# qcc4cp/qcc

Measured on AMD Instinct MI355X. Metric: gate-applies/sec (2^30-amplitude units), QFT, higher is better.
Workload: dtype f64; 1 GPU; 30-qubit QFT complex128, 465 gates/step (qc.qft order), basis-state input, state resident in HBM, 2^30 amplitudes per GPU [BASELINE config 2]; qubits=30, fusion=1

## Files before the change

### include/qcc_hip.h

```cpp
#ifndef QCC_HIP_H_
#define QCC_HIP_H_

#include <stdint.h>

#ifdef __cplusplus
extern "C" {
#endif

typedef struct qh_state_s *qh_handle;

#define QH_OK 0
#define QH_ERR_BAD_QUBIT 1
#define QH_ERR_SAME_QUBIT 2
#define QH_ERR_BAD_DTYPE 3
#define QH_ERR_HIP 4
#define QH_ERR_ARG 5
#define QH_ERR_NOMEM 6
#define QH_ERR_NO_DEVICE 7
#define QH_ERR_NONLOCAL 8
#define QH_ERR_COMM 9

#define QH_FUSE_OFF 0
#define QH_FUSE_SWEEP 1

const char *qh_last_error(void);
int qh_version(void);
int qh_device_count(int *count);

int qh_create(int nbits, int bit_width, int device, qh_handle *out);
int qh_attach(int nbits, int bit_width, int device, void *device_ptr,
              void *hip_stream, qh_handle *out);
int qh_create_host_mapped(int nbits, int bit_width, int device, qh_handle *out);
int qh_host_ptr(qh_handle h, void **host_ptr);
int qh_create_dry(int nbits, int bit_width, qh_handle *out);
int qh_destroy(qh_handle h);

int qh_set_shard(qh_handle h, int nbits_global, uint64_t shard_index);
int qh_device_ptr(qh_handle h, void **ptr);
int qh_set_relayout(qh_handle h, int on, int *actual);
int qh_stream(qh_handle h, void **stream);
int qh_nbits(qh_handle h, int *nbits_local, int *nbits_global);

int qh_init_basis(qh_handle h, uint64_t index);
int qh_init_product(qh_handle h, int nfactors, const int *nq, const double *const *amps,
                    const uint64_t *basis);
int qh_upload(qh_handle h, const void *host, uint64_t offset, uint64_t count);
int qh_download(qh_handle h, void *host, uint64_t offset, uint64_t count);

int qh_apply1(qh_handle h, int tgt, const double gate[8]);
int qh_applyc(qh_handle h, int ctl, int tgt, const double gate[8]);
int qh_apply_bits(qh_handle h, uint64_t ctl_mask, int tgt_bit,
                  const double gate[8]);
int qh_apply_matrix(qh_handle h, int k, const int32_t *bits, uint64_t ctl_mask, const double *matrix);

int qh_apply_mux(qh_handle h, int k, const int32_t *sel_bits, int tgt_bit, const double *gates);
int qh_apply_diag(qh_handle h, int k, const int32_t *bits, const double *values);

#define QH_NO_CTL INT32_MIN
int qh_apply_stream(qh_handle h, uint64_t count, const int32_t *ops, const double *gates);

int qh_set_fusion(qh_handle h, int level);
int qh_flush(qh_handle h);
int qh_sync(qh_handle h);
int qh_pending_gates(qh_handle h, uint64_t *count);
int qh_discard_pending(qh_handle h);

int qh_remap_swap(qh_handle h, int phys_bit_a, int phys_bit_b);
int qh_get_bitmap(qh_handle h, int32_t *phys_of_logical );
int qh_phys_to_logical(qh_handle h, uint64_t phys_index, uint64_t *logical);
int qh_logical_to_phys(qh_handle h, uint64_t logical_index, uint64_t *phys);

#define QH_COMM_ID_BYTES 128
typedef int (*qh_round_fn)(void *user, int npeers, const int *peers, void *const *send_host,
                           void *const *recv_host, uint64_t bytes);
typedef struct {
  uint64_t exchanges;
  uint64_t rounds;
  uint64_t bytes_sent;
  uint64_t slabs;
  uint64_t sweeps_overlapped;
  double span_ms;
  uint64_t rounds_packed;
  uint64_t geometry_checks;
  uint32_t comm_ranks;
  uint32_t comm_rank;
} qh_xstats;
typedef struct {
  uint64_t signature;
  uint64_t slab_mask;
  uint64_t block_bits;
  uint64_t rounds_per_slab;
  uint64_t staging_bytes;
  uint32_t slabs;
  uint32_t chunk_bits;
  uint32_t packed;
  uint32_t peers;
  uint32_t sweeps_before;
  uint32_t last_sweep_split;
} qh_xgeom;
int qh_exchange_geometry(qh_handle h, qh_xgeom *out);
int qh_comm_init_dry(qh_handle h, int nranks, int rank);
int qh_comm_unique_id(void *id );
int qh_comm_init(qh_handle h, int nranks, int rank, const void *id);
int qh_comm_init_custom(qh_handle h, int nranks, int rank, qh_round_fn fn, void *user);
int qh_comm_destroy(qh_handle h);
int qh_exchange_alltoall(qh_handle h, int base_bit, uint64_t chunk_amps);
int qh_exchange_pair(qh_handle h, int shard_bit, int local_bit, uint64_t chunk_amps);
int qh_exchange_loopback(qh_handle h, int local_bit, uint64_t chunk_amps);
int qh_exchange_wait(qh_handle h);
int qh_exchange_stats(qh_handle h, qh_xstats *out);
int qh_comm_allreduce_sum(qh_handle h, double *inout, int count);

int qh_norm2(qh_handle h, double *out);
int qh_amplitude(qh_handle h, uint64_t logical_index, double out[2]);
int qh_argmax(qh_handle h, uint64_t *phys_index, double *prob);
int qh_prob_bit(qh_handle h, int logical_bit, double *p1);
int qh_prob_bit_value(qh_handle h, int logical_bit, int value, double *p);
int qh_scale(qh_handle h, double re, double im);
int qh_project_bit(qh_handle h, int logical_bit, int value);
int qh_marginal(qh_handle h, int k, const int32_t *bits, double *out);
int qh_sample(qh_handle h, uint64_t count, const double *u, uint64_t *logical_out);
int qh_project_bits(qh_handle h, uint64_t mask, uint64_t value);
int qh_expect_pauli(qh_handle h, uint64_t nterms, const uint64_t *xmask, const uint64_t *zmask, double *out);
typedef struct { uint64_t index; double re, im; } qh_entry;
#define QH_SELECT_MAX (1u << 20)
#define QH_TOPK_MAX 4096
int qh_select(qh_handle h, double threshold, uint64_t cap, qh_entry *out, uint64_t *count, double *weight);
int qh_topk(qh_handle h, uint64_t k, qh_entry *out, uint64_t *count);
int qh_amplitudes(qh_handle h, uint64_t count, const uint64_t *logical, double *out, uint64_t *nlocal);

int qh_clone(qh_handle src, qh_handle *out);
int qh_copy(qh_handle dst, qh_handle src);
int qh_inner(qh_handle a, qh_handle b, double out[2]);
#define QH_INNER_LINEAR 0
#define QH_INNER_TILES 1
#define QH_INNER_GATHER 2
typedef struct {
  uint32_t path;
  uint32_t nrest;
  uint64_t free_a, free_b;
  uint8_t tile_a[8], tile_b[8], shuffle[8];
  uint8_t rest_a[56], rest_b[56];
  uint8_t pos_b[64];
} qh_inner_tiles;
int qh_inner_plan(qh_handle a, qh_handle b, qh_inner_tiles *out);
int qh_axpby(qh_handle dst, const double alpha[2], qh_handle src, const double beta[2], double *norm2);

int qh_extend(qh_handle src, int k, const double *amps, uint64_t basis, qh_handle *out);
int qh_release(qh_handle src, int k, const int32_t *bits, uint64_t value, double weight[2], qh_handle *out);

typedef struct {
  uint64_t gates_submitted;
  uint64_t kernels_launched;
  uint64_t sweeps;
  uint64_t bytes_algorithmic;
  uint64_t bytes_swept;
  uint64_t gates_noop;
} qh_stats;
int qh_get_stats(qh_handle h, qh_stats *out);
int qh_reset_stats(qh_handle h);
int qh_timer_begin(qh_handle h);
int qh_timer_end(qh_handle h, float *milliseconds);
int qh_timer_lap(qh_handle h);
int qh_timer_laps(qh_handle h, float *milliseconds, int cap, int *count);
int qh_plan_json(qh_handle h, char *buf, uint64_t cap, uint64_t *needed);

int qh_plan_export(qh_handle h, void *buf, uint64_t cap, uint64_t *needed);

int qh_plan_handlers(qh_handle h, void *buf, uint64_t cap, uint64_t *needed);

int qh_host_apply1(void *psi, const double gate[8], int nbits, int tgt,
                   int bit_width);
int qh_host_applyc(void *psi, const double gate[8], int nbits, int ctl, int tgt,
                   int bit_width);
int qh_host_release(void);

#ifdef __cplusplus
}
#endif
#endif
```

### qcc_amd/csrc/engine.hip

```cpp
#include <hip/hip_runtime.h>

#include <algorithm>
#include <chrono>
#include <cmath>
#include <cstdarg>
#include <cstddef>
#include <cstdio>
#include <cstdlib>
#include <cstring>
#include <ctime>
#include <string>
#include <vector>

#include "../../include/qcc_hip.h"
#include "buffers.hip.h"
#include "kernels_gate.hip.h"
#include "kernels_dense.hip.h"
#include "kernels_mux.hip.h"
#include "kernels_measure.hip.h"
#include "kernels_select.hip.h"
#include "select_plan.h"
#include "kernels_expect.hip.h"
#include "kernels_inner.hip.h"
#include "kernels_axpby.hip.h"
// ... 221 lines not shown
  launch_diag_u<R, 2, true>(h, nwork, sel, ins, f0r, f0i, f1r, f1i, lowpred);
}

int launch_single(qh_state_s *h, const qh::GateRec &r) {
  const Placed ctl = place(h, r.ctl_mask);
  if ((h->shard & ctl.held) != ctl.held) {
    h->stats.gates_noop++;
    return QH_OK;
  }
  const uint64_t cm_all = ctl.local;
  const LowSplit low = split_low(h, cm_all);
  uint32_t lowpred = low.lowpred;
  const uint64_t cm = low.cm;
  const int nc_all = __builtin_popcountll(cm_all);
  const int nc = __builtin_popcountll(cm);
  if (nc + 1 > qh::kMaxIns) return fail(QH_ERR_ARG, "too many local control bits (%d)", nc);
  const double *g = r.g;
  const bool diag = qh::is_diag(g);
  auto diag_kernel = [&](uint64_t nwork, int sel, uint64_t ones, double f0r, double f0i, double f1r, double f1i) {
    if (h->dry) return;
    const qh::BitIns ins = make_ins(ones, -1);
    with_real(h, [&](auto x) { launch_diag<decltype(x)>(h, nwork, sel, ins, f0r, f0i, f1r, f1i, lowpred); });
  };
  if (r.tgt >= h->nloc) {
    if (!diag)
      return fail(QH_ERR_NONLOCAL,
                  "non-diagonal gate targets physical bit %d held by the shard index "
                  "(local bits: %d); exchange first",
                  r.tgt, h->nloc);
    const bool set = (h->shard >> (r.tgt - h->nloc)) & 1ull;
    const double fr = set ? g[6] : g[0], fi = set ? g[7] : g[1];
    if (fr == 1.0 && fi == 0.0) {
      h->stats.gates_noop++;
      return QH_OK;
    }
    const uint64_t nwork = 1ull << (h->nloc - nc);
    diag_kernel(nwork, -1, cm, 1, 0, fr, fi);
    count_kernel(h, 1ull << (h->nloc - nc_all), nwork);
    return QH_OK;
  }
  if (diag) {
    const bool one_sided = (g[0] == 1.0 && g[1] == 0.0);
    if (one_sided && g[6] == 1.0 && g[7] == 0.0) {
      h->stats.gates_noop++;
      return QH_OK;
    }
    if (one_sided) {
      const bool tgt_low = h->nloc > 2 && r.tgt < 2;
      if (tgt_low) lowpred |= 1u << r.tgt;
      const uint64_t nwork = 1ull << (h->nloc - nc - (tgt_low ? 0 : 1));
      diag_kernel(nwork, -1, tgt_low ? cm : (cm | (1ull << r.tgt)), 1, 0, g[6], g[7]);
      count_kernel(h, 1ull << (h->nloc - nc_all - 1), nwork);
    } else {
      const uint64_t nwork = 1ull << (h->nloc - nc);
      diag_kernel(nwork, r.tgt, cm, g[0], g[1], g[6], g[7]);
      count_kernel(h, 1ull << (h->nloc - nc_all), nwork);
    }
    return QH_OK;
  }
  const uint64_t nwork = 1ull << (h->nloc - nc - 1);
  if (!h->dry) {
    const qh::BitIns ins = make_ins(cm, r.tgt), ins1 = make_ins(cm, -1);
    with_real(h, [&](auto x) { launch_pair<decltype(x)>(h, nwork, r.tgt, ins, ins1, g, lowpred); });
  }
  count_kernel(h, 1ull << (h->nloc - nc_all), 2 * nwork);
  return QH_OK;
}

int check_launch(qh_state_s *h) {
  if (h->dry) return QH_OK;
  hipError_t e = hipGetLastError();
  if (e != hipSuccess) return fail(QH_ERR_HIP, "kernel launch: %s", hipGetErrorString(e));
  return QH_OK;
}

int use_device(qh_state_s *h) {
  if (h->dry) return QH_OK;
  HIP_TRY(hipSetDevice(h->device));
  return QH_OK;
}

int comm_timeout_ms() { return env_int("QH_COMM_TIMEOUT_MS", 300000); }
bool watched(const qh_state_s *h) {
  if (!h->comm || h->comm->dry) return false;
  return (h->comm->nranks > 1 && !h->comm->custom) || env_int("QH_COMM_WATCH_ALL", 0) != 0;
}
void abort_comm_and_drain(qh_state_s *h) {
  qh::Comm *c = h->comm;
  if (!c || c->dry) return;
  if (c->nccl) {
    (void)qh::rccl().CommAbort(c->nccl);
    c->nccl = nullptr;
  }
  const auto t0 = std::chrono::steady_clock::now();
  for (hipStream_t s : {c->xstream, c->cstream, c->pstream, h->stream}) {
    if (!s) continue;
    while (hipStreamQuery(s) == hipErrorNotReady) {
      if (std::chrono::duration<double>(std::chrono::steady_clock::now() - t0).count() > 10.0) return;
      struct timespec ts = {0, 200000};
      nanosleep(&ts, nullptr);
    }
  }
  (void)hipGetLastError();
}
template <typename Query> int poll_until_done(qh_state_s *h, Query query, const char *what) {
  const auto t0 = std::chrono::steady_clock::now();
  for (unsigned spins = 0;; ++spins) {
    const hipError_t e = query();
    if (e == hipSuccess) return QH_OK;
    if (e != hipErrorNotReady) {
      (void)hipGetLastError();
      return fail(QH_ERR_HIP, "%s: %s", what, hipGetErrorString(e));
    }
    if (spins > 2000) {
      const double ms = std::chrono::duration<double, std::milli>(std::chrono::steady_clock::now() - t0).count();
      if (ms > comm_timeout_ms()) {
        h->poisoned = true;
        abort_comm_and_drain(h);
        return fail(QH_ERR_COMM, "%s: rank %d of %d still waiting after %.0f s (QH_COMM_TIMEOUT_MS): a peer is missing or the "
                    "ranks disagree about an exchange; the communicator was aborted, the state of this handle is undefined", what,
                    h->comm->rank, h->comm->nranks, ms * 1e-3);
      }
      struct timespec ts = {0, 50000};
      nanosleep(&ts, nullptr);
    }
  }
}
int wait_stream(qh_state_s *h, hipStream_t s, const char *what) {
  if (!watched(h)) {
    HIP_TRY(hipStreamSynchronize(s));
    return QH_OK;
  }
  return poll_until_done(h, [&] { return hipStreamQuery(s); }, what);
}
int wait_event(qh_state_s *h, hipEvent_t e, const char *what) {
  if (!watched(h)) {
    HIP_TRY(hipEventSynchronize(e));
    return QH_OK;
  }
  return poll_until_done(h, [&] { return hipEventQuery(e); }, what);
}

bool relayout_eligible(const qh_state_s *h) {
  return env_int("QH_RELAYOUT", 1) != 0 && h->owns_mem && !h->host_psi && qh::sweep_supported(h->nloc, h->bw);
}
bool relayout_wanted(const qh_state_s *h) {
  if (h->dry) return env_int("QH_RELAYOUT", 1) != 0;
  if (h->relayout >= 0) return h->relayout == 1;
  return relayout_eligible(h) && !(h->comm && h->comm->nranks > 1);
}
qh::PlanRequest plan_request(const qh_state_s *h, bool relayout) {
  return qh::PlanRequest{h->nloc, h->bw, h->shard, relayout, h->nglob > h->nloc, qh::PlanSwitches::from_env()};
}
hipError_t alloc_state_buffer(void **p, size_t bytes) {
  static const int contig = env_int("QH_ALLOC_CONTIG", -1), debug = env_int("QH_ALLOC_DEBUG", 0);
  const auto t0 = std::chrono::steady_clock::now();
  hipError_t e = hipErrorOutOfMemory;
  bool got_contig = false;
  const bool want_contig = contig < 0 ? (bytes >= (4ull << 30) && bytes <= (32ull << 30)) : (contig > 0 && bytes >= (64ull << 20));
  if (want_contig) {
    e = hipExtMallocWithFlags(p, bytes, hipDeviceMallocContiguous);
    got_contig = e == hipSuccess;
    if (!got_contig) {
      (void)hipGetLastError();
      *p = nullptr;
    }
  }
  if (!got_contig) e = hipMalloc(p, bytes);
  if (debug)
    fprintf(stderr, "[qh alloc %zu MiB %s at %p in %.1f ms]\n", bytes >> 20, got_contig ? "contiguous" : "plain", *p,
            std::chrono::duration<double, std::milli>(std::chrono::steady_clock::now() - t0).count());
  return e;
}
bool second_buffer_fits(const qh_state_s *h, size_t bytes) {
  size_t fr = 0, total = 0;
  const size_t reserve = (bytes >> 5) + (3ull << 29) + ((h->comm && h->comm->nranks > 1) ? (4ull << 30) : 0);
  return hipMemGetInfo(&fr, &total) == hipSuccess && fr > bytes + reserve;
}
bool alloc_second_buffer(qh_state_s *h) {
  if (h->d_alt) return true;
  const size_t bytes = (size_t)h->amp_bytes() << h->nloc;
  if (second_buffer_fits(h, bytes) && alloc_state_buffer(&h->d_alt, bytes) == hipSuccess)
    return true;
  (void)hipGetLastError();
  h->d_alt = nullptr;
  return false;
}
bool relayout_ready(qh_state_s *h) {
  if (h->dry) return relayout_wanted(h);
  if (h->relayout < 0) {
    h->relayout = 0;
    if (relayout_eligible(h) && !(h->comm && h->comm->nranks > 1) && alloc_second_buffer(h)) h->relayout = 1;
  }
  return h->relayout == 1;
}

bool layout_is_canonical(const qh_state_s *h) {
  int last = -1;
  for (int b = 0; b < h->nglob; ++b) {
    if (h->perm[b] >= h->nloc) continue;
    if (h->perm[b] < last) return false;
    last = h->perm[b];
  }
  return true;
}

int canonicalize(qh_state_s *h) {
  if (h->dry || layout_is_canonical(h)) return QH_OK;
  const bool borrowed = !h->d_alt;
  if (borrowed && !alloc_second_buffer(h))
    return fail(QH_ERR_NOMEM, "no room for the second buffer of %llu bytes that bringing a permuted layout back to canonical order needs",
                (unsigned long long)(h->amp_bytes() << h->nloc));
  std::vector<int> loc;
  for (int b = 0; b < h->nglob; ++b) if (h->perm[b] < h->nloc) loc.push_back(b);
  std::vector<int> posn;
  for (int b : loc) posn.push_back(h->perm[b]);
  std::sort(posn.begin(), posn.end());
  qh::BitPerm bp{};
  bp.n = h->nloc;
  for (size_t k = 0; k < loc.size(); ++k) bp.src_of_dst[posn[k]] = (uint8_t)h->perm[loc[k]];
  const uint64_t n = 1ull << h->nloc;
  with_real(h, [&](auto x) {
    using R = decltype(x);
    using A = typename qh::AmpT<R>::type;
    hipLaunchKernelGGL(qh::k_permute_bits<R>, dim3(grid_for(n, 1ull << 22)), dim3(256), 0, h->stream, (const A *)h->d_psi, (A *)h->d_alt, n, bp);
  });
  int rc = check_launch(h);
  if (rc == QH_OK && borrowed) {
    hipError_t e = hipMemcpyAsync(h->d_psi, h->d_alt, (size_t)h->amp_bytes() << h->nloc, hipMemcpyDefault, h->stream);
    if (e == hipSuccess) e = hipStreamSynchronize(h->stream);
    if (e != hipSuccess) rc = fail(QH_ERR_HIP, hipGetErrorString(e));
  }
  if (borrowed) {
    if (rc) (void)hipStreamSynchronize(h->stream);
    (void)hipFree(h->d_alt);
    h->d_alt = nullptr;
  } else if (rc == QH_OK) {
    std::swap(h->d_psi, h->d_alt);
  }
  if (rc) return rc;
  for (size_t k = 0; k < loc.size(); ++k) h->perm[loc[k]] = posn[k];
  return QH_OK;
}

int flush_impl(qh_state_s *h, qh::SlabIO *split = nullptr, qh::TileMaxOut *tmax = nullptr) {
  int rc = use_device(h);
  if (rc) return rc;
  if (h->poisoned)
    return fail(QH_ERR_HIP, "the state of this handle is undefined: a sweep of an earlier flush failed after others had run; "
                            "re-initialise it (qh_init_basis / qh_init_product / qh_upload of the whole shard)");
  std::vector<qh::Arrival> *arr = (h->comm && !h->comm->arrivals.empty()) ? &h->comm->arrivals : nullptr;
  if (h->queue.empty()) {
    qh::wait_all_arrivals(arr, h->stream);
    return QH_OK;
  }
  if (h->fusion == QH_FUSE_SWEEP && qh::sweep_supported(h->nloc, h->bw)) {
    const uint64_t launched0 = h->stats.kernels_launched;
    qh::SlabIO local;
    qh::SlabIO *io = split ? split : &local;
    io->arrivals = arr;
    io->comm = h->comm;
    const bool relay = relayout_ready(h);
    void *result = h->d_psi;
    uint8_t final_pos[64];
    rc = qh::run_fused(h->queue, plan_request(h, relay), h->d_psi, h->stream, h->dry, &h->sweep, &h->stats, &g_err,
                       h->comm ? io : nullptr, h->d_alt, &result, final_pos, tmax);
    if (rc == QH_OK && relay) {
      if (result != h->d_psi) std::swap(h->d_psi, h->d_alt);
      for (int b = 0; b < h->nglob; ++b)
        if (h->perm[b] < h->nloc) h->perm[b] = final_pos[h->perm[b]];
    }
    qh::wait_all_arrivals(arr, h->stream);
    if (h->comm) h->comm->stats.sweeps_overlapped += io->sweeps_overlapped;
    if (rc != QH_OK && h->stats.kernels_launched == launched0) return rc;
    if (rc == QH_OK) rc = check_launch(h);
    if (rc != QH_OK) {
      g_err += " [sweeps of this flush may have run partially: its gates were dropped and the state is undefined until re-initialised]";
      h->poisoned = true;
    }
    h->queue.clear();
    return rc;
  }
  qh::wait_all_arrivals(arr, h->stream);
  size_t done = 0;
  for (const auto &r : h->queue) {
    rc = launch_single(h, r);
    if (rc == QH_OK) rc = check_launch(h);
    if (rc) break;
    ++done;
  }
  h->queue.erase(h->queue.begin(), h->queue.begin() + done);
  return rc;
}

int enter(qh_state_s *h) {
  if (h->dry) return fail(QH_ERR_ARG, "not on a dry (planner-only) handle");
  return flush_impl(h);
}
int read_back(qh_state_s *h, void *host, const void *dev, size_t bytes, const char *what = "reader") {
  HIP_TRY(hipMemcpyAsync(host, dev, bytes, hipMemcpyDeviceToHost, h->stream));
  return wait_stream(h, h->stream, what);
}

int set_relayout(qh_state_s *h, bool on, int *actual = nullptr) {
  if (h->dry) {
    if (actual) *actual = relayout_wanted(h) ? 1 : 0;
// ... 1824 lines not shown
  return QH_OK;
}

}

namespace {

constexpr uint64_t kExpectBlocks = 4096;

template <typename R, int TT>
void launch_expect(qh_state_s *h, bool pair, unsigned nblk, const qh::ExpectArgs &a, double *slab) {
  using A = typename qh::AmpT<R>::type;
  if (pair)
    hipLaunchKernelGGL((qh::k_expect_batch<R, TT, true>), dim3(nblk), dim3(256), 0, h->stream, (const A *)h->d_psi, a, slab);
  else
    hipLaunchKernelGGL((qh::k_expect_batch<R, TT, false>), dim3(nblk), dim3(256), 0, h->stream, (const A *)h->d_psi, a, slab);
}

}

extern "C" {

int qh_expect_pauli(qh_handle h, uint64_t nterms, const uint64_t *xmask, const uint64_t *zmask, double *out) {
  if (!h || (nterms && (!xmask || !zmask || !out))) return fail(QH_ERR_ARG, "expect_pauli: null handle, masks or out");
  if (h->nglob < 64)
    for (uint64_t t = 0; t < nterms; ++t)
      if ((xmask[t] | zmask[t]) >> h->nglob)
        return fail(QH_ERR_BAD_QUBIT, "expect_pauli: term %llu (x 0x%llx, z 0x%llx) has bits >= %d", (unsigned long long)t,
                    (unsigned long long)xmask[t], (unsigned long long)zmask[t], h->nglob);
  int rc = enter(h);
  if (rc) return rc;
  if (nterms == 0) return QH_OK;
  struct Term { uint64_t px, pz, idx; uint32_t neg, ny; };
  std::vector<Term> terms(nterms);
  for (uint64_t t = 0; t < nterms; ++t) {
    const Placed x = place(h, to_phys(h, xmask[t])), z = place(h, to_phys(h, zmask[t]));
    if (x.held) {
      const int b = __builtin_ctzll(to_logical(h, x.held << h->nloc));
      return fail(QH_ERR_NONLOCAL, "expect_pauli: term %llu has X or Y on logical bit %d, held by the shard index (physical bit %d, "
                  "local bits: %d); exchange first", (unsigned long long)t, b, h->perm[b], h->nloc);
    }
    terms[t] = Term{x.local, z.local, t, (uint32_t)__builtin_popcountll(h->shard & z.held) & 1u,
                    (uint32_t)__builtin_popcountll(xmask[t] & zmask[t]) & 3u};
  }
  std::stable_sort(terms.begin(), terms.end(), [](const Term &l, const Term &r) { return l.px < r.px; });
  qh::ScratchLayout lay;
  const size_t slab_off = lay.add((size_t)kExpectBlocks * qh::kExpectT * sizeof(double)), out_off = lay.add((size_t)nterms * sizeof(double));
  HIP_TRY(h->meas.reserve(lay.total));
  double *slab = (double *)(h->meas.as<char>() + slab_off), *dout = (double *)(h->meas.as<char>() + out_off);
  uint64_t batches = 0;
  for (uint64_t first = 0; first < nterms;) {
    uint64_t cnt = 1;
    while (first + cnt < nterms && cnt < (uint64_t)qh::kExpectT && terms[first + cnt].px == terms[first].px) ++cnt;
    const uint64_t px = terms[first].px;
    const bool pair = (px >> 6) != 0;
    qh::ExpectArgs a{};
    a.x = px;
    a.tb = pair ? 63 - __builtin_clzll(px) : 0;
    const int per_bits = pair ? 3 : 4, nom = 8 + per_bits, wbits = pair ? h->nloc - 1 : h->nloc;
    a.cw = std::min(nom, wbits);
    const uint64_t nchunks = 1ull << (wbits - a.cw), nblk = std::min(nchunks, kExpectBlocks);
    a.cpb = (uint32_t)(nchunks / nblk);
    for (uint64_t k = 0; k < cnt; ++k) {
      const Term &tm = terms[first + k];
      uint64_t z = tm.pz;
      if (pair) z = (z & ((1ull << a.tb) - 1ull)) | ((z >> (a.tb + 1)) << a.tb);
      a.zt[k] = (uint8_t)(z & 255ull);
      const uint32_t zu = (uint32_t)(z >> 8) & ((1u << per_bits) - 1u);
      for (uint32_t u = 0; u < (1u << per_bits); ++u) a.zu[k] |= (uint16_t)((__builtin_popcount(u & zu) & 1) << u);
      a.zc[k] = z >> nom;
      const uint32_t one = (((tm.ny >> 1) ^ tm.neg) & 1u) ? 0xBFF00000u : 0x3FF00000u;
      if (tm.ny & 1u) a.cim[k] = one; else a.cre[k] = one;
    }
    const int tt = cnt <= 4 ? 4 : qh::kExpectT;
    with_real(h, [&](auto x) {
      using R = decltype(x);
      if (tt == 4) launch_expect<R, 4>(h, pair, (unsigned)nblk, a, slab);
      else launch_expect<R, qh::kExpectT>(h, pair, (unsigned)nblk, a, slab);
    });
    hipLaunchKernelGGL(qh::k_expect_fold, dim3((unsigned)cnt), dim3(256), 0, h->stream, (const double *)slab, (uint32_t)nblk, tt,
                       pair ? 2.0 : 1.0, dout + first);
    if ((rc = check_launch(h))) return rc;
    first += cnt;
    ++batches;
  }
  std::vector<double> vals(nterms);
  if ((rc = read_back(h, vals.data(), dout, (size_t)nterms * sizeof(double)))) return rc;
  for (uint64_t k = 0; k < nterms; ++k) out[terms[k].idx] = vals[k];
  h->stats.kernels_launched += batches;
  h->stats.bytes_swept += batches * ((1ull << h->nloc) * h->amp_bytes());
  return QH_OK;
}

int qh_get_stats(qh_handle h, qh_stats *out) {
  if (!h || !out) return fail(QH_ERR_ARG, "null");
  *out = h->stats;
  return QH_OK;
}
int qh_reset_stats(qh_handle h) {
  if (!h) return fail(QH_ERR_ARG, "null");
  h->stats = qh_stats{};
  return QH_OK;
}

int qh_timer_begin(qh_handle h) {
  if (!h) return fail(QH_ERR_ARG, "null handle");
  int rc = enter(h);
  if (rc) return rc;
  rc = make_events(h);
  if (rc) return rc;
  HIP_TRY(hipEventRecord(h->ev0, h->stream));
  return QH_OK;
}
int qh_timer_end(qh_handle h, float *ms) {
  if (!h || !ms) return fail(QH_ERR_ARG, "null handle or out");
  if (!h->ev0) return fail(QH_ERR_ARG, "qh_timer_end without qh_timer_begin");
  int rc = enter(h);
  if (rc) return rc;
  HIP_TRY(hipEventRecord(h->ev1, h->stream));
  if ((rc = wait_event(h, h->ev1, "qh_timer_end"))) return rc;
  HIP_TRY(hipEventElapsedTime(ms, h->ev0, h->ev1));
  return QH_OK;
}

int qh_timer_lap(qh_handle h) {
  if (!h) return fail(QH_ERR_ARG, "null handle");
  const int rc = enter(h);
  if (rc) return rc;
  if (h->laps_used == h->laps.size()) {
    hipEvent_t e = nullptr;
    HIP_TRY(hipEventCreate(&e));
    h->laps.push_back(e);
  }
  HIP_TRY(hipEventRecord(h->laps[h->laps_used++], h->stream));
  return QH_OK;
}
int qh_timer_laps(qh_handle h, float *ms, int cap, int *count) {
  if (!h || !count || h->dry) return fail(QH_ERR_ARG, "null/dry");
  HIP_TRY(hipSetDevice(h->device));
  const int n = h->laps_used > 0 ? (int)h->laps_used - 1 : 0;
  if (h->laps_used) {
    const int rc = wait_event(h, h->laps[h->laps_used - 1], "qh_timer_laps");
    if (rc) return rc;
  }
  for (int k = 0; k < n && ms && k < cap; ++k) HIP_TRY(hipEventElapsedTime(&ms[k], h->laps[k], h->laps[k + 1]));
  *count = n;
  h->laps_used = 0;
  return QH_OK;
}

int qh_plan_json(qh_handle h, char *buf, uint64_t cap, uint64_t *needed) {
  if (!h) return fail(QH_ERR_ARG, "null");
  std::string s;
  if (int rc = qh::guard_planning(&g_err, [&] { s = qh::plan_to_json(h->queue, plan_request(h, relayout_wanted(h))); })) return rc;
  if (needed) *needed = s.size() + 1;
  if (buf && cap) {
    const uint64_t n = std::min<uint64_t>(cap - 1, s.size());
    memcpy(buf, s.data(), n);
    buf[n] = 0;
  }
  return QH_OK;
}

int qh_plan_export(qh_handle h, void *buf, uint64_t cap, uint64_t *needed) {
  if (!h) return fail(QH_ERR_ARG, "null");
  if (!qh::sweep_supported(h->nloc, h->bw)) return fail(QH_ERR_ARG, "state too small for sweeps");
  qh::PlanResult pr;
  if (int rc = qh::guard_planning(&g_err, [&] { pr = qh::plan_best(h->queue, plan_request(h, relayout_wanted(h))); })) return rc;
  std::vector<uint64_t> out;
  auto put_bytes = [&](const void *p, size_t n) {
    const size_t w = (n + 7) / 8, at = out.size();
    out.resize(at + w, 0);
    if (n) memcpy(&out[at], p, n);
  };
  out.push_back(0x51485033ull);
  out.push_back(pr.sweeps.size());
  out.push_back(pr.noop_gates);
  put_bytes(pr.final_pos, 64);
  for (auto &sp : pr.sweeps) {
    int64_t hdr[28] = {0};
    int k = 0;
    hdr[k++] = sp.rb;
    for (int i = 0; i < 6; ++i) hdr[k++] = sp.regpos[i];
    for (int i = 0; i < 6; ++i) hdr[k++] = sp.regpos_store[i];
    for (int i = 0; i < 3; ++i) hdr[k++] = sp.lanehi[i];
    hdr[k++] = sp.nwave;
    for (int i = 0; i < 2; ++i) hdr[k++] = sp.wavepos[i];
    hdr[k++] = (int64_t)sp.fixed_ones;
    hdr[k++] = (int64_t)sp.ntiles;
    hdr[k++] = (int64_t)sp.ops.size();
    hdr[k++] = (int64_t)sp.groups.size();
    hdr[k++] = (int64_t)sp.oterms.size();
    hdr[k++] = (int64_t)sp.tables.size();
    hdr[k++] = sp.n_ltab;
    hdr[k++] = sp.lane_low;
    hdr[k++] = sp.relayout ? 1 : 0;
    put_bytes(hdr, sizeof hdr);
    put_bytes(sp.dest_pos, 64);
    {
      int64_t st[20] = {0};
      for (int i = 0; i < 6; ++i) { st[i] = sp.seat[i]; st[6 + i] = sp.seat_store[i]; st[12 + i] = sp.seat_dest[i]; }
      st[18] = sp.wavepos_store[0];
      st[19] = sp.wavepos_store[1];
      put_bytes(st, sizeof st);
      int64_t kd[8 + 1 + 2 * qh::kMaxUnitSegs] = {0};
      for (int i = 0; i < 6; ++i) kd[i] = sp.reg_dest[i];
      kd[6] = sp.wave_dest[0];
      kd[7] = sp.wave_dest[1];
      uint64_t masks[qh::kMaxUnitSegs] = {0};
      int shifts[qh::kMaxUnitSegs] = {0};
      kd[8] = sp.relayout ? qh::unit_segments(sp, h->nloc, masks, shifts) : 0;
      for (int i = 0; i < qh::kMaxUnitSegs; ++i) { kd[9 + i] = (int64_t)masks[i]; kd[9 + qh::kMaxUnitSegs + i] = shifts[i]; }
      put_bytes(kd, sizeof kd);
    }
    put_bytes(sp.ops.data(), sp.ops.size() * sizeof(qh::SweepOp));
    put_bytes(sp.groups.data(), sp.groups.size() * sizeof(qh::DGroup));
    put_bytes(sp.oterms.data(), sp.oterms.size() * sizeof(qh::OTerm));
    put_bytes(sp.tables.data(), sp.tables.size() * sizeof(double));
  }
  const uint64_t bytes = out.size() * 8;
  if (needed) *needed = bytes;
  if (buf && cap) {
    if (cap < bytes) return fail(QH_ERR_ARG, "buffer too small (call with NULL to get the size)");
    memcpy(buf, out.data(), bytes);
  }
  return QH_OK;
}

int qh_plan_handlers(qh_handle h, void *buf, uint64_t cap, uint64_t *needed) {
  if (!h) return fail(QH_ERR_ARG, "null");
  if (!qh::sweep_supported(h->nloc, h->bw)) return fail(QH_ERR_ARG, "state too small for sweeps");
  qh::PlanResult pr;
  if (int rc = qh::guard_planning(&g_err, [&] { pr = qh::plan_best(h->queue, plan_request(h, relayout_wanted(h))); })) return rc;
  std::vector<uint32_t> out{0x51484831u, (uint32_t)pr.sweeps.size()};
  std::vector<qh::SweepOp> ops;
  std::vector<qh::DGroup> groups;
  for (auto &sp : pr.sweeps) {
    ops.assign(sp.ops.size() + 1, qh::SweepOp{});
    groups.assign(sp.groups.size(), qh::DGroup{});
    const uint32_t n_ltab_lds = (uint32_t)(h->bw == 128 ? qh::ltab_lds_count<true>(sp) : qh::ltab_lds_count<false>(sp));
    qh::build_device_copy(sp, h->bw, n_ltab_lds, ops.data(), groups.data());
    for (uint32_t v : {(uint32_t)h->bw, (uint32_t)sp.rb, (uint32_t)sp.nwave, (uint32_t)(sp.relayout ? 1 : 0), (uint32_t)sp.ops.size(),
                       (uint32_t)sp.groups.size()})
      out.push_back(v);
    for (size_t k = 0; k < sp.ops.size(); ++k) { out.push_back(ops[k].kind); out.push_back(ops[k].flags); }
    for (const qh::DGroup &g : groups) out.push_back(g.flags);
  }
  if (out.size() & 1) out.push_back(0);
  const uint64_t bytes = out.size() * 4;
  if (needed) *needed = bytes;
  if (buf && cap) {
    if (cap < bytes) return fail(QH_ERR_ARG, "buffer too small (call with NULL to get the size)");
    memcpy(buf, out.data(), bytes);
  }
  return QH_OK;
}

}

namespace {

#define NCCL_TRY(expr)                                                                     \
  do {                                                                                     \
    ncclResult_t r_ = (expr);                                                              \
    if (r_ != ncclSuccess)                                                                 \
      return fail(QH_ERR_COMM, "%s: %s (%s:%d)", #expr, qh::rccl().GetErrorString(r_), __FILE__, __LINE__); \
  } while (0)

int check_ranks(int nranks, int rank) {
  if (nranks < 1 || (nranks & (nranks - 1)) || rank < 0 || rank >= nranks)
    return fail(QH_ERR_ARG, "nranks %d must be a power of two, rank %d inside it", nranks, rank);
  if (nranks > qh::kMaxXferMoves + 1) return fail(QH_ERR_ARG, "at most %d ranks", qh::kMaxXferMoves + 1);
  return QH_OK;
}

int comm_common_init(qh_state_s *h, int nranks, int rank) {
  if (!h) return fail(QH_ERR_ARG, "null handle");
  if (h->comm) return fail(QH_ERR_ARG, "handle already has a communicator");
  if (int rc = check_ranks(nranks, rank)) return rc;
  if (h->bw != 128 && h->bw != 64) return fail(QH_ERR_BAD_DTYPE, "bit width");
  int rc0 = enter(h);
  if (rc0) return rc0;
  if (nranks > 1 && h->relayout != 0) {
    rc0 = set_relayout(h, false);
    if (rc0) return rc0;
  }
  auto *c = new qh::Comm;
  c->nranks = nranks;
  c->rank = rank;
  hipError_t e = hipStreamCreateWithFlags(&c->xstream, hipStreamNonBlocking);
  if (e == hipSuccess) e = hipStreamCreateWithFlags(&c->cstream, hipStreamNonBlocking);
  if (e == hipSuccess) e = hipStreamCreateWithFlags(&c->pstream, hipStreamNonBlocking);
  if (e == hipSuccess) e = hipEventCreate(&c->t0);
  if (e == hipSuccess) e = hipEventCreate(&c->t1);
  if (e != hipSuccess) {
    delete c;
    return fail(QH_ERR_HIP, "exchange streams/events: %s", hipGetErrorString(e));
  }
  h->comm = c;
  return QH_OK;
}

void close_timing(qh::Comm *c) {
  if (!c->timing_open) return;
  float ms = 0;
  if (hipEventSynchronize(c->t1) == hipSuccess && hipEventElapsedTime(&ms, c->t0, c->t1) == hipSuccess)
    c->stats.span_ms += ms;
  c->timing_open = false;
}

template <typename A>
void launch_xfer(bool unpack, void *psi, void *stage, uint64_t n, uint64_t start, const qh::XferGeom &g, hipStream_t st) {
  const uint64_t total = n * (uint64_t)g.np;
  const unsigned grid = grid_for(total, 1ull << 20);
  if (unpack) hipLaunchKernelGGL(qh::k_xunpack<A>, dim3(grid), dim3(256), 0, st, (A *)psi, (const A *)stage, n, start, g);
  else hipLaunchKernelGGL(qh::k_xpack<A>, dim3(grid), dim3(256), 0, st, (const A *)psi, (A *)stage, n, start, g);
}

int verify_geometry(qh_state_s *h, uint64_t sig) {
  qh::Comm *c = h->comm;
  if (c->nranks <= 1) return QH_OK;
  if (c->custom) {
    const int np = c->nranks - 1;
    std::vector<uint64_t> mine(np, sig), theirs(np, 0);
    std::vector<int> peers;
    std::vector<void *> sp, rp;
    for (int j = 0, k = 0; j < c->nranks; ++j) {
      if (j == c->rank) continue;
      peers.push_back(j);
      sp.push_back(&mine[k]);
      rp.push_back(&theirs[k]);
      ++k;
    }
    if (c->custom(c->custom_user, np, peers.data(), sp.data(), rp.data(), sizeof(uint64_t)) != 0)
      return fail(QH_ERR_COMM, "host-staged transport: the round callback failed (geometry check)");
    for (int k = 0; k < np; ++k)
      if (theirs[k] != sig)
        return fail(QH_ERR_COMM, "exchange geometry differs between rank %d (%016llx) and rank %d (%016llx): the ranks "
                    "planned different sweeps or layouts", c->rank, (unsigned long long)sig, peers[k], (unsigned long long)theirs[k]);
    c->stats.geometry_checks++;
    return QH_OK;
  }
  if (!c->nccl) return fail(QH_ERR_COMM, "no RCCL communicator on this handle (never set up, or aborted by the watchdog)");
  static const int mode = env_int("QH_EXCHANGE_VERIFY", -1);
  if (mode == 0) return QH_OK;
  if (mode < 0 && std::find(c->verified.begin(), c->verified.end(), sig) != c->verified.end()) return QH_OK;
  HIP_TRY(c->d_sig.reserve(4 * sizeof(double)));
  HIP_TRY(c->h_sig.reserve(8 * sizeof(double)));
  double *v = c->h_sig.as<double>(), *w = v + 4, *d_sig = c->d_sig.as<double>();
  v[0] = (double)(sig >> 32); v[1] = (double)(sig & 0xffffffffu); v[2] = -v[0]; v[3] = -v[1];
  HIP_TRY(hipMemcpyAsync(d_sig, v, 4 * sizeof(double), hipMemcpyHostToDevice, c->xstream));
  NCCL_TRY(qh::rccl().AllReduce(d_sig, d_sig, 4, ncclDouble, ncclMax, c->nccl, c->xstream));
  HIP_TRY(hipMemcpyAsync(w, d_sig, 4 * sizeof(double), hipMemcpyDeviceToHost, c->xstream));
  const int rc = wait_stream(h, c->xstream, "exchange geometry check (all-reduce of the signature)");
  if (rc) return rc;
  if (w[0] != -w[2] || w[1] != -w[3])
    return fail(QH_ERR_COMM, "exchange geometry differs between ranks (signature of rank %d: %016llx; largest / smallest halves seen: "
                "%08x%08x / %08x%08x): the ranks planned different sweeps or layouts, or run with different planner switches "
                "(QH_* environment) or builds", c->rank, (unsigned long long)sig, (unsigned)w[0], (unsigned)w[1], (unsigned)-w[2], (unsigned)-w[3]);
  if (c->verified.size() >= 256) c->verified.erase(c->verified.begin());
  c->verified.push_back(sig);
  c->stats.geometry_checks++;
  return QH_OK;
}

uint64_t env_build_hash(const qh::ExchangeSwitches &xsw) {
  std::string s = qh::PlanSwitches::from_env().key();
  s += xsw.key() + std::to_string(env_int("QH_RELAYOUT", 1) != 0) + ";";
  s += "v" + std::to_string(qh_version()) + ":" + std::to_string(sizeof(qh::SweepArgs)) + ":" + std::to_string(sizeof(qh::SweepOp)) +
       ":" + std::to_string(sizeof(qh::SweepPlan)) + ":" + std::to_string(sizeof(qh_xgeom));
  uint64_t hsh = 0xcbf29ce484222325ull;
  for (unsigned char ch : s) { hsh ^= ch; hsh *= 0x100000001b3ull; }
  return hsh;
}

void launch_packed_round(qh_state_s *h, const qh::ExchangePlan &pl, const std::vector<qh::BlockMove> &moves, bool unpack, void *stage,
                         int k, uint64_t ci, hipStream_t st) {
  qh::XferGeom g{};
  g.ins.n = pl.nins;
  for (int i = 0; i < pl.nins; ++i) g.ins.pos[i] = pl.ins_pos[i];
  g.np = pl.np;
  for (int m = 0; m < pl.np; ++m) g.off[m] = pl.packed_offset(k, unpack ? moves[m].land : moves[m].blk);
  with_real(h, [&](auto x) {
    launch_xfer<typename qh::AmpT<decltype(x)>::type>(unpack, h->d_psi, stage, pl.chunk_amps(), pl.round_start(ci), g, st);
  });
}
// ... 409 lines not shown
```

### qcc_amd/csrc/kernels_sweep.hip.h

```cpp
#pragma once
#include <hip/hip_runtime.h>

#include <string>
#include <vector>

#include "kernels_gate.hip.h"
#include <deque>
#include <memory>

#include "planner.h"
#include "exchange.hip.h"

namespace qh {

struct SweepParams {
  const SweepOp *ops;
  const DGroup *groups;
  const OTerm *oterms;
  uint32_t nops;
  uint32_t tables_rel;
  uint32_t n_ltab_lds;
  uint32_t pad0;
  uint64_t store_delta_mask;
  uint64_t prof_buf;
  uint64_t tilemax;
  uint64_t slot_off[64];
  uint64_t slot_off_store[64];
};
static_assert(kMaxInsertBits + kMaxSlabBits <= kMaxIns, "planner/kernels disagree on inserted bits");
static_assert(kExchangeSlabBits == kMaxSlabBits, "exchange_plan.h / planner disagree on slab bits");
static_assert(sizeof(SweepOp) == 96 && sizeof(DGroup) == 64 && sizeof(OTerm) == 24, "asm island layouts");
static_assert(offsetof(SweepParams, slot_off) == 0x40 && offsetof(SweepParams, nops) == 0x18 && offsetof(SweepParams, tilemax) == 0x38 &&
                  offsetof(SweepParams, slot_off_store) == 0x240 && offsetof(SweepParams, store_delta_mask) == 0x28,
              "asm island layouts");

struct LaneGeom {
  int lane_low;
  int rot;
  int blk_bits;
  int nwave;
  int wpos[kMaxWaveBits];
  int wdst[kMaxWaveBits];
  int ltab_in_island;
};

constexpr uint64_t kProfRows = 8192, kProfRecs = 128;
struct UnitPerm {
  int n;
  int shift[kMaxUnitSegs];
  uint64_t mask[kMaxUnitSegs];
  int nslab;
  int slab_pos[kMaxSlabBits];
  uint64_t slab_val;
};

struct alignas(8) SweepArgs {
  uint64_t psi;
  uint64_t dst;
  uint64_t prm;
  uint64_t idx_high;
  uint64_t nunits;
  uint64_t ins_ones;
  uint64_t slab_val;
  uint64_t ltab_src;
  uint32_t n_ltab;
  uint32_t exch_bytes;
  uint32_t stride_units;
  uint32_t seat_dest;
  uint8_t ins_n, lane_low, rot, blk_bits;
  uint8_t nwave, wpos[2], island_copies;
  uint8_t wdst[2], up_n, up_nslab;
  uint8_t slab_pos[kMaxSlabBits], wpb;
  uint8_t seat[8];
  uint8_t ins_pos[16];
  int8_t up_shift[kMaxUnitSegs];
  uint64_t up_mask[kMaxUnitSegs];
};
static_assert(kMaxUnitSegs == 8 && kMaxSlabBits == 3 && kMaxIns <= 16 && kMaxWaveBits == 2 && kLaneBits <= 8, "SweepArgs layout");
static_assert(offsetof(SweepArgs, n_ltab) == 64 && offsetof(SweepArgs, ins_n) == 80 && offsetof(SweepArgs, ins_pos) == 104 &&
                  offsetof(SweepArgs, up_shift) == 120 && offsetof(SweepArgs, up_mask) == 128 && sizeof(SweepArgs) == 192,
              "SweepArgs layout (k_sweep reads it by dword index)");

typedef uint32_t qh_u32x16 __attribute__((ext_vector_type(16)));

inline int flush_pace(const PlanResult &pr, bool wide, int nloc) {
  if (const char *e = getenv("QH_SWEEP_PACE")) return atoi(e);
  if (!wide || pr.sweeps.empty()) return 0;
  double joules = 0, ms = 0;
  for (const SweepPlan &sp : pr.sweeps) {
    if (sp.nwave > 1) return 0;
    const double units = (double)sp.swept_bytes / (2.0 * 16.0 * (double)(1ull << 30));
    ms += (nloc <= 31 ? 5.45 : 5.85) * units;
    joules += 4.9 * units + sweep_op_energy_nj(sp) * (double)sp.ntiles * 1e-9 * 1.15;
  }
  const double watts = joules / ms * 1e3;
  return (watts >= 1320.0 && watts <= 1450.0) ? 12 : 0;
}

template <int RB, bool WIDE>
__global__ __launch_bounds__(256) void k_sweep(SweepArgs args_in_kernarg_segment) {
  constexpr uint32_t kAmp = WIDE ? 16u : 8u;
#ifdef QH_PROF
  const uint64_t prof_t_entry = __builtin_amdgcn_s_memtime();
#endif
  const uint32_t lane_u = threadIdx.x & 63;
  const uint32_t wave_s = __builtin_amdgcn_readfirstlane(threadIdx.x >> 6);
  extern __shared__ __attribute__((aligned(16))) unsigned char xbuf[];
  const uint32_t lds_base = (uint32_t)(uintptr_t)(__attribute__((address_space(3))) unsigned char *)xbuf;
  for (uint32_t turn = 0;; ++turn) {
    qh_u32x16 q0, q1, q2;
    asm volatile("s_load_dwordx16 %0, %3, 0x0\n\ts_load_dwordx16 %1, %3, 0x40\n\ts_load_dwordx16 %2, %3, 0x80\n\t"
                 "s_waitcnt lgkmcnt(0)"
                 : "=&s"(q0), "=&s"(q1), "=&s"(q2)
                 : "s"((uint64_t)(uintptr_t)__builtin_amdgcn_kernarg_segment_ptr()));
    auto dw = [&](int i) -> uint32_t { return i < 16 ? q0[i] : i < 32 ? q1[i - 16] : q2[i - 32]; };
    auto qw = [&](int i) -> uint64_t { return (uint64_t)dw(i) | ((uint64_t)dw(i + 1) << 32); };
    auto by = [&](int i, int b) -> uint32_t { return (dw(i) >> (8 * b)) & 255u; };
    const uint32_t lane_low = by(20, 1), nwave = by(21, 0), wpb = by(23, 3);
    const uint32_t n_lt = dw(16), exch_bytes = dw(17);
    const uint32_t lds_ltab = lds_base + exch_bytes;
    const uint32_t wg_threads = wpb << 6;
    const bool island_copies = by(21, 3) != 0;
    if (turn == 0 && n_lt && !island_copies) {
      typedef double v2d_t __attribute__((ext_vector_type(2)));
      const __attribute__((address_space(1))) v2d_t *src = (const __attribute__((address_space(1))) v2d_t *)qw(14);
      v2d_t *dst = (v2d_t *)(xbuf + exch_bytes);
      for (uint32_t i = threadIdx.x; i < n_lt * 64u; i += wg_threads) dst[i] = src[i];
      __syncthreads();
    }
    const uint32_t nlt_now = island_copies && turn == 0 ? n_lt : 0u;
    uint64_t bi = blockIdx.x;
    const uint32_t rot = by(20, 2), blk_bits = by(20, 3);
    if (rot) bi = ((bi >> rot) | (bi << (blk_bits - rot))) & ((1ull << blk_bits) - 1);
    const uint32_t upb = wpb >> nwave;
    const uint64_t wu = bi * upb + (wave_s >> nwave) + (uint64_t)turn * dw(18);
    if (wu >= qw(8)) break;
    uint32_t lane_t = lane_u;
    asm volatile("" : "+v"(lane_t));
    uint32_t loff = 0;
#pragma unroll
    for (int i = 0; i < kLaneBits; ++i) loff |= ((lane_t >> i) & 1u) << by(24 + i / 4, i % 4);
    const uint32_t voff = loff * kAmp;
    uint64_t wave_off = 0, woff = 0;
#pragma unroll
    for (int j = 0; j < kMaxWaveBits; ++j)
      if ((uint32_t)j < nwave) {
        wave_off |= (uint64_t)((wave_s >> j) & 1u) << by(21, 1 + j);
        woff |= (uint64_t)((wave_s >> j) & 1u) << by(22, j);
      }
    uint64_t base = wu << lane_low;
    const uint32_t ins_n = by(20, 0);
#pragma unroll
    for (int k = 0; k < kMaxIns; ++k)
      if ((uint32_t)k < ins_n) {
        const uint64_t low = (1ull << by(26 + k / 4, k % 4)) - 1ull;
// ... 43 lines not shown
#ifdef QH_PROF
    const uint64_t prof_id = (wu << nwave) | (wave_s & ((1u << nwave) - 1u));
    const uint64_t prof_buf = ((const __attribute__((address_space(4))) SweepParams *)prm)->prof_buf;
    const uint64_t prof_row = (prof_buf && (prof_id & 63) == 0 && (prof_id >> 6) < kProfRows)
                                  ? prof_buf + (prof_id >> 6) * (kProfRecs * 8) : 0;
    if (prof_row && lane_u == 0) ((uint64_t *)prof_row)[125] = prof_t_entry;
#endif
    if constexpr (WIDE) {
      if constexpr (RB == 2) {
#include "sweep_island_rb2.inc"
      } else if constexpr (RB == 3) {
#include "sweep_island_rb3.inc"
      } else if constexpr (RB == 4) {
#include "sweep_island_rb4.inc"
      } else {
#ifdef QH_PROF
#include "sweep_island_prof_rb5.inc"
#else
#include "sweep_island_rb5.inc"
#endif
      }
    } else {
      if constexpr (RB == 2) {
#include "sweep_island_f32_rb2.inc"
      } else if constexpr (RB == 3) {
#include "sweep_island_f32_rb3.inc"
      } else if constexpr (RB == 4) {
#include "sweep_island_f32_rb4.inc"
      } else if constexpr (RB == 5) {
#include "sweep_island_f32_rb5.inc"
      } else {
#include "sweep_island_f32_rb6.inc"
      }
    }
  }
}

inline uint32_t group_handler_bits(const DGroup &g, int rb, bool sign_oterms = false) {
  uint32_t id = 0;
  const int pc = popc(g.reg_mask);
  if (pc == 1) id = 1 + (uint32_t)__builtin_ctz(g.reg_mask);
  else if (pc == 2) {
    const int b0 = __builtin_ctz(g.reg_mask), b1 = 31 - __builtin_clz(g.reg_mask);
    int idx = 0;
    for (int x = 0; x < b0; ++x) idx += rb - 1 - x;
    id = 1 + (uint32_t)rb + (uint32_t)(idx + b1 - b0 - 1);
  } else if (pc > 2) id = 1 + (uint32_t)rb + (uint32_t)(rb * (rb - 1) / 2);
  const uint32_t n_masks = 1 + (uint32_t)rb + (uint32_t)(rb * (rb - 1) / 2) + 1;
  const bool general = (g.flags & DG_LTAB) || g.ntab || g.n_oterms;
  if (sign_oterms) return 16u | ((id + n_masks + (uint32_t)rb) << 8);
  if (g.flags & DG_BITFAC)
    id = (general ? n_masks : 4 * n_masks + (uint32_t)rb) + (uint32_t)__builtin_ctz(g.reg_mask);
  else if (!general && g.re == -1.0 && g.im == 0.0) id += n_masks + (uint32_t)rb;
  else if (!general && g.lane_mask == 0) id += 2 * n_masks + (uint32_t)rb;
  else if (!general) id += 3 * n_masks + (uint32_t)rb;
  return (general ? 4u : 0u) | (id << 8);
}
#include "sweep_handlers.inc"
inline uint32_t reg_mask_number(uint32_t reg_mask, int rb) {
  const int pc = popc(reg_mask);
  if (pc == 1) return (uint32_t)__builtin_ctz(reg_mask);
  if (pc == 2) {
    const int b0 = __builtin_ctz(reg_mask), b1 = 31 - __builtin_clz(reg_mask);
    int idx = 0;
    for (int x = 0; x < b0; ++x) idx += rb - 1 - x;
    const uint32_t no = (uint32_t)(rb + idx + b1 - b0 - 1);
    return no < 15u ? no : 15u;
  }
  return 15u;
}
constexpr uint32_t kOpSentinel = (kHidDone << 16) | 0xffffu;
inline uint32_t op_handler_id(const SweepOp &o) {
  switch (o.kind) {
    case OP_DIAG: return kHidDiag;
    case OP_WSWAP: return kHidWswap;
    case OP_LSWAP: return kHidLswap + 2 * o.cm_reg + (o.tb - 4);
    default: break;
  }
  if (!(o.flags & OPF_BFLY)) return kHidDense;
  if (o.kind == OP_DENSE_LANE) return (o.flags & OPF_LANE_DPP) ? kHidBflyLaneDpp : kHidBflyLane;
  const uint32_t variant = (o.flags >> OPF_BFLY_SHIFT) & 7;
  if (o.flags & (OPF_ROT_P | OPF_ROT_M)) return kHidBflyRot + 8 * (5 * ((o.flags & OPF_ROT_M) ? 1u : 0u) + variant) + o.tb;
  return kHidBflyReg + 8 * variant + o.tb;
}

inline void build_device_copy(const SweepPlan &sp, int bw, uint32_t n_ltab_lds, SweepOp *ops_out, DGroup *groups_out) {
  if (!sp.ops.empty()) memcpy(ops_out, sp.ops.data(), sp.ops.size() * sizeof(SweepOp));
  for (size_t k = 0; k < sp.ops.size(); ++k) {
    SweepOp *o = ops_out + k;
    o->kind |= op_handler_id(*o) << 16;
    if (o->flags & (OPF_ROT_P | OPF_ROT_M)) {
      const double c = o->g[0], c2 = 2.0 * o->g[0];
      memcpy(&o->cm_thread, &c, 8);
      memcpy(&o->cm_reg, &c2, 8);
    }
  }
  ops_out[sp.ops.size()].kind = kOpSentinel;
  for (size_t k = 0; k < sp.ops.size(); ++k) {
    SweepOp *o = ops_out + k;
    if ((o->kind & 0xffffu) != OP_DIAG) continue;
    bool any = false, all_neg = true;
    for (uint32_t gi = 0; gi < o->n_groups; ++gi) {
      const DGroup &g = sp.groups[o->group_off + gi];
      if (g.reg_mask) continue;
      any = true;
      all_neg &= !(g.flags & (DG_LTAB | DG_BITFAC)) && !g.ntab && !g.n_oterms && g.re == -1.0 && g.im == 0.0;
    }
    if (any && all_neg) o->flags |= 1u << 9;
  }
  if (bw == 128)
    for (size_t k = 0; k < sp.ops.size(); ++k) {
      SweepOp *o = ops_out + k;
      if ((o->kind & 0xffffu) != OP_DIAG || o->n_groups != 1 || (o->flags & OPF_DEFER_C)) continue;
      const DGroup &g = sp.groups[o->group_off];
      if (!g.reg_mask || (g.flags & (DG_LTAB | DG_BITFAC)) || g.ntab || g.n_oterms || g.lane_mask > 63u) continue;
      const uint32_t cls = (g.re == -1.0 && g.im == 0.0) ? 0u : g.lane_mask == 0 ? 1u : 2u;
      const uint32_t mi = reg_mask_number(g.reg_mask, sp.rb);
      o->kind = OP_DIAG | ((kHidDiag1 + 16u * cls + mi) << 16);
      o->tb = g.lane_mask | (g.reg_mask << 8);
      memcpy(&o->cm_reg, &g.re, 8);
      memcpy(&o->cm_thread, &g.im, 8);
    }
  if (!sp.groups.empty()) memcpy(groups_out, sp.groups.data(), sp.groups.size() * sizeof(DGroup));
  for (size_t k = 0; k < sp.groups.size(); ++k) {
    DGroup *g = groups_out + k;
    if (n_ltab_lds && (g->flags & DG_LTAB) && g->ltab_off / 64 < n_ltab_lds) g->flags |= DG_LTAB_LDS;
    bool sign_ot = !(g->flags & (DG_LTAB | DG_BITFAC)) && g->ntab == 0 && g->n_oterms > 0 && g->re == 1.0 && g->im == 0.0;
    for (uint32_t t = 0; sign_ot && t < g->n_oterms; ++t) {
      const OTerm &o = sp.oterms[g->oterm_off + t];
      sign_ot = o.re == -1.0 && o.im == 0.0;
    }
    g->flags |= group_handler_bits(*g, sp.rb, sign_ot);
  }
}

struct PlanCacheEntry {
  std::vector<GateRec> queue;
  std::string key;
  std::shared_ptr<const PlanResult> plan;
};

inline bool same_queue(const std::vector<GateRec> &a, const std::vector<GateRec> &b) {
  if (a.size() != b.size()) return false;
  for (size_t i = 0; i < a.size(); ++i)
    if (a[i].ctl_mask != b[i].ctl_mask || a[i].tgt != b[i].tgt || a[i].neg_mask != b[i].neg_mask ||
        memcmp(a[i].g, b[i].g, sizeof a[i].g) != 0)
      return false;
  return true;
}

struct SweepBuffers {
  std::deque<PlanCacheEntry> plans;
  StagedUpload<1> ops;
};

inline bool sweep_supported(int nloc, int bw) { return (bw == 128 || bw == 64) && nloc >= kLaneBits + 2; }

template <bool WIDE> inline void sweep_block_shape(const SweepPlan &sp, int *wpb, size_t *exch_bytes) {
  const bool contiguous = sp.contiguous();
  *wpb = contiguous ? 2 : 4;
  *exch_bytes = 0;
  if (sp.nwave) {
    *wpb = 1 << sp.nwave;
    const int nr = 1 << sp.rb;
    *exch_bytes = (size_t)*wpb * std::min(8, nr / 2) * 64 * (WIDE ? 16 : 8);
  }
}

template <bool WIDE> inline int ltab_lds_count(const SweepPlan &sp) {
  constexpr int cap = 16;
  int wpb;
  size_t exch;
  sweep_block_shape<WIDE>(sp, &wpb, &exch);
  const long per_wg = 160l * 1024 * wpb / 12 - (long)exch - 512;
  const int fit = (int)std::max(0l, per_wg / 1024);
  return std::max(0, std::min(std::min(sp.n_ltab, cap), fit));
}

inline int sweep_rot(bool contiguous) { return contiguous ? 3 : 6; }

inline uint64_t sweep_tile_bits(const SweepPlan &sp) {
  uint64_t m = ((1ull << sp.lane_low) - 1) | sp.fixed_ones;
  for (int k = 0; k < sp.rb; ++k) m |= (1ull << sp.regpos[k]) | (1ull << sp.regpos_store[k]);
  for (int k = 0; k < sp.nlanehi(); ++k) m |= 1ull << sp.lanehi[k];
  for (int k = 0; k < sp.nwave; ++k) m |= 1ull << sp.wavepos[k];
  return m;
}

inline bool sweep_takes_slab(const SweepPlan &sp, uint64_t slab_mask) {
  return !(sweep_tile_bits(sp) & slab_mask) && popc(slab_mask) <= kMaxSlabBits &&
         popc(sp.fixed_ones) + sp.rb + sp.nlanehi() + sp.nwave + popc(slab_mask) <= kMaxIns &&
         (sp.ntiles >> popc(slab_mask)) >= 64;
}

inline BitIns make_tile_ins(const SweepPlan &sp, uint64_t slab_mask = 0, uint64_t slab_val = 0) {
  BitIns ins{};
  ins.n = 0;
  ins.ones = sp.fixed_ones | slab_val;
  uint64_t regmask = slab_mask;
  for (int k = 0; k < sp.rb; ++k) regmask |= 1ull << sp.regpos[k];
  for (int k = 0; k < sp.nlanehi(); ++k) regmask |= 1ull << sp.lanehi[k];
  for (int k = 0; k < sp.nwave; ++k) regmask |= 1ull << sp.wavepos[k];
  for (int b = 0; b < 64; ++b)
    if (((regmask | sp.fixed_ones) >> b) & 1ull) ins.pos[ins.n++] = b;
  return ins;
}

template <bool WIDE>
void launch_sweep_t(const SweepPlan &sp, void *psi, int nloc, uint64_t shard, hipStream_t stream,
                    const SweepParams *d_prm, const SweepParams &h_prm, int pace, uint64_t slab_mask, uint64_t slab_val, void *dst) {
  int wpb;
  size_t lds_bytes;
  sweep_block_shape<WIDE>(sp, &wpb, &lds_bytes);
  const uint32_t exch_bytes = (uint32_t)lds_bytes;
  lds_bytes += (size_t)ltab_lds_count<WIDE>(sp) * 1024;
  const uint64_t ntiles = sp.ntiles >> popc(slab_mask);
  uint64_t blocks = (ntiles + wpb - 1) / wpb;
  const int upw = sp.nwave >= 2 ? 4 : 1;
  if (upw > 1 && blocks % upw == 0 && blocks / upw >= 4096) blocks /= upw;
  if (blocks > 0x7fffffffull) blocks = 0x7fffffffull;
  const dim3 grid((unsigned)blocks), block(64 * wpb);
  const BitIns ins = make_tile_ins(sp, slab_mask, slab_val);
  LaneGeom lg;
  lg.lane_low = sp.lane_low;
  lg.nwave = sp.nwave;
  for (int k = 0; k < kMaxWaveBits; ++k) lg.wpos[k] = k < sp.nwave ? sp.wavepos[k] : 0;
  for (int k = 0; k < kMaxWaveBits; ++k) lg.wdst[k] = k < sp.nwave ? sp.wave_dest[k] : 0;
  lg.ltab_in_island = !WIDE;
  lg.rot = 0;
  lg.blk_bits = 0;
  while ((1ull << lg.blk_bits) < blocks) lg.blk_bits++;
  const int rot = sweep_rot(sp.contiguous());
  if (rot > 0 && (1ull << lg.blk_bits) == blocks && ntiles % (blocks * wpb) == 0 && lg.blk_bits > rot + 2) lg.rot = rot;
  const uint64_t idx_high = shard << nloc;
  UnitPerm up{};
  if (dst && sp.relayout) {
    up.n = unit_segments(sp, nloc, up.mask, up.shift);
    if (up.n == 1 && up.shift[0] == 0) up.n = 0;
    if (slab_mask) {
      const uint64_t tile = sweep_tile_bits(sp);
      for (uint64_t m = slab_mask; m; m &= m - 1) {
        const int b = __builtin_ctzll(m);
        const int upos = popc(~tile & ((1ull << b) - 1));
        up.slab_pos[up.nslab++] = upos;
        if ((slab_val >> b) & 1ull) up.slab_val |= 1ull << upos;
      }
    }
  }
  SweepArgs ka{};
  ka.psi = (uint64_t)psi;
  ka.dst = (uint64_t)dst;
  ka.prm = (uint64_t)d_prm;
  ka.idx_high = idx_high;
  ka.nunits = ntiles >> sp.nwave;
  ka.ins_ones = ins.ones;
  ka.slab_val = up.slab_val;
  ka.ltab_src = (uint64_t)((const char *)h_prm.groups + h_prm.tables_rel);
  ka.n_ltab = h_prm.n_ltab_lds;
  ka.exch_bytes = exch_bytes;
  const uint32_t upb = (uint32_t)wpb >> sp.nwave;
  ka.stride_units = (uint32_t)blocks * upb;
  ka.ins_n = (uint8_t)ins.n;
  ka.lane_low = (uint8_t)lg.lane_low;
  ka.rot = (uint8_t)lg.rot;
  ka.blk_bits = (uint8_t)lg.blk_bits;
  ka.nwave = (uint8_t)lg.nwave;
  for (int k = 0; k < kMaxWaveBits; ++k) { ka.wpos[k] = (uint8_t)lg.wpos[k]; ka.wdst[k] = (uint8_t)lg.wdst[k]; }
  ka.island_copies = lg.ltab_in_island && (uint64_t)blocks * upb == ka.nunits;
  ka.up_n = (uint8_t)up.n;
  ka.up_nslab = (uint8_t)up.nslab;
  for (int k = 0; k < kMaxSlabBits; ++k) ka.slab_pos[k] = (uint8_t)up.slab_pos[k];
  ka.wpb = (uint8_t)wpb;
  for (int i = 0; i < kLaneBits; ++i) {
    ka.seat[i] = (uint8_t)sp.seat[i];
    ka.seat_dest |= (uint32_t)((dst && sp.relayout) ? sp.seat_dest[i] : i) << (4 * i);
  }
  ka.seat[7] = (uint8_t)std::max(0, std::min(255, pace));
  for (int k = 0; k < ins.n; ++k) ka.ins_pos[k] = (uint8_t)ins.pos[k];
  for (int k = 0; k < up.n; ++k) { ka.up_shift[k] = (int8_t)up.shift[k]; ka.up_mask[k] = up.mask[k]; }
  switch (sp.rb) {
    case 2: hipLaunchKernelGGL((k_sweep<2, WIDE>), grid, block, lds_bytes, stream, ka); break;
    case 3: hipLaunchKernelGGL((k_sweep<3, WIDE>), grid, block, lds_bytes, stream, ka); break;
    case 4: hipLaunchKernelGGL((k_sweep<4, WIDE>), grid, block, lds_bytes, stream, ka); break;
    case 6:
      if constexpr (!WIDE) {
        hipLaunchKernelGGL((k_sweep<6, false>), grid, block, lds_bytes, stream, ka);
        break;
      }
      [[fallthrough]];
    default: hipLaunchKernelGGL((k_sweep<5, WIDE>), grid, block, lds_bytes, stream, ka); break;
  }
}

inline void launch_sweep(const SweepPlan &sp, void *psi, int nloc, uint64_t shard, int bw, hipStream_t stream,
                         const SweepParams *d_prm, const SweepParams &h_prm, int pace, uint64_t slab_mask, uint64_t slab_val,
                         void *dst) {
  if (bw == 128) launch_sweep_t<true>(sp, psi, nloc, shard, stream, d_prm, h_prm, pace, slab_mask, slab_val, dst);
  else launch_sweep_t<false>(sp, psi, nloc, shard, stream, d_prm, h_prm, pace, slab_mask, slab_val, dst);
}

struct TileMaxOut {
  void *buf = nullptr;
  uint64_t cap = 0;
  bool valid = false;
  uint64_t nunits = 0;
  BitIns ins{};
  uint64_t tile_mask = 0;
};

struct SlabIO {
  std::vector<Arrival> *arrivals = nullptr;
  bool split_last = false;
  uint64_t avoid = 0;
  int want_bits = 3;
  Comm *comm = nullptr;
  uint64_t slab_mask = 0;
  std::vector<uint64_t> slab_vals;
  std::vector<hipEvent_t> slab_done;
  bool split_done = false;
  uint64_t sweeps_overlapped = 0;
};

inline void wait_all_arrivals(std::vector<Arrival> *arr, hipStream_t stream) {
  if (!arr) return;
  for (const Arrival &a : *arr) if (a.ev) (void)hipStreamWaitEvent(stream, a.ev, 0);
  arr->clear();
}

inline int run_fused(const std::vector<GateRec> &queue, const PlanRequest &rq, void *psi, hipStream_t stream, bool dry,
                     SweepBuffers *bufs, qh_stats *stats, std::string *err, SlabIO *slab = nullptr, void *psi_alt = nullptr,
                     void **result = nullptr, uint8_t *final_pos = nullptr, TileMaxOut *tmax = nullptr) {
  const int nloc = rq.nloc, bw = rq.bw;
  const uint64_t shard = rq.shard;
  std::shared_ptr<const PlanResult> cached;
  const int rc = guard_planning(err, [&] {
    const std::string key = rq.key();
    const bool use_cache = !getenv("QH_PLAN_CACHE") || atoi(getenv("QH_PLAN_CACHE")) != 0;
    if (use_cache)
      for (auto &e : bufs->plans)
        if (e.key == key && same_queue(e.queue, queue)) { cached = e.plan; return; }
    cached = std::make_shared<const PlanResult>(plan_best(queue, rq));
    if (use_cache) {
      bufs->plans.push_front(PlanCacheEntry{queue, key, cached});
      if (bufs->plans.size() > 4) bufs->plans.pop_back();
    }
  });
  if (rc) return rc;
  const PlanResult &pr = *cached;
  const int pace = dry ? 0 : flush_pace(pr, bw == 128, nloc);
  stats->gates_noop += pr.noop_gates;
  size_t n_ops = 0, n_groups = 0, n_ot = 0, n_tab = 0;
  for (auto &sp : pr.sweeps) {
    if (popc(sp.fixed_ones) + sp.rb + sp.nlanehi() + sp.nwave > kMaxIns) {
      *err = "sweep needs more inserted bits than the tile enumeration supports";
      return QH_ERR_ARG;
    }
    n_ops += sp.ops.size() + 1;
    n_groups += sp.groups.size();
    n_ot += sp.oterms.size();
    n_tab += sp.tables.size();
  }
  const bool want_tmax = tmax && tmax->buf && !dry && !slab && !pr.sweeps.empty() && pr.sweeps.back().fixed_ones == 0 &&
                         (pr.sweeps.back().ntiles >> pr.sweeps.back().nwave) <= tmax->cap;
  if (tmax) tmax->valid = false;
  const size_t bytes_prm = pr.sweeps.size() * sizeof(SweepParams);
  const size_t bytes_ops = n_ops * sizeof(SweepOp), bytes_groups = n_groups * sizeof(DGroup),
               bytes_ot = (n_ot * sizeof(OTerm) + 15) / 16 * 16, bytes_tab = n_tab * sizeof(double);
  const size_t total = bytes_prm + bytes_ops + bytes_groups + bytes_ot + bytes_tab + 256;
  std::vector<char> host_dry;
  char *hbase = nullptr, *d_base = nullptr;
  if (dry) {
    host_dry.resize(total);
    hbase = host_dry.data();
  } else {
    if (hipEvent_t e = bufs->ops.busy()) (void)hipEventSynchronize(e);
    size_t cap = bufs->ops.host.cap;
    if (cap < total) {
      if (cap) (void)hipStreamSynchronize(stream);
      cap = std::max<size_t>(total * 2, 1 << 20);
    }
    unsigned slot = 0;
    const hipError_t e = bufs->ops.acquire(cap, &hbase, &d_base, &slot);
    if (e != hipSuccess) {
      *err = std::string("op buffers (pinned + device): ") + hipGetErrorString(e);
      return e == hipErrorOutOfMemory ? QH_ERR_NOMEM : QH_ERR_HIP;
    }
  }
  memset(hbase, 0, total);
  char *h_prm = hbase, *h_ops = h_prm + bytes_prm, *h_groups = h_ops + bytes_ops,
       *h_ot = h_groups + bytes_groups, *h_tab = h_ot + bytes_ot;
  {
    size_t io = 0, ig = 0, it = 0, is = 0, itab = 0;
    for (auto &sp : pr.sweeps) {
      SweepParams prm{};
      prm.ops = (const SweepOp *)(d_base + bytes_prm) + io;
      prm.groups = (const DGroup *)(d_base + bytes_prm + bytes_ops) + ig;
      prm.oterms = (const OTerm *)(d_base + bytes_prm + bytes_ops + bytes_groups) + it;
      prm.nops = (uint32_t)sp.ops.size();
      prm.n_ltab_lds = (uint32_t)(bw == 128 ? ltab_lds_count<true>(sp) : ltab_lds_count<false>(sp));
      prm.tables_rel = (uint32_t)((d_base + bytes_prm + bytes_ops + bytes_groups + bytes_ot + itab * sizeof(double)) -
                                  (const char *)prm.groups);
      for (int k = 0; k < 64; ++k) {
        uint64_t o = 0;
        for (int b = 0; b < sp.rb; ++b)
          if ((k >> b) & 1) o |= 1ull << sp.regpos[b];
        prm.slot_off[k] = o * (bw == 128 ? 16 : 8);
        o = 0;
        for (int b = 0; b < sp.rb; ++b)
          if ((k >> b) & 1) o |= 1ull << (sp.relayout ? sp.reg_dest[b] : sp.regpos_store[b]);
        prm.slot_off_store[k] = o * (bw == 128 ? 16 : 8);
      }
      prm.store_delta_mask = sp.relayout ? 0ull : ~0ull;
      if (want_tmax && is + 1 == pr.sweeps.size()) prm.tilemax = (uint64_t)tmax->buf;
      memcpy(h_prm + is * sizeof(SweepParams), &prm, sizeof prm);
      build_device_copy(sp, bw, prm.n_ltab_lds, (SweepOp *)(h_ops + io * sizeof(SweepOp)), (DGroup *)(h_groups + ig * sizeof(DGroup)));
      if (!sp.oterms.empty()) memcpy(h_ot + it * sizeof(OTerm), sp.oterms.data(), sp.oterms.size() * sizeof(OTerm));
      if (!sp.tables.empty()) memcpy(h_tab + itab * sizeof(double), sp.tables.data(), sp.tables.size() * sizeof(double));
      io += sp.ops.size() + 1; ig += sp.groups.size(); it += sp.oterms.size(); itab += sp.tables.size(); is++;
    }
  }
  if (!dry) {
    hipError_t e = hipMemcpyAsync(d_base, hbase, total, hipMemcpyHostToDevice, stream);
    if (e == hipSuccess) e = bufs->ops.commit(stream, 0);
    if (e != hipSuccess) {
      *err = std::string("hipMemcpyAsync(op buffer): ") + hipGetErrorString(e);
      return QH_ERR_HIP;
    }
  }
#ifdef QH_PROF
  static char *d_prof = nullptr;
  const size_t prof_bytes = kProfRows * kProfRecs * 8;
  if (!dry) {
    if (!d_prof) (void)hipMalloc(&d_prof, prof_bytes * 16);
    (void)hipMemsetAsync(d_prof, 0, prof_bytes * 16, stream);
    for (size_t k = 0; k < pr.sweeps.size() && k < 16; ++k) {
      const uint64_t v = (uint64_t)(d_prof + k * prof_bytes);
      (void)hipMemcpyAsync(d_base + k * sizeof(SweepParams) + offsetof(SweepParams, prof_buf), &v, 8,
                           hipMemcpyHostToDevice, stream);
      (void)hipStreamSynchronize(stream);
    }
  }
#endif
  if (result) *result = psi;
  if (final_pos) memcpy(final_pos, pr.final_pos, 64);
  static const bool timing = env_flag("QH_SWEEP_TIMING", false);
  std::vector<hipEvent_t> tev;
  void *cur = psi, *other = psi_alt;
  size_t is = 0;
  uint64_t avoid_cur = slab ? slab->avoid : 0;
  uint64_t earlier_tiles = 0;
  for (auto &sp : pr.sweeps) {
    auto moved = [&](uint64_t v) {
      if (!sp.relayout) return v;
      uint64_t o = v >> nloc << nloc;
      for (uint64_t t = v & ((1ull << nloc) - 1); t; t &= t - 1) o |= 1ull << sp.dest_pos[__builtin_ctzll(t)];
      return o;
    };
    if (sp.relayout && !dry && !other) {
      *err = "internal: a relayout sweep was planned without a second buffer";
      return QH_ERR_ARG;
    }
    const SweepParams *prm = (const SweepParams *)d_base + is;
    SweepParams hprm;
    memcpy(&hprm, h_prm + is * sizeof(SweepParams), sizeof hprm);
    const bool first = is == 0, last = is + 1 == pr.sweeps.size();
    bool launched = false;
    if (slab) {
      if (first && slab->arrivals && !slab->arrivals->empty()) {
        const uint64_t am = (*slab->arrivals)[0].slab_mask;
        const bool split_too = last && slab->split_last;
        if (am && !split_too && sweep_takes_slab(sp, am)) {
          for (const Arrival &a : *slab->arrivals) {
            if (dry) continue;
            (void)hipStreamWaitEvent(stream, a.ev, 0);
            launch_sweep(sp, cur, nloc, shard, bw, stream, prm, hprm, pace, a.slab_mask, a.slab_val, sp.relayout ? other : nullptr);
          }
          slab->arrivals->clear();
          slab->sweeps_overlapped++;
          launched = true;
        } else {
          wait_all_arrivals(slab->arrivals, stream);
        }
      }
      if (!launched && last && slab->split_last && (slab->comm || dry)) {
        const int want = std::min(slab->want_bits, kMaxSlabBits);
        const uint64_t taken_bits = avoid_cur | sweep_tile_bits(sp);
        uint64_t m = pick_slab_bits(nloc, taken_bits | ~earlier_tiles, want, kLaneBits);
        if (popc(m) < want) m |= pick_slab_bits(nloc, taken_bits | m, want - popc(m), kLaneBits);
        while (m && !sweep_takes_slab(sp, m)) m &= m - 1;
        if (m) {
          const int K = 1 << popc(m);
          for (int k = 0; k < K; ++k) {
            const uint64_t sv = deposit_bits((uint64_t)k, m);
            hipEvent_t e = nullptr;
            if (!dry) {
              launch_sweep(sp, cur, nloc, shard, bw, stream, prm, hprm, pace, m, sv, sp.relayout ? other : nullptr);
              e = slab->comm->event();
              if (e) (void)hipEventRecord(e, stream);
            }
            slab->slab_done.push_back(e);
            slab->slab_vals.push_back(moved(sv));
          }
          slab->slab_mask = moved(m);
          slab->sweeps_overlapped++;
          slab->split_done = true;
          launched = true;
        }
      }
    }
    if (timing && !dry) {
      hipEvent_t e;
      (void)hipEventCreate(&e);
      (void)hipEventRecord(e, stream);
      tev.push_back(e);
    }
    if (want_tmax && last) {
      tmax->nunits = sp.ntiles >> sp.nwave;
      if (hipMemsetAsync(tmax->buf, 0, tmax->nunits * 8, stream) != hipSuccess) { *err = "hipMemsetAsync(tile maxima)"; return QH_ERR_HIP; }
      uint64_t tm = 0;
      const int tb = kLaneBits + sp.rb + sp.nwave;
      if (sp.relayout) tm = (1ull << tb) - 1;
      else {
        for (int i = 0; i < kLaneBits; ++i) tm |= 1ull << sp.seat_store[i];
        for (int k = 0; k < sp.rb; ++k) tm |= 1ull << sp.regpos_store[k];
        for (int k = 0; k < sp.nwave; ++k) tm |= 1ull << sp.wavepos_store[k];
      }
      tmax->tile_mask = tm;
      tmax->ins = BitIns{};
      for (int b = 0; b < 64; ++b) if ((tm >> b) & 1ull) tmax->ins.pos[tmax->ins.n++] = b;
      tmax->valid = popc(tm) == tb && tmax->ins.n <= kMaxIns;
    }
    if (!dry && !launched) launch_sweep(sp, cur, nloc, shard, bw, stream, prm, hprm, pace, 0, 0, sp.relayout ? other : nullptr);
    if (!dry && sp.relayout) {
      std::swap(cur, other);
      if (result) *result = cur;
    }
    avoid_cur = moved(avoid_cur);
    earlier_tiles = moved(earlier_tiles | (sweep_tile_bits(sp) & ~((1ull << kLaneBits) - 1)));
    is++;
    stats->kernels_launched++;
    stats->sweeps++;
    stats->bytes_algorithmic += sp.alg_bytes;
    stats->bytes_swept += sp.swept_bytes;
  }
#ifdef QH_PROF
  if (!dry && getenv("QH_PROF_OUT")) {
    (void)hipStreamSynchronize(stream);
    std::vector<uint64_t> rec(kProfRows * kProfRecs);
    FILE *f = fopen(getenv("QH_PROF_OUT"), "a");
    for (size_t k = 0; f && k < pr.sweeps.size() && k < 16; ++k) {
      const SweepPlan &sp = pr.sweeps[k];
      (void)hipMemcpy(rec.data(), d_prof + k * prof_bytes, prof_bytes, hipMemcpyDeviceToHost);
      const size_t nrec = std::min<size_t>(sp.ops.size() + 5, kProfRecs);
      std::vector<std::vector<double>> dt(nrec);
      size_t rows = 0;
      for (size_t r = 0; r < kProfRows; ++r) {
        const uint64_t *t = &rec[r * kProfRecs];
        if (!t[0] || !t[nrec - 1]) continue;
        rows++;
        for (size_t j = 0; j + 1 < nrec; ++j) dt[j].push_back((double)(t[j + 1] - t[j]));
      }
      double life = 0, real = 0, tmin = 1e300, tmax = 0, rmin = 1e300, rmax = 0;
      for (size_t r = 0; r < kProfRows; ++r) {
        const uint64_t *t = &rec[r * kProfRecs];
        if (!t[0] || !t[nrec - 1] || !t[126] || !t[127]) continue;
        life += (double)(t[nrec - 1] - t[0]);
        real += (double)(t[127] - t[126]);
        tmin = std::min(tmin, (double)t[0]); tmax = std::max(tmax, (double)t[nrec - 1]);
        rmin = std::min(rmin, (double)t[126]); rmax = std::max(rmax, (double)t[127]);
      }
      fprintf(f, "sweep %zu rb %d nwave %d relayout %d ops %zu rows %zu\n", k, sp.rb, sp.nwave, (int)sp.relayout, sp.ops.size(), rows);
      if (real > 0)
        fprintf(f, "  s_memtime ticks per 10 ns of s_memrealtime: %.3f (waves), %.3f (whole sweep); sweep = %.3f ms by the 100 MHz counter; "
                   "mean wave lifetime %.0f ticks\n", life / real, (tmax - tmin) / (rmax - rmin), (rmax - rmin) * 1e-5, life / rows);
      auto stat = [&](size_t j, const char *what) {
        std::vector<double> &v = dt[j];
        if (v.empty()) return;
        std::sort(v.begin(), v.end());
        double sum = 0;
        for (double x : v) sum += x;
        fprintf(f, "  %-44s mean %9.0f  p10 %8.0f  median %8.0f  p90 %8.0f\n", what, sum / v.size(), v[v.size() / 10], v[v.size() / 2],
                v[v.size() * 9 / 10]);
      };
      stat(0, "tile load (issue + wait)");
      char what[128];
      for (size_t j = 0; j < sp.ops.size() && j + 2 < nrec - 1; ++j) {
        const SweepOp &o = sp.ops[j];
        static const char *kn[] = {"REG", "LANE", "DIAG", "LSWAP", "WSWAP"};
        snprintf(what, sizeof what, "op %2zu %-5s tb %u flags %#x groups %u", j, kn[o.kind], o.tb, o.flags, o.kind == OP_DIAG ? o.n_groups : 0);
        stat(j + 2, what);
      }
      stat(1, "first op header wait / dispatch");
      {
        std::vector<double> v;
        for (size_t r = 0; r < kProfRows; ++r) {
          const uint64_t *t = &rec[r * kProfRecs];
          if (t[0] && t[125] && t[0] > t[125]) v.push_back((double)(t[0] - t[125]));
        }
        if (!v.empty()) {
          std::sort(v.begin(), v.end());
          double sum = 0;
          for (double x : v) sum += x;
          fprintf(f, "  %-44s mean %9.0f  p10 %8.0f  median %8.0f  p90 %8.0f\n", "kernel entry -> island (C++ prologue)", sum / v.size(),
                  v[v.size() / 10], v[v.size() / 2], v[v.size() * 9 / 10]);
        }
      }
      if (sp.ops.size() + 5 <= kProfRecs) {
        stat(nrec - 3, "store issue");
        stat(nrec - 2, "store completion");
      }
    }
    if (f) fclose(f);
  }
#endif
  if (timing && !dry && !tev.empty()) {
    hipEvent_t e;
    (void)hipEventCreate(&e);
    (void)hipEventRecord(e, stream);
    tev.push_back(e);
    (void)hipEventSynchronize(e);
    fprintf(stderr, "[qh sweeps psi=%p alt=%p]", psi, psi_alt);
    for (size_t i = 0; i + 1 < tev.size(); ++i) {
      float ms = 0;
      (void)hipEventElapsedTime(&ms, tev[i], tev[i + 1]);
      fprintf(stderr, " %.3f", ms);
    }
    fprintf(stderr, " ms\n");
    for (hipEvent_t x : tev) (void)hipEventDestroy(x);
  }
  return QH_OK;
}

}
```

### qcc_amd/csrc/planner.h

```cpp
#pragma once
#include <sched.h>
#include <stdint.h>

#include <algorithm>
#include <atomic>
#include <cassert>
#include <cmath>
#include <cstdio>
#include <cstdlib>
#include <cstring>
#include <exception>
#include <new>
#include <string>
#include <thread>
#include <vector>

#include "../../include/qcc_hip.h"

namespace qh {

struct GateRec {
  uint64_t ctl_mask;
  int tgt;
  double g[8];
  uint64_t neg_mask = 0;
  uint8_t ghost = 0, variant = 0;
  uint8_t force_dense = 0;
};

inline bool is_diag(const double g[8]) {
  return g[2] == 0.0 && g[3] == 0.0 && g[4] == 0.0 && g[5] == 0.0;
}
inline bool is_one(double re, double im) { return re == 1.0 && im == 0.0; }
inline bool plan_diag(const double g[8], int tgt) {
  return is_diag(g) && (tgt < 0 || !(g[0] == 0.0 && g[1] == 0.0));
}
inline bool plan_diag(const GateRec &r) { return !r.force_dense && plan_diag(r.g, r.tgt); }

constexpr int kLaneBits = 6;
constexpr int kLaneLow = 3;
constexpr int kLaneHi = 3;
constexpr int kMaxLaneHiBit = 27;
constexpr int kMaxRegBits = 6;
inline int max_reg_bits(int bw) { return bw == 128 ? 5 : 6; }
constexpr int kMaxWaveBits = 2;
constexpr int kMaxSweepOps = 1024;
constexpr int kMaxInsertBits = 12;
constexpr int kMaxSlabBits = 3;

enum : uint32_t { OP_DENSE_REG = 0, OP_DENSE_LANE = 1, OP_DIAG = 2,
                  OP_LSWAP = 3,
                  OP_WSWAP = 4 };
enum : uint32_t { OPF_DEFER_C = 1, OPF_USE_C = 2, OPF_REAL = 4,
                  OPF_BFLY = 8, OPF_BFLY_SHIFT = 4,
                  OPF_LANE_DPP = 128, OPF_SWAP_RI = 256,
                  OPF_GHOST = 1024,
                  OPF_ROT_P = 2048, OPF_ROT_M = 4096 };

inline bool env_flag(const char *name, bool dflt) {
  const char *e = getenv(name);
  return e ? atoi(e) != 0 : dflt;
}

inline int env_int(const char *name, int dflt) {
  const char *e = getenv(name);
  return e ? atoi(e) : dflt;
}

struct PlanSwitches {
  bool wave_pinned = false;
  int wave_bits = 1;
  bool split_lanes = true;
  int max_rb = kMaxRegBits;
  bool bfly = true, propagate_x = true, defer_diag = true, rot_fuse = true;
  int lane_valu = 1, seats = 1;
  bool search = true, search_wb2 = true;
  bool steps_pinned = false; uint64_t steps = 0;
  int streams = 0;
  int only_wb = -1, pick = -1;
  int tiles_wb = 0;
  std::vector<std::vector<int>> tiles;
  bool threads = true, log = false, dag = false, verbose = false;

  static PlanSwitches from_env() {
    PlanSwitches w;
    if (const char *e = getenv("QH_WAVE_BITS")) { w.wave_pinned = true; w.wave_bits = std::max(0, std::min(kMaxWaveBits, atoi(e))); }
    w.split_lanes = env_flag("QH_SPLIT_LANES", true);
    w.max_rb = std::max(2, std::min(kMaxRegBits, env_int("QH_SWEEP_RB", kMaxRegBits)));
    w.bfly = env_flag("QH_BFLY", true), w.propagate_x = env_flag("QH_PROPAGATE_X", true);
    w.defer_diag = env_flag("QH_DEFER_DIAG", true), w.rot_fuse = env_flag("QH_ROT_FUSE", true);
    w.lane_valu = env_int("QH_LANE_VALU", 1), w.seats = env_int("QH_SEATS", 1);
    w.search = env_flag("QH_PLAN_SEARCH", true), w.search_wb2 = env_flag("QH_PLAN_SEARCH_WB2", true);
    if (const char *e = getenv("QH_PLAN_SEARCH_STEPS")) { w.steps_pinned = true; w.steps = strtoull(e, nullptr, 10); }
    if (const char *e = getenv("QH_PLAN_SEARCH_STREAMS")) w.streams = std::max(1, std::min(8, atoi(e)));
    w.only_wb = env_int("QH_PLAN_ONLY_WB", -1), w.pick = env_int("QH_PLAN_SEARCH_PICK", -1);
    if (const char *e = getenv("QH_PLAN_TILES")) {
      w.tiles.emplace_back();
      w.tiles_wb = atoi(e);
      const char *p = strchr(e, ':');
      for (p = p ? p + 1 : e; *p; ++p) {
        if (*p == ';') w.tiles.emplace_back();
        else if (*p != ',') { char *end = nullptr; w.tiles.back().push_back((int)strtol(p, &end, 10)); if (end == p) break; p = end - 1; }
      }
    }
    w.threads = env_flag("QH_PLAN_SEARCH_THREADS", true), w.log = env_flag("QH_PLAN_SEARCH_LOG", false);
    w.dag = env_flag("QH_PLAN_DAG", false), w.verbose = env_flag("QH_PLAN_VERBOSE", false);
    return w;
  }
  std::string key() const {
    char b[192];
    snprintf(b, sizeof b, "%d,%d;%d;%d;%d%d%d%d;%d;%d;%d%d;%d,%llu;%d;%d;%d;%d:", wave_pinned, wave_bits, split_lanes, max_rb, bfly,
             propagate_x, defer_diag, rot_fuse, lane_valu, seats, search, search_wb2, steps_pinned, (unsigned long long)steps, streams,
             only_wb, pick, tiles_wb);
    std::string s = b;
    for (const auto &t : tiles) {
      s += ';';
      for (int v : t) s += std::to_string(v) + ',';
    }
    return s;
  }
};

struct PlanRequest {
  int nloc, bw;
  uint64_t shard;
  bool relayout;
  bool keep_ghosts;
  PlanSwitches sw;
  std::string key() const {
    return std::to_string(nloc) + "," + std::to_string(bw) + "," + std::to_string(shard) + "," + std::to_string(relayout) +
           std::to_string(keep_ghosts) + ":" + sw.key();
  }
};

inline int butterfly_variant(const double *g) {
  const double cr = g[0], ci = g[1];
  if (cr == 0.0 && ci == 0.0) return -1;
  auto eq = [&](int k, double r, double i) { return g[2 * k] == r && g[2 * k + 1] == i; };
  if (eq(1, cr, ci) && eq(2, cr, ci) && eq(3, -cr, -ci)) return 0;
  if (eq(1, -cr, -ci) && eq(2, cr, ci) && eq(3, cr, ci)) return 1;
  if (eq(1, cr, ci) && eq(2, -cr, -ci) && eq(3, cr, ci)) return 2;
  if (eq(1, ci, -cr) && eq(2, ci, -cr) && eq(3, cr, ci)) return 3;
  if (eq(1, -ci, cr) && eq(2, -ci, cr) && eq(3, cr, ci)) return 4;
  return -1;
}

struct OTerm {
  uint64_t mask;
  double re, im;
};
constexpr uint32_t DG_LTAB = 1u;
constexpr uint32_t DG_LTAB_LDS = 2u;
constexpr uint32_t DG_BITFAC = 8u;
constexpr int kBitFacs = 4;
inline int bitfac_others(int rb, int j, int out[kBitFacs]) {
  int n = 0;
  for (int b = 0; b < rb && n < kBitFacs; ++b) if (b != j) out[n++] = b;
  return n;
}
struct DGroup {
  uint32_t lane_mask, reg_mask;
  uint32_t oterm_off, n_oterms;
  double re, im;
  uint32_t flags, ltab_off;
  uint32_t ntab, tab_shift;
  uint32_t tab_off[4];
};
struct SweepOp {
  uint32_t kind;
  uint32_t tb;
  uint32_t cm_reg;
  uint32_t n_groups;
  uint64_t cm_thread;
  uint32_t group_off;
  uint32_t flags;
  double g[8];
};

struct SweepPlan {
  int rb = 0;
  int regpos[kMaxRegBits] = {0};
  int regpos_store[kMaxRegBits] = {0};
  int lane_low = kLaneLow;
  int lanehi[kLaneHi] = {3, 4, 5};
  int nlanehi() const { return kLaneBits - lane_low; }
  int seat[kLaneBits] = {0, 1, 2, 3, 4, 5};
  int seat_store[kLaneBits] = {0, 1, 2, 3, 4, 5};
  int seat_dest[kLaneBits] = {0, 1, 2, 3, 4, 5};
  bool contiguous() const {
    for (int k = 0; k < nlanehi(); ++k) if (lanehi[k] != lane_low + k) return false;
    return true;
  }
  int nwave = 0;
  int wavepos[kMaxWaveBits] = {0};
  uint64_t fixed_ones = 0;
  uint64_t ntiles = 0;
  bool relayout = false;
  uint8_t dest_pos[64] = {0};
  int wavepos_store[kMaxWaveBits] = {0};
  int reg_dest[kMaxRegBits] = {6, 7, 8, 9, 10, 11};
  int wave_dest[kMaxWaveBits] = {11, 12};
  std::vector<SweepOp> ops;
  std::vector<DGroup> groups;
  std::vector<OTerm> oterms;
  std::vector<double> tables;
  std::vector<double> ltabs;
  int n_ltab = 0;
  uint64_t gates = 0;
  uint64_t alg_bytes = 0;
  uint64_t swept_bytes = 0;
};

struct PlanResult {
  std::vector<SweepPlan> sweeps;
  uint64_t noop_gates = 0;
  bool moved = false;
  uint8_t final_pos[64];
  PlanResult() { for (int p = 0; p < 64; ++p) final_pos[p] = (uint8_t)p; }
};

inline int popc(uint64_t x) { return __builtin_popcountll(x); }

inline uint64_t gate_alg_bytes(const GateRec &r, int nloc, uint64_t amp_bytes) {
  const uint64_t lm = (nloc >= 64) ? ~0ull : ((1ull << nloc) - 1);
  const int nc = popc(r.ctl_mask & lm);
  const bool diag = is_diag(r.g);
  uint64_t touched = 1ull << (nloc - nc);
  if (diag && r.tgt < nloc && is_one(r.g[0], r.g[1])) touched >>= 1;
  return touched * amp_bytes * 2;
}

constexpr int kMaxUnitSegs = 8;
inline int unit_segments(const SweepPlan &sp, int nloc, uint64_t *masks, int *shifts) {
  uint64_t tile = 0;
  for (int i = 0; i < kLaneBits; ++i) tile |= 1ull << sp.seat_store[i];
  for (int k = 0; k < sp.rb; ++k) tile |= 1ull << sp.regpos_store[k];
  for (int k = 0; k < sp.nwave; ++k) tile |= 1ull << sp.wavepos_store[k];
  const int tilebits = popc(tile);
  int nseg = 0, i = 0, last_shift = 1 << 20;
  for (int p = 0; p < nloc; ++p) {
    if ((tile >> p) & 1ull) continue;
    const int shift = ((int)sp.dest_pos[p] - tilebits) - i;
    if (shift != last_shift) {
      ++nseg;
      last_shift = shift;
      if (masks && nseg <= kMaxUnitSegs) { masks[nseg - 1] = 0; shifts[nseg - 1] = shift; }
    }
    if (masks && nseg <= kMaxUnitSegs) masks[nseg - 1] |= 1ull << i;
    ++i;
  }
  return nseg;
}

class Planner {
 public:
  struct PassRec { uint64_t dense_bits, diag_bits; uint32_t score; int tgt; };
  struct PassState { size_t idx = 0; uint64_t blocked_all = 0, blocked_diag = 0; size_t count = 0, score = 0; bool valid = false; };
  explicit Planner(const PlanRequest &rq, int wave_bits = -1)
      : nloc_(rq.nloc), shard_(rq.shard), amp_bytes_(rq.bw == 128 ? 16 : 8), split_lanes_(rq.sw.split_lanes),
        relayout_(rq.relayout), keep_ghosts_(rq.keep_ghosts), butterflies_(rq.sw.bfly),
        max_wave_(wave_bits >= 0 ? std::min(wave_bits, kMaxWaveBits) : rq.sw.wave_bits), propagate_x_(rq.sw.propagate_x),
        lane_valu_(rq.sw.lane_valu), defer_diag_(rq.sw.defer_diag), rot_fuse_(rq.sw.rot_fuse), seats_(rq.sw.seats) {
    rb_cap_ = std::min({rq.sw.max_rb, max_reg_bits(rq.bw), nloc_ - kLaneBits});
    lane_low_ = rq.bw == 128 ? 3 : 4;
    lane_hi_ = kLaneBits - lane_low_;
  }

  void prepare(const std::vector<GateRec> &queue, std::vector<GateRec> *pending_out, std::vector<uint64_t> *alg_out, uint64_t *noops) {
    struct { uint64_t noop_gates = 0; } out;
    std::vector<GateRec> pending;
    pending.reserve(queue.size());
    alg_override_.clear();
    const uint64_t lm = (1ull << nloc_) - 1;
    for (const auto &q : queue) {
      const uint64_t hi = q.ctl_mask >> nloc_;
      GateRec r = q;
      r.ctl_mask &= lm;
      r.variant = (hi != 0 || q.tgt >= nloc_) ? 1 : 0;
      r.ghost = ((shard_ & hi) != hi) ? 1 : 0;
      if (r.ghost && !keep_ghosts_) { out.noop_gates++; continue; }
      if (r.tgt >= nloc_) {
        const bool set = (shard_ >> (r.tgt - nloc_)) & 1ull;
        const double fr = set ? r.g[6] : r.g[0], fi = set ? r.g[7] : r.g[1];
        if (is_one(fr, fi)) r.ghost = 1;
        if (r.ghost && !keep_ghosts_) { out.noop_gates++; continue; }
        if (r.ctl_mask) {
          const int c = __builtin_ctzll(r.ctl_mask);
          r.ctl_mask &= ~(1ull << c);
          r.tgt = c;
          r.force_dense = ((r.g[0] == 0.0 && r.g[1] == 0.0) || (r.g[6] == 0.0 && r.g[7] == 0.0)) ? 1 : 0;
          r.g[0] = 1; r.g[1] = 0; r.g[6] = fr; r.g[7] = fi;
        } else {
          r.tgt = -1;
          r.g[0] = fr; r.g[1] = fi; r.g[6] = fr; r.g[7] = fi;
        }
        if (r.ghost) { r.g[0] = r.g[6] = 1; r.g[1] = r.g[7] = 0; }
        r.g[2] = r.g[3] = r.g[4] = r.g[5] = 0;
        if (r.ghost) out.noop_gates++;
        pending.push_back(r);
        alg_override_.push_back(r.ghost ? 0 : gate_alg_bytes(q, nloc_, amp_bytes_));
        continue;
      }
      if (!r.variant && is_diag(r.g) && is_one(r.g[0], r.g[1]) && is_one(r.g[6], r.g[7])) { out.noop_gates++; continue; }
      if (r.ghost) out.noop_gates++;
      pending.push_back(r);
      alg_override_.push_back(r.ghost ? 0 : gate_alg_bytes(r, nloc_, amp_bytes_));
    }
    std::vector<uint64_t> alg = alg_override_;
    std::vector<uint32_t> weight(pending.size(), 1);
    for (size_t i = 0; i < pending.size(); ++i) if (pending[i].ghost) weight[i] = 0;
    fuse_sleator_weinfurter(&pending, &alg, &weight);
    if (propagate_x_) propagate_x(&pending, &alg, &weight, &out.noop_gates);
    weight_.swap(weight);
    pending_out->swap(pending);
    alg_out->swap(alg);
    *noops = out.noop_gates;
  }

  void skeleton(const std::vector<GateRec> &queue, size_t *nsweeps, bool *far_tile, std::vector<uint64_t> *tiles_out = nullptr) {
    std::vector<GateRec> pending;
    std::vector<uint64_t> alg;
    uint64_t noops = 0;
    prepare(queue, &pending, &alg, &noops);
    *nsweeps = 0;
    *far_tile = false;
    const uint64_t always = (1ull << lane_low_) - 1;
    while (!pending.empty()) {
      std::vector<int> sel, lanehi, regs, waves;
      select_tile_bits(pending, &sel);
      assign_bits(sel, &lanehi, &regs, &waves);
      if (!relayout_ || *nsweeps == 0) {
        int far = 0;
        for (int b : lanehi) far += b >= 25;
        for (int b : regs) far += b >= 25;
        if (far >= 8) *far_tile = true;
      }
      std::vector<uint8_t> flags(pending.size(), 0);
      pass(pending, always | mask_of(lanehi) | mask_of(regs) | mask_of(waves), pending.size(), &flags);
      if (tiles_out) tiles_out->push_back(mask_of(sel));
      std::vector<GateRec> rest;
      for (size_t i = 0; i < pending.size(); ++i) if (!flags[i]) rest.push_back(pending[i]);
      if (rest.size() == pending.size()) rest.erase(rest.begin());
      pending.swap(rest);
      ++*nsweeps;
    }
  }

  void canonical_records(const std::vector<GateRec> &pending, std::vector<PassRec> *rec0, int back[64], uint64_t *movable) {
    const uint64_t always = (1ull << lane_low_) - 1;
    int canon[64], ncanon = lane_low_;
    for (int b = 0; b < 64; ++b) canon[b] = b < lane_low_ ? b : -1;
    auto canon_mask = [&](uint64_t m) {
      uint64_t o = 0;
      for (uint64_t t = m; t; t &= t - 1) {
        const int b = __builtin_ctzll(t);
        if (canon[b] < 0) canon[b] = ncanon++;
        o |= 1ull << canon[b];
      }
      return o;
    };
    rec0->resize(pending.size());
    uint64_t dense_used = 0;
    for (size_t i = 0; i < pending.size(); ++i) {
      const GateRec &r = pending[i];
// ... 39 lines not shown
  }
  std::string dag_json(const std::vector<GateRec> &queue) {
    std::vector<GateRec> pending;
    std::vector<uint64_t> alg;
    uint64_t noops = 0;
    prepare(queue, &pending, &alg, &noops);
    std::vector<PassRec> rec0;
    int back[64];
    uint64_t movable = 0;
    canonical_records(pending, &rec0, back, &movable);
    std::vector<int> node_bit;
    std::vector<std::vector<int>> succ, pred;
    build_dag(rec0, &node_bit, &succ, &pred);
    std::string o = "{\"line_bits\":" + std::to_string(lane_low_) + ",\"cap_per_wave_bits\":[" + std::to_string(lane_hi_ + rb_cap_) + "," +
                    std::to_string(lane_hi_ + rb_cap_ + 1) + "," + std::to_string(lane_hi_ + rb_cap_ + 2) + "],\"target_bit\":[";
    for (size_t g = 0; g < node_bit.size(); ++g) o += (g ? "," : "") + std::to_string(back[node_bit[g]]);
    o += "],\"edges\":[";
    bool first = true;
    for (size_t u = 0; u < succ.size(); ++u)
      for (int v : succ[u]) { o += (first ? "[" : ",[") + std::to_string(u) + "," + std::to_string(v) + "]"; first = false; }
    return o + "]}";
  }
  bool search_levels(const std::vector<GateRec> &queue, size_t K, uint64_t change_budget, uint64_t stream,
                     std::vector<std::vector<int>> *tiles_out, uint64_t *changes_used = nullptr) {
    if (changes_used) *changes_used = 0;
    if (K < 2 || K > 8) return false;
    std::vector<GateRec> pending;
    std::vector<uint64_t> alg;
    uint64_t noops = 0;
    prepare(queue, &pending, &alg, &noops);
    std::vector<PassRec> rec0;
    int back[64];
    uint64_t movable = 0;
    canonical_records(pending, &rec0, back, &movable);
    const uint64_t always = (1ull << lane_low_) - 1;
    const int cap = lane_hi_ + rb_cap_ + max_wave_;
    if ((size_t)popc(movable) > K * (size_t)cap) return false;
    std::vector<int> node_bit;
    std::vector<std::vector<int>> succ, pred;
    build_dag(rec0, &node_bit, &succ, &pred);
    const int ng = (int)node_bit.size();
    if (!ng) return false;
    std::vector<int> depth(ng, 0);
    int maxd = 0;
    for (int u = 0; u < ng; ++u) for (int v : succ[u]) { depth[v] = std::max(depth[v], depth[u] + 1); maxd = std::max(maxd, depth[v]); }
    std::vector<int> chain[64];
    for (int g = 0; g < ng; ++g) chain[node_bit[g]].push_back(g);
    std::vector<int8_t> L(ng);
    int occ[64][8], ntile[8];
    uint64_t changes = 0;
    auto set_level = [&](int g, int to) {
      const int q = node_bit[g], from = L[g];
      ++changes;
      if (!((always >> q) & 1)) {
        if (--occ[q][from] == 0) --ntile[from];
        if (occ[q][to]++ == 0) ++ntile[to];
      }
      L[g] = (int8_t)to;
    };
    auto init = [&]() {
      memset(occ, 0, sizeof occ);
      memset(ntile, 0, sizeof ntile);
      for (int g = 0; g < ng; ++g) {
        L[g] = (int8_t)std::min<int>((int)K - 1, depth[g] * (int)K / (maxd + 1));
        const int q = node_bit[g];
        if (!((always >> q) & 1) && occ[q][L[g]]++ == 0) ++ntile[L[g]];
      }
    };
    auto cost = [&](int *over) {
      long sq = 0;
      int o = 0;
      for (size_t s = 0; s < K; ++s) { sq += (long)ntile[s] * ntile[s]; if (ntile[s] > cap) o += ntile[s] - cap; }
      *over = o;
      return (long)o * 100000 + sq;
    };
    std::vector<int> stk;
    std::vector<std::pair<int, int8_t>> undo;
    auto move = [&](int g, bool down) {
      const int to = L[g] + (down ? -1 : 1);
      if (to < 0 || to >= (int)K) return false;
      stk.assign(1, g);
      undo.emplace_back(g, L[g]);
      set_level(g, to);
      while (!stk.empty()) {
        const int u = stk.back();
        stk.pop_back();
        for (int v : down ? pred[u] : succ[u])
          if (down ? L[v] > to : L[v] < to) { undo.emplace_back(v, L[v]); set_level(v, to); stk.push_back(v); }
      }
      return true;
    };
    auto revert = [&]() { for (size_t i = undo.size(); i-- > 0;) set_level(undo[i].first, undo[i].second); undo.clear(); };
    uint64_t rng = 0x9e3779b97f4a7c15ull * (2 * stream + 1);
    auto rnd = [&](uint32_t n) { rng ^= rng << 13; rng ^= rng >> 7; rng ^= rng << 17; return (uint32_t)((rng >> 11) % n); };
    constexpr long kRestart = 1500;
    constexpr int kTenure = 7;
    std::vector<long> tabu((size_t)ng * 2);
    std::vector<int> cands;
    bool found = false;
    for (long walk = 0; !found; ++walk) {
      init();
      std::fill(tabu.begin(), tabu.end(), -1);
      int over = 0, best_over = 0;
      long best_key = cost(&best_over);
      over = best_over;
      for (long it = 0; it < kRestart && over > 0; ++it) {
        if (++changes > change_budget) goto out;
        if (walk == 0 && it == 400 && best_over > 4) goto out;
        cands.clear();
        for (size_t s = 0; s < K; ++s) {
          if (ntile[s] <= cap) continue;
          for (uint64_t t = movable; t; t &= t - 1) {
            const int q = __builtin_ctzll(t);
            if (!occ[q][s]) continue;
            int first = -1, last = -1;
            for (int g : chain[q]) if (L[g] == (int8_t)s) { if (first < 0) first = g; last = g; }
            cands.push_back(first * 2);
            cands.push_back(last * 2 + 1);
          }
        }
        long bk = 1L << 60;
        int bm = -1, ties = 0;
        for (int m : cands) {
          undo.clear();
          if (!move(m >> 1, m & 1)) continue;
          int o = 0;
          const long k = cost(&o);
          revert();
          if (tabu[m] > it && !(o < best_over)) continue;
          if (k < bk) { bk = k; bm = m; ties = 1; }
          else if (k == bk && rnd((uint32_t)++ties) == 0) bm = m;
        }
        if (bm < 0) continue;
        undo.clear();
        move(bm >> 1, bm & 1);
        const long k = cost(&over);
        for (const auto &u : undo) tabu[(size_t)u.first * 2 + ((bm & 1) ? 0 : 1)] = it + kTenure + (long)rnd(kTenure);
        if (k < best_key) { best_key = k; best_over = over; }
      }
      found = over == 0;
    }
  out:
    if (changes_used) *changes_used = changes;
    if (!found) return false;
    tiles_out->clear();
    for (size_t s = 0; s < K; ++s) {
      std::vector<int> b;
      for (uint64_t t = movable; t; t &= t - 1) if (occ[__builtin_ctzll(t)][s]) b.push_back(back[__builtin_ctzll(t)]);
      std::sort(b.begin(), b.end());
      tiles_out->push_back(b);
    }
    return true;
  }
  void set_tiles(const std::vector<std::vector<int>> &t) { tiles_ = t; }

  PlanResult plan(const std::vector<GateRec> &queue) {
    PlanResult out;
    std::vector<GateRec> pending;
    std::vector<uint64_t> alg;
    prepare(queue, &pending, &alg, &out.noop_gates);
    const uint64_t lm = (1ull << nloc_) - 1;
    std::vector<int> first_tile;
    keep_line_bits_ = !tiles_.empty();
    while (!pending.empty()) {
      std::vector<GateRec> rest;
      std::vector<uint64_t> rest_alg;
      std::vector<uint32_t> rest_w;
      std::vector<int> forced;
      const std::vector<int> *fs = nullptr;
      if (out.sweeps.size() < tiles_.size()) {
        for (int b : tiles_[out.sweeps.size()])
          if (b >= lane_low_ && b < nloc_) forced.push_back(out.final_pos[b]);
        fs = &forced;
      }
      out.sweeps.push_back(build_sweep(pending, alg, &rest, &rest_alg, &rest_w, fs));
      if (out.sweeps.size() == 1) {
        const SweepPlan &f = out.sweeps[0];
        for (int k = 0; k < f.nlanehi(); ++k) first_tile.push_back(f.lanehi[k]);
        for (int k = 0; k < f.rb; ++k) first_tile.push_back(f.regpos[k]);
        for (int k = 0; k < f.nwave; ++k) first_tile.push_back(f.wavepos[k]);
      }
      if (out.sweeps.back().relayout) {
        std::vector<int> ahead;
        if (!rest.empty() && out.sweeps.size() < tiles_.size()) {
          for (int b : tiles_[out.sweeps.size()])
            if (b >= lane_low_ && b < nloc_) ahead.push_back(out.final_pos[b]);
        } else if (!rest.empty()) {
          select_tile_bits(rest, &ahead);
        } else if (out.sweeps.size() > 1) {
          for (int p : first_tile) ahead.push_back(out.final_pos[p]);
        }
        std::sort(ahead.begin(), ahead.end());
        finish_relayout(&out.sweeps.back(), ahead);
        if (unit_segments(out.sweeps.back(), nloc_, nullptr, nullptr) > kMaxUnitSegs)
          finish_relayout(&out.sweeps.back(), std::vector<int>());
      }
      const SweepPlan &done = out.sweeps.back();
      if (done.relayout) {
        auto map_mask = [&](uint64_t m) {
          uint64_t o = m >> nloc_ << nloc_;
          for (uint64_t t = m & lm; t; t &= t - 1) o |= 1ull << done.dest_pos[__builtin_ctzll(t)];
          return o;
        };
        for (GateRec &r : rest) {
          r.ctl_mask = map_mask(r.ctl_mask);
          r.neg_mask = map_mask(r.neg_mask);
          if (r.tgt >= 0 && r.tgt < nloc_) r.tgt = done.dest_pos[r.tgt];
        }
        for (int p = 0; p < nloc_; ++p) out.final_pos[p] = done.dest_pos[out.final_pos[p]];
        out.moved = true;
      }
      pending.swap(rest);
      alg.swap(rest_alg);
      weight_.swap(rest_w);
    }
    return out;
  }

 private:
  int nloc_;
  uint64_t shard_;
  uint64_t amp_bytes_;
  int rb_cap_;
  int lane_low_ = kLaneLow, lane_hi_ = kLaneHi;
  bool split_lanes_;
  bool relayout_;
  bool keep_ghosts_;
  bool butterflies_;
  static constexpr size_t dense_weight_ = 1;
  int max_wave_;
  bool propagate_x_;
  static constexpr bool store_swapped_ = true, lanes_by_count_ = true, lanes_high_ = true, bitfac_ = true, fold_sink_ = true;
  static constexpr int min_table_terms_ = 2;
  bool fold_pending_ = false;
  bool keep_line_bits_ = false;
  double fold_re_ = 1, fold_im_ = 0;
  int lane_valu_;
  bool defer_diag_;
  static constexpr bool lookahead_ = true, reorder_ = true, lswap_early_ = true;
  bool rot_fuse_;
  int seats_;
  std::vector<uint64_t> alg_override_;
  std::vector<uint32_t> weight_;
  std::vector<std::vector<int>> tiles_;

  static bool near(double a, double b) { return std::fabs(a - b) <= 4e-15; }
  static bool same_gate(const double a[8], const double b[8]) {
    for (int i = 0; i < 8; ++i) if (!near(a[i], b[i])) return false;
    return true;
  }
  static bool is_x(const double g[8]) {
    const double x[8] = {0, 0, 1, 0, 1, 0, 0, 0};
    for (int i = 0; i < 8; ++i) if (g[i] != x[i]) return false;
    return true;
  }
  void propagate_x(std::vector<GateRec> *pending, std::vector<uint64_t> *alg, std::vector<uint32_t> *weight,
                   uint64_t *noops) const {
    std::vector<GateRec> out;
    std::vector<uint64_t> oalg;
    std::vector<uint32_t> ow;
    uint64_t flip = 0, carry_alg = 0;
    uint32_t carry_w = 0;
    auto emit_x = [&](int bit) {
      GateRec x{};
      x.ctl_mask = 0;
      x.tgt = bit;
      x.g[2] = 1.0; x.g[4] = 1.0;
      out.push_back(x);
      oalg.push_back(carry_alg);
      ow.push_back(carry_w);
      carry_alg = 0;
      carry_w = 0;
    };
    for (size_t i = 0; i < pending->size(); ++i) {
      GateRec r = (*pending)[i];
      if (r.tgt >= 0 && r.ctl_mask == 0 && r.neg_mask == 0 && is_x(r.g) && !r.variant) {
        flip ^= 1ull << r.tgt;
        carry_alg += (*alg)[i];
        carry_w += (*weight)[i];
        continue;
      }
      if (r.tgt >= 0 && ((flip >> r.tgt) & 1ull)) {
        for (int k = 0; k < 2; ++k) {
          std::swap(r.g[k], r.g[6 + k]);
          std::swap(r.g[2 + k], r.g[4 + k]);
        }
      }
      uint64_t c = (r.ctl_mask | r.neg_mask) & flip;
      const bool singular = r.variant || (r.g[0] == 0.0 && r.g[1] == 0.0) || (r.g[6] == 0.0 && r.g[7] == 0.0);
      if (plan_diag(r) && c && (singular || popc((r.neg_mask ^ c) & (r.ctl_mask | r.neg_mask)) > 3)) {
        for (uint64_t t = c; t; t &= t - 1) {
          const int b = __builtin_ctzll(t);
          emit_x(b);
          flip &= ~(1ull << b);
        }
        c = 0;
      }
      const uint64_t to_neg = r.ctl_mask & c, to_pos = r.neg_mask & c;
      r.ctl_mask = (r.ctl_mask & ~to_neg) | to_pos;
      r.neg_mask = (r.neg_mask & ~to_pos) | to_neg;
      out.push_back(r);
      oalg.push_back((*alg)[i] + carry_alg);
      ow.push_back((*weight)[i] + carry_w);
      carry_alg = 0;
      carry_w = 0;
    }
    for (uint64_t t = flip; t; t &= t - 1) emit_x(__builtin_ctzll(t));
    if (carry_w) {
      if (!ow.empty()) { ow.back() += carry_w; oalg.back() += carry_alg; }
      else *noops += carry_w;
    }
    pending->swap(out);
    alg->swap(oalg);
    weight->swap(ow);
  }

  static void mat2(const double a[8], const double b[8], double out[8]) {
    for (int r = 0; r < 2; ++r)
      for (int c = 0; c < 2; ++c) {
        double re = 0, im = 0;
        for (int k = 0; k < 2; ++k) {
          const double ar = a[2 * (2 * r + k)], ai = a[2 * (2 * r + k) + 1];
          const double br = b[2 * (2 * k + c)], bi = b[2 * (2 * k + c) + 1];
          re += ar * br - ai * bi;
          im += ar * bi + ai * br;
        }
        out[2 * (2 * r + c)] = re;
        out[2 * (2 * r + c) + 1] = im;
      }
  }

  void fuse_sleator_weinfurter(std::vector<GateRec> *pending, std::vector<uint64_t> *alg,
                               std::vector<uint32_t> *weight) const {
    std::vector<GateRec> out;
    std::vector<uint64_t> oalg;
    std::vector<uint32_t> ow;
    const std::vector<GateRec> &q = *pending;
    size_t i = 0;
    while (i < q.size()) {
      bool fused = false;
      if (i + 4 < q.size()) {
        const GateRec &g1 = q[i], &g2 = q[i + 1], &g3 = q[i + 2], &g4 = q[i + 3], &g5 = q[i + 4];
        const int t = g1.tgt, b = g2.tgt;
        const bool any_variant = g1.variant || g2.variant || g3.variant || g4.variant || g5.variant;
        if (!any_variant && t >= 0 && b >= 0 && b != t && g3.tgt == t && g5.tgt == t && g4.tgt == b && is_x(g2.g) &&
            is_x(g4.g) && g2.ctl_mask == g4.ctl_mask && g1.ctl_mask == g2.ctl_mask &&
            g3.ctl_mask == g5.ctl_mask && !((g1.ctl_mask >> b) & 1ull) && ((g3.ctl_mask >> b) & 1ull)) {
          const uint64_t common = g3.ctl_mask & ~(1ull << b);
          const uint64_t a_mask = g1.ctl_mask & ~common;
          if ((g1.ctl_mask & common) == common && popc(a_mask) == 1 && same_gate(g1.g, g5.g)) {
            double prod[8];
            mat2(g3.g, g1.g, prod);
            const double id[8] = {1, 0, 0, 0, 0, 0, 1, 0};
            if (same_gate(prod, id)) {
              GateRec r = g1;
              r.ctl_mask = g1.ctl_mask | (1ull << b);
              mat2(g1.g, g1.g, r.g);
              for (int k = 0; k < 8; ++k) {
                if (std::fabs(r.g[k]) < 4e-16) r.g[k] = 0.0;
                if (near(r.g[k], 1.0)) r.g[k] = 1.0;
                if (near(r.g[k], -1.0)) r.g[k] = -1.0;
              }
              out.push_back(r);
              oalg.push_back((*alg)[i] + (*alg)[i + 1] + (*alg)[i + 2] + (*alg)[i + 3] + (*alg)[i + 4]);
              ow.push_back(5);
              i += 5;
              fused = true;
// ... 875 lines not shown
        g.re = groups[uniform].re; g.im = groups[uniform].im;
        attach_outside(g, groups[uniform]);
        done[uniform] = true;
      }
      sp->groups.push_back(g);
    }
    for (size_t i = 0; i < groups.size(); ++i) {
      if (done[i]) continue;
      PGroup &pg = groups[i];
      DGroup g{};
      g.lane_mask = pg.lane; g.reg_mask = pg.reg; g.re = pg.re; g.im = pg.im;
      attach_outside(g, pg);
      sp->groups.push_back(g);
    }
    if (fold_pending_) {
      DGroup *host = nullptr;
      bool c_part = false;
      for (size_t k = op.group_off; k < sp->groups.size(); ++k) {
        DGroup &g = sp->groups[k];
        if (g.reg_mask) continue;
        c_part = true;
        if (!host && ((g.flags & DG_LTAB) || g.lane_mask == 0)) host = &g;
      }
      if (host) {
        cmul_acc(&host->re, &host->im, fold_re_, fold_im_);
        fold_pending_ = false;
      } else if (c_part) {
        DGroup g{};
        g.re = fold_re_; g.im = fold_im_;
        sp->groups.push_back(g);
        fold_pending_ = false;
      }
    }
    fuse_bit_factors(sp, op.group_off, geom.rb);
    op.n_groups = (uint32_t)(sp->groups.size() - op.group_off);
    sp->ops.push_back(op);
  }

  void fuse_bit_factors(SweepPlan *sp, uint32_t first, int rb) const {
    if (!bitfac_) return;
    auto scalar2 = [](const DGroup &g) {
      return g.lane_mask == 0 && g.flags == 0 && g.ntab == 0 && g.n_oterms == 0 && popc(g.reg_mask) == 2;
    };
    int best_j = -1, best_n = 0;
    for (int j = 0; j < rb; ++j) {
      int others[kBitFacs];
      const int no = bitfac_others(rb, j, others);
      int n = 0;
      for (size_t k = first; k < sp->groups.size(); ++k) {
        const DGroup &g = sp->groups[k];
        if (!scalar2(g) || !(g.reg_mask >> j & 1)) continue;
        const int i = __builtin_ctz(g.reg_mask & ~(1u << j));
        for (int t = 0; t < no; ++t) n += others[t] == i;
      }
      if (n > best_n) { best_n = n; best_j = j; }
    }
    if (best_j < 0) return;
    int base = -1;
    for (size_t k = first; k < sp->groups.size(); ++k)
      if (sp->groups[k].reg_mask == (1u << best_j) && sp->groups[k].ntab <= 3) { base = (int)k; break; }
    if (best_n < (base >= 0 ? 2 : 3)) return;
    int others[kBitFacs];
    const int no = bitfac_others(rb, best_j, others);
    double w[2 * kBitFacs] = {1, 0, 1, 0, 1, 0, 1, 0};
    std::vector<DGroup> kept;
    const int base_abs = base;
    for (size_t k = first; k < sp->groups.size(); ++k) {
      const DGroup &g = sp->groups[k];
      int slot = -1;
      if (scalar2(g) && (g.reg_mask >> best_j & 1)) {
        const int i = __builtin_ctz(g.reg_mask & ~(1u << best_j));
        for (int t = 0; t < no; ++t) if (others[t] == i) slot = t;
      }
      if (slot < 0) { kept.push_back(g); continue; }
      cmul_acc(&w[2 * slot], &w[2 * slot + 1], g.re, g.im);
      if ((int)k < base_abs) base--;
    }
    if (base < 0) {
      DGroup g{};
      g.reg_mask = 1u << best_j;
      g.re = 1; g.im = 0;
      kept.push_back(g);
      base = (int)kept.size() - 1;
    } else {
      base -= (int)first;
    }
    kept[base].flags |= DG_BITFAC;
    kept[base].tab_off[3] = (uint32_t)(sp->tables.size() / 2);
    for (double x : w) sp->tables.push_back(x);
    sp->groups.resize(first);
    for (const DGroup &g : kept) sp->groups.push_back(g);
  }
};

inline bool plan_has_far_tile(const PlanResult &pr) {
  for (const SweepPlan &sp : pr.sweeps) {
    int far = 0;
    for (int k = 0; k < sp.nlanehi(); ++k) far += sp.lanehi[k] >= 25;
    for (int k = 0; k < sp.rb; ++k) far += sp.regpos[k] >= 25;
    if (far >= 8) return true;
  }
  return false;
}

inline double sweep_op_energy_nj(const SweepPlan &sp) {
  const double nr = (double)(1u << sp.rb);
  double e = 0;
  for (const SweepOp &op : sp.ops) {
    const uint32_t f = op.flags;
    if (f & OPF_GHOST) continue;
    switch (op.kind) {
      case OP_DENSE_REG:
        if ((f & OPF_BFLY) && (f & (OPF_ROT_P | OPF_ROT_M))) e += 3 * nr * 1.58;
        else if (f & OPF_BFLY) e += 2 * nr * 1.5;
        else if (f & OPF_REAL) e += 5 * nr * 1.9;
        else e += (10 * nr + 10) * 1.95;
        break;
      case OP_DENSE_LANE:
        if ((f & OPF_LANE_DPP) && (f & OPF_BFLY)) e += (nr * (op.tb == 2 ? 10 : 6) + 14) * 1.0;
        else if (f & OPF_LANE_DPP) e += (nr * (op.tb == 2 ? 12 : 8) + 20) * 1.1;
        else if (f & OPF_BFLY) e += (2 * nr + 8) * 1.5 + 4 * nr * 1.0;
        else e += (((f & OPF_REAL) ? 4 : 10) * nr + 30) * 1.9 + 4 * nr * 1.0;
        break;
      case OP_LSWAP: e += (2 * nr + 8) * 1.2; break;
      case OP_WSWAP: e += 5 * 1.0 + 2 * nr * 1.0; break;
      case OP_DIAG: {
        bool c_touched = false, c_sign = false;
        for (uint32_t gi = 0; gi < op.n_groups; ++gi) {
          const DGroup &g = sp.groups[op.group_off + gi];
          const double slots = nr / (double)(1u << popc((uint64_t)g.reg_mask));
          const bool general = (g.flags & DG_LTAB) || g.ntab || g.n_oterms;
          const bool sign = g.re == -1.0 && g.im == 0.0 && !(g.flags & DG_LTAB) && !g.ntab;
          if (g.flags & DG_BITFAC) { e += (124 + ((g.lane_mask || general) ? 11 : 0)) * 1.95; continue; }
          if (sign) {
            if (!g.reg_mask) { e += 6 * 1.0; c_touched = c_sign = true; }
            else e += (4 + 2 * slots) * 1.0;
            continue;
          }
          double pro = 0;
          if (general) pro = 4 + 4 * g.ntab + 4 * g.n_oterms + ((g.flags & DG_LTAB) ? 4 : 7);
          else if (g.lane_mask) pro = 11;
          if (!g.reg_mask) { e += (pro + 4) * 1.9; c_touched = true; c_sign = false; }
          else e += 4 * slots * 1.95 + pro * 1.0;
        }
        if (c_touched && !(f & OPF_DEFER_C)) e += (c_sign ? (2 * nr + 1) : 4 * nr) * 1.95;
        break;
      }
      default: break;
    }
  }
  return e;
}

inline double plan_predicted_ms(const PlanResult &pr, int nloc, int bw) {
  double ms = 0;
  for (const SweepPlan &sp : pr.sweeps) {
    const double scale = (double)sp.swept_bytes / (2.0 * 16.0 * (double)(1ull << 30));
    const double e_ops_j = sweep_op_energy_nj(sp) * (double)sp.ntiles * 1e-9;
    const double floor_ms = (sp.nwave >= 2 ? 6.0 : 5.5) * scale;
    ms += std::max(floor_ms, 3.0 * scale + 0.99 * e_ops_j) + (sp.nwave >= 2 ? 0.3 * scale : 0.0);
  }
  (void)nloc; (void)bw;
  return ms;
}

inline unsigned usable_cpus() {
  unsigned n = std::thread::hardware_concurrency();
  cpu_set_t set;
  if (sched_getaffinity(0, sizeof set, &set) == 0) { const int c = CPU_COUNT(&set); if (c > 0 && (!n || (unsigned)c < n)) n = (unsigned)c; }
  for (const char *path : {"/sys/fs/cgroup/cpu.max", "/sys/fs/cgroup/cpu/cpu.cfs_quota_us"}) {
    FILE *f = fopen(path, "r");
    if (!f) continue;
    long long quota = -1, period = 100000;
    char word[32] = {0};
    if (fscanf(f, "%31s %lld", word, &period) >= 1 && strcmp(word, "max") != 0) quota = atoll(word);
    fclose(f);
    if (strstr(path, "cfs_quota")) {
      period = 100000;
      if (FILE *g = fopen("/sys/fs/cgroup/cpu/cpu.cfs_period_us", "r")) { if (fscanf(g, "%lld", &period) != 1) period = 100000; fclose(g); }
    }
    if (quota > 0 && period > 0) { const unsigned q = (unsigned)std::max<long long>(1, quota / period); if (!n || q < n) n = q; }
    break;
  }
  return n;
}

inline PlanResult plan_best(const std::vector<GateRec> &queue, const PlanRequest &rq) {
  const PlanSwitches &sw = rq.sw;
  const int nloc = rq.nloc, bw = rq.bw;
  const bool keep_ghosts = rq.keep_ghosts;
  if (sw.wave_pinned) return Planner(rq).plan(queue);
  if (!sw.tiles.empty()) {
    Planner forced(rq, sw.tiles_wb);
    forced.set_tiles(sw.tiles);
    return forced.plan(queue);
  }
  int best_wb = 1;
  size_t best_n = 0, n_of[kMaxWaveBits + 1] = {0, 0, 0};
  bool have = false, best_far = false, far_of[kMaxWaveBits + 1] = {false, false, false};
  const int only_wb = sw.only_wb;
  for (int wb : {1, 2, 0}) {
    if (only_wb >= 0 && wb != only_wb) continue;
    size_t n = 0;
    bool far = false;
    Planner(rq, wb).skeleton(queue, &n, &far);
    n_of[wb] = n;
    far_of[wb] = far;
    if (!have || (best_far && !far) || (best_far == far && n < best_n)) {
      best_wb = wb;
      best_n = n;
      best_far = far;
      have = true;
    }
    if (best_n <= 1 && !best_far) break;
  }
  Planner chosen(rq, best_wb);
  uint64_t dense_bits = 0;
  for (const GateRec &q : queue) if (q.tgt >= 0 && q.tgt < nloc && !plan_diag(q.g, q.tgt)) dense_bits |= 1ull << q.tgt;
  const int lane_low = bw == 128 ? 3 : 4;
  const int cap0 = (kLaneBits - lane_low) + std::min({sw.max_rb, max_reg_bits(bw), nloc - kLaneBits});
  if (best_n >= 3 && sw.search) {
    const double sweep_us = 2.0 * (double)(bw == 128 ? 16 : 8) * (double)(1ull << nloc) / 5.5e6;
    const uint64_t budget = sw.steps_pinned ? sw.steps : std::min<uint64_t>((uint64_t)(sweep_us * 640.0), 5000000);
    struct Task {
      int wb;
      size_t K;
      uint64_t stream, used = 0;
      bool ok = false, planned = false;
      double ms = 0;
      PlanResult pr;
      std::exception_ptr failed;
    };
    std::vector<Task> tasks;
    const size_t nmovable = (size_t)popc(dense_bits >> lane_low);
    std::vector<std::pair<int, size_t>> shapes;
    for (int wb : {1, 2, 0}) {
      if (budget < 5000) break;
      if (wb != best_wb && (wb == 0 || far_of[wb] || n_of[wb] == 0 || best_n < 4 || (wb == 2 && !sw.search_wb2))) continue;
      if (only_wb >= 0 && wb != only_wb) continue;
      const size_t cap = (size_t)(cap0 + wb), greedy = n_of[wb];
      const size_t kmin = std::max<size_t>({2, (nmovable + cap - 1) / cap, greedy > 3 ? greedy - 3 : 0});
      for (size_t K = kmin; K + 1 <= greedy && K <= best_n && K <= 8; ++K) shapes.emplace_back(wb, K);
    }
    int streams = 6;
    if (const unsigned hw = usable_cpus(); hw && !keep_ghosts && !shapes.empty())
      streams = std::max(1, std::min(6, (int)(hw / shapes.size())));
    if (sw.streams) streams = sw.streams;
    for (const auto &sh : shapes)
      for (int s = 0; s < streams; ++s) { tasks.emplace_back(); tasks.back().wb = sh.first; tasks.back().K = sh.second; tasks.back().stream = (uint64_t)(s + 1); }
    auto run = [&](Task &t) {
      const size_t i = (size_t)(&t - &tasks[0]);
      try {
        std::vector<std::vector<int>> tiles;
        t.ok = Planner(rq, t.wb).search_levels(queue, t.K, budget, t.stream, &tiles, &t.used);
        if (!t.ok) return;
        Planner forced(rq, t.wb);
        forced.set_tiles(tiles);
        t.pr = forced.plan(queue);
        t.planned = t.pr.sweeps.size() <= t.K && !plan_has_far_tile(t.pr);
      } catch (...) { t.failed = std::current_exception(); return; }
      if (t.planned) t.ms = keep_ghosts ? 1000.0 * (double)t.pr.sweeps.size() + 1e-3 * (double)(i + 1) : plan_predicted_ms(t.pr, nloc, bw);
    };
    std::atomic<size_t> next{0};
    auto drain = [&] { for (size_t i; (i = next++) < tasks.size(); ) run(tasks[i]); };
    std::vector<std::thread> pool;
    const size_t workers = sw.threads ? std::min<size_t>(tasks.size(), usable_cpus()) : 0;
    try { while (pool.size() < workers) pool.emplace_back(drain); } catch (...) {}
    PlanResult greedy_plan;
    std::exception_ptr greedy_failed;
    try { greedy_plan = chosen.plan(queue); } catch (...) { greedy_failed = std::current_exception(); next = tasks.size(); }
    drain();
    for (std::thread &x : pool) x.join();
    if (greedy_failed) std::rethrow_exception(greedy_failed);
    const Task *win = nullptr;
    double best_ms = keep_ghosts ? 1000.0 * (double)greedy_plan.sweeps.size() : plan_predicted_ms(greedy_plan, nloc, bw);
    for (const Task &t : tasks)
      if (t.planned && t.pr.sweeps.size() <= greedy_plan.sweeps.size() && t.ms < best_ms) { win = &t; best_ms = t.ms; }
    if (sw.pick >= 0) {
      if ((size_t)sw.pick < tasks.size() && tasks[sw.pick].planned) win = &tasks[sw.pick];
    }
    if (sw.log) {
      for (const Task &t : tasks)
        fprintf(stderr, "[qh plan search]   task %d: wave bits %d K=%zu stream %llu: %s after %llu label changes%s\n", (int)(&t - &tasks[0]), t.wb, t.K, (unsigned long long)t.stream,
                t.failed ? "FAILED (exception)" : t.ok ? "found" : "not found", (unsigned long long)t.used,
                t.planned ? (", " + std::to_string(t.pr.sweeps.size()) + " sweeps, predicted " + std::to_string(t.ms) + " ms").c_str() : "");
      fprintf(stderr, "[qh plan search] greedy: %d wave bit(s), %zu sweeps, predicted %.2f ms; chosen: %s (%zu tasks, budget %llu label changes each)\n", best_wb,
              greedy_plan.sweeps.size(), plan_predicted_ms(greedy_plan, nloc, bw),
              win ? (std::to_string(win->pr.sweeps.size()) + " sweeps with " + std::to_string(win->wb) + " wave bit(s), predicted " + std::to_string(win->ms) + " ms").c_str() : "greedy",
              tasks.size(), (unsigned long long)budget);
    }
    if (keep_ghosts)
      for (const Task &t : tasks) if (t.failed) std::rethrow_exception(t.failed);
    if (win) return win->pr;
    return greedy_plan;
  }
  return chosen.plan(queue);
}

template <class F> int guard_planning(std::string *err, F &&f) {
  try { f(); } catch (const std::bad_alloc &) { *err = "planning: out of host memory"; return QH_ERR_NOMEM; }
  catch (const std::exception &e) { *err = std::string("planning: ") + e.what(); return QH_ERR_ARG; }
  return QH_OK;
}

inline std::string plan_to_json(const std::vector<GateRec> &queue, const PlanRequest &rq) {
  if (rq.nloc < kLaneBits + 2) return "{\"sweeps\":[],\"note\":\"state too small for sweeps\"}";
  PlanResult pr = plan_best(queue, rq);
  std::string s = "{\"noop_gates\":" + std::to_string(pr.noop_gates);
  if (rq.sw.dag)
    s += ",\"dag\":" + Planner(rq, 1).dag_json(queue);
  s += ",\"sweeps\":[";
  char buf[384];
  for (size_t i = 0; i < pr.sweeps.size(); ++i) {
    const SweepPlan &sp = pr.sweeps[i];
    int nd = 0, ndiag = 0, nbf = 0;
    int nswap = 0, ndpp = 0;
    for (auto &o : sp.ops) {
      if (o.kind == OP_LSWAP || o.kind == OP_WSWAP) { nswap++; continue; }
      (o.kind == OP_DIAG ? ndiag : nd)++;
      if (o.flags & OPF_BFLY) nbf++;
      if (o.flags & OPF_LANE_DPP) ndpp++;
    }
    std::string rp = "[";
    for (int k = 0; k < sp.rb; ++k) rp += (k ? "," : "") + std::to_string(sp.regpos[k]);
    rp += "],\"lanehi\":[";
    for (int k = 0; k < sp.nlanehi(); ++k) rp += (k ? "," : "") + std::to_string(sp.lanehi[k]);
    rp += "],\"wavepos\":[";
    for (int k = 0; k < sp.nwave; ++k) rp += (k ? "," : "") + std::to_string(sp.wavepos[k]);
    rp += "]";
    rp += sp.relayout ? ",\"relayout\":1" : ",\"relayout\":0";
    snprintf(buf, sizeof buf,
             "%s{\"gates\":%llu,\"dense_ops\":%d,\"butterfly_ops\":%d,\"dpp_ops\":%d,\"lswap_ops\":%d,\"diag_ops\":%d,\"groups\":%zu,\"oterms\":%zu,\"table_entries\":%zu,"
             "\"regpos\":%s,\"fixed_ones\":%llu,\"ntiles\":%llu,\"alg_bytes\":%llu,\"swept_bytes\":%llu}",
             i ? "," : "", (unsigned long long)sp.gates, nd, nbf, ndpp, nswap, ndiag, sp.groups.size(), sp.oterms.size(),
             sp.tables.size() / 2, rp.c_str(), (unsigned long long)sp.fixed_ones, (unsigned long long)sp.ntiles,
             (unsigned long long)sp.alg_bytes, (unsigned long long)sp.swept_bytes);
    s += buf;
    if (rq.sw.verbose) {
      s.pop_back();
      s += ",\"ops\":[";
      for (size_t k = 0; k < sp.ops.size(); ++k) {
        const SweepOp &o = sp.ops[k];
        snprintf(buf, sizeof buf, "%s{\"kind\":%u,\"tb\":%u,\"flags\":%u,\"cm_reg\":%u,\"cm_thread\":%llu,\"groups\":[",
                 k ? "," : "", o.kind, o.tb, o.flags, o.cm_reg, (unsigned long long)o.cm_thread);
        s += buf;
        for (uint32_t gi = 0; o.kind == OP_DIAG && gi < o.n_groups; ++gi) {
          const DGroup &g = sp.groups[o.group_off + gi];
          snprintf(buf, sizeof buf, "%s[%u,%u,%u,%u,%u,%.17g,%.17g]", gi ? "," : "", g.lane_mask, g.reg_mask, g.flags, g.ntab, g.n_oterms, g.re, g.im);
          s += buf;
        }
        s += "]}";
      }
      s += "]}";
    }
  }
  s += "]}";
  return s;
}

}
```

### qcc_amd/device.py

```python
import ctypes

import numpy as np

from qcc_amd import gates as _gates
from qcc_amd import native

_dp = ctypes.POINTER(ctypes.c_double)
MAX_MARGINAL_BITS = 16


def _g8(gate):
  g = _gates.as8(gate)
  return g, g.ctypes.data_as(_dp)


def merge_factors(factors, table_bits=12, max_factors=32):
  out = []
  for n, x in factors:
    n = int(n)
    if n == 0:
      continue
    is_int = isinstance(x, (int, np.integer))
    if out:
      pn, px = out[-1]
# ... 282 lines not shown
    u = np.ascontiguousarray(u, dtype=np.float64).reshape(-1)
    out = np.zeros(u.size, dtype=np.uint64)
    native.check(self.lib.qh_sample(self.h, int(u.size), u.ctypes.data_as(_dp),
                                    out.ctypes.data_as(ctypes.POINTER(ctypes.c_uint64))))
    return out

  def expect_pauli(self, xmasks, zmasks):
    x = np.ascontiguousarray([int(v) for v in xmasks], dtype=np.uint64)
    z = np.ascontiguousarray([int(v) for v in zmasks], dtype=np.uint64)
    if x.size != z.size:
      raise ValueError(f'expect_pauli: {x.size} x masks, {z.size} z masks')
    out = np.zeros(x.size, dtype=np.float64)
    u64p = ctypes.POINTER(ctypes.c_uint64)
    native.check(self.lib.qh_expect_pauli(self.h, int(x.size), x.ctypes.data_as(u64p), z.ctypes.data_as(u64p),
                                          out.ctypes.data_as(_dp)))
    return out

  @staticmethod
  def _entries(buf, count):
    if not count:
      return np.zeros(0, dtype=np.uint64), np.zeros(0, dtype=np.complex128)
    rec = np.frombuffer(buf, dtype=np.dtype([('index', np.uint64), ('re', np.float64), ('im', np.float64)]), count=count)
    amp = np.empty(count, dtype=np.complex128)
    amp.real, amp.imag = rec['re'], rec['im']
    return rec['index'].copy(), amp

  def select(self, threshold, cap=1 << 16):
    cap = int(cap)
    buf = (native.QhEntry * cap)() if cap else None
    n, w = ctypes.c_uint64(), ctypes.c_double()
    native.check(self.lib.qh_select(self.h, float(threshold), cap, buf, ctypes.byref(n), ctypes.byref(w)))
    idx, amp = self._entries(buf, n.value if n.value <= cap else 0)
    return idx, amp, int(n.value), float(w.value)

  def topk(self, k):
    k = int(k)
    buf = (native.QhEntry * k)() if k else None
    n = ctypes.c_uint64()
    native.check(self.lib.qh_topk(self.h, k, buf, ctypes.byref(n)))
    return self._entries(buf, n.value)

  def amplitudes(self, indices, nlocal=False):
    idx = np.ascontiguousarray(indices, dtype=np.uint64).reshape(-1)
    out = np.zeros(idx.size, dtype=np.complex128)
    n = ctypes.c_uint64()
    native.check(self.lib.qh_amplitudes(self.h, int(idx.size), idx.ctypes.data_as(ctypes.POINTER(ctypes.c_uint64)),
                                        out.ctypes.data_as(_dp), ctypes.byref(n)))
    return (out, int(n.value)) if nlocal else out

  def clone(self):
    h = ctypes.c_void_p()
    native.check(self.lib.qh_clone(self.h, ctypes.byref(h)))
    other = object.__new__(DeviceState)
    other.lib, other.nbits, other.bit_width, other.dtype = self.lib, self.nbits, self.bit_width, self.dtype
    other.h, other.nbits_global = h, self.nbits_global
    return other

  def _sibling(self, call, nbits_delta):
    h = ctypes.c_void_p()
    rc = call(ctypes.byref(h))
    if rc == native.QH_ERR_NOMEM:
      from qcc_amd.lib import backend
      backend.drop_device_pool()
      rc = call(ctypes.byref(h))
    native.check(rc)
    other = object.__new__(DeviceState)
    other.lib, other.bit_width, other.dtype, other.h = self.lib, self.bit_width, self.dtype, h
    other.nbits, other.nbits_global = self.nbits + nbits_delta, self.nbits_global + nbits_delta
    return other

  def extend(self, nqubits, amps=None, basis=0):
    k = int(nqubits)
    tab = None
    if amps is not None:
      tab = np.ascontiguousarray(amps, dtype=np.complex128).reshape(-1)
      if not 1 <= k <= 16 or tab.size != 1 << k:
        raise ValueError(f'extend: {tab.size} amplitudes for {k} qubits')
    ptr = tab.ctypes.data_as(_dp) if tab is not None else None
    return self._sibling(lambda out: self.lib.qh_extend(self.h, k, ptr, int(basis), out), k)

  def release(self, bits, value=0):
    b = np.ascontiguousarray([int(x) for x in bits], dtype=np.int32)
    w = (ctypes.c_double * 2)()
    bp = b.ctypes.data_as(ctypes.POINTER(ctypes.c_int32))
    new = self._sibling(lambda out: self.lib.qh_release(self.h, int(b.size), bp, int(value), w, out), -int(b.size))
    return new, float(w[0]), float(w[1])

  def copy_from(self, other):
    native.check(self.lib.qh_copy(self.h, other.h))

  def inner(self, other):
    out = (ctypes.c_double * 2)()
    native.check(self.lib.qh_inner(self.h, other.h, out))
    return complex(out[0], out[1])

  def axpby(self, alpha, other, beta, norm=False):
    a, b = complex(alpha), complex(beta)
    out = ctypes.c_double() if norm else None
    native.check(self.lib.qh_axpby(self.h, (ctypes.c_double * 2)(a.real, a.imag), other.h, (ctypes.c_double * 2)(b.real, b.imag),
                                   ctypes.byref(out) if norm else None))
    return out.value if norm else None

  def inner_plan(self, other):
    t = native.QhInnerTiles()
    native.check(self.lib.qh_inner_plan(self.h, other.h, ctypes.byref(t)))
    return t.as_dict()

  def project_bits(self, mask, value):
    native.check(self.lib.qh_project_bits(self.h, int(mask), int(value)))

  def phys_to_logical(self, i):
    o = ctypes.c_uint64()
    native.check(self.lib.qh_phys_to_logical(self.h, int(i), ctypes.byref(o)))
    return o.value

  def logical_to_phys(self, i):
    o = ctypes.c_uint64()
    native.check(self.lib.qh_logical_to_phys(self.h, int(i), ctypes.byref(o)))
    return o.value

  def remap_swap(self, a, b):
    native.check(self.lib.qh_remap_swap(self.h, int(a), int(b)))

  def amplitude(self, logical_index):
    out = (ctypes.c_double * 2)()
    native.check(self.lib.qh_amplitude(self.h, int(logical_index), out))
    return self.dtype(complex(out[0], out[1]))

  def stats(self):
    s = native.QhStats()
    native.check(self.lib.qh_get_stats(self.h, ctypes.byref(s)))
    return s.as_dict()

  def reset_stats(self):
    native.check(self.lib.qh_reset_stats(self.h))

  def timer_begin(self):
    native.check(self.lib.qh_timer_begin(self.h))

  def timer_end(self):
    ms = ctypes.c_float()
    native.check(self.lib.qh_timer_end(self.h, ctypes.byref(ms)))
    return ms.value

  def timer_lap(self):
    native.check(self.lib.qh_timer_lap(self.h))

  def timer_laps(self, cap=4096):
    buf = (ctypes.c_float * cap)()
    n = ctypes.c_int(0)
    native.check(self.lib.qh_timer_laps(self.h, buf, cap, ctypes.byref(n)))
    return [float(buf[k]) for k in range(min(n.value, cap))]

  def plan_json(self):
    need = ctypes.c_uint64()
    native.check(self.lib.qh_plan_json(self.h, None, 0, ctypes.byref(need)))
    buf = ctypes.create_string_buffer(need.value)
    native.check(self.lib.qh_plan_json(self.h, buf, need.value, None))
    return buf.value.decode()


NO_CTL = -(2 ** 31)
```

### qcc_amd/native.py

```python
import ctypes
import os
import subprocess

PKG = os.path.dirname(os.path.abspath(__file__))
ROOT = os.path.dirname(PKG)
LIB_PATH = os.environ.get('QCC_HIP_LIB') or os.path.join(PKG, 'libqcc_hip.so')
SOURCES = [os.path.join(PKG, 'csrc', f) for f in
           ('engine.hip', 'buffers.hip.h', 'kernels_gate.hip.h', 'kernels_dense.hip.h', 'kernels_mux.hip.h', 'kernels_measure.hip.h', 'kernels_select.hip.h', 'select_plan.h', 'kernels_expect.hip.h', 'kernels_inner.hip.h', 'kernels_axpby.hip.h', 'inner_plan.h', 'kernels_resize.hip.h', 'resize_plan.h', 'kernels_sweep.hip.h', 'planner.h', 'exchange.hip.h', 'exchange_plan.h',
            'sweep_island_rb2.inc', 'sweep_island_rb3.inc', 'sweep_island_rb4.inc',
            'sweep_island_rb5.inc', 'sweep_island_f32_rb2.inc', 'sweep_island_f32_rb3.inc',
            'sweep_island_f32_rb4.inc', 'sweep_island_f32_rb5.inc', 'sweep_island_f32_rb6.inc', 'sweep_handlers.inc',
            'libq_facade.cc')]
HEADERS = [os.path.join(ROOT, 'include', 'libq.h')]
HEADER = os.path.join(ROOT, 'include', 'qcc_hip.h')

QH_OK = 0
QH_ERR_BAD_QUBIT, QH_ERR_SAME_QUBIT, QH_ERR_BAD_DTYPE, QH_ERR_HIP = 1, 2, 3, 4
QH_ERR_ARG, QH_ERR_NOMEM, QH_ERR_NO_DEVICE, QH_ERR_NONLOCAL, QH_ERR_COMM = 5, 6, 7, 8, 9
QH_FUSE_OFF, QH_FUSE_SWEEP = 0, 1

_u64, _i32, _vp, _dp = ctypes.c_uint64, ctypes.c_int, ctypes.c_void_p, ctypes.POINTER(ctypes.c_double)


class QhStats(ctypes.Structure):
  _fields_ = [('gates_submitted', _u64), ('kernels_launched', _u64), ('sweeps', _u64),
              ('bytes_algorithmic', _u64), ('bytes_swept', _u64), ('gates_noop', _u64)]

  def as_dict(self):
    return {k: int(getattr(self, k)) for k, _ in self._fields_}


QH_INNER_LINEAR, QH_INNER_TILES, QH_INNER_GATHER = 0, 1, 2


class QhInnerTiles(ctypes.Structure):
  _u8 = ctypes.c_uint8
  _fields_ = [('path', ctypes.c_uint32), ('nrest', ctypes.c_uint32), ('free_a', _u64), ('free_b', _u64),
              ('tile_a', _u8 * 8), ('tile_b', _u8 * 8), ('shuffle', _u8 * 8), ('rest_a', _u8 * 56), ('rest_b', _u8 * 56),
              ('pos_b', _u8 * 64)]

  def as_dict(self):
    return {k: (int(getattr(self, k)) if isinstance(getattr(self, k), int) else list(getattr(self, k))) for k, _ in self._fields_}


QH_SELECT_MAX, QH_TOPK_MAX = 1 << 20, 4096


class QhEntry(ctypes.Structure):
  _fields_ = [('index', _u64), ('re', ctypes.c_double), ('im', ctypes.c_double)]


SIGNATURES = {
    'qh_last_error': (ctypes.c_char_p, []),
    'qh_version': (_i32, []),
    'qh_device_count': (_i32, [ctypes.POINTER(_i32)]),
    'qh_create': (_i32, [_i32, _i32, _i32, ctypes.POINTER(_vp)]),
    'qh_attach': (_i32, [_i32, _i32, _i32, _vp, _vp, ctypes.POINTER(_vp)]),
    'qh_create_dry': (_i32, [_i32, _i32, ctypes.POINTER(_vp)]),
    'qh_create_host_mapped': (_i32, [_i32, _i32, _i32, ctypes.POINTER(_vp)]),
    'qh_host_ptr': (_i32, [_vp, ctypes.POINTER(_vp)]),
    'qh_destroy': (_i32, [_vp]),
    'qh_set_shard': (_i32, [_vp, _i32, _u64]),
    'qh_device_ptr': (_i32, [_vp, ctypes.POINTER(_vp)]),
    'qh_stream': (_i32, [_vp, ctypes.POINTER(_vp)]),
    'qh_nbits': (_i32, [_vp, ctypes.POINTER(_i32), ctypes.POINTER(_i32)]),
    'qh_init_basis': (_i32, [_vp, _u64]),
    'qh_init_product': (_i32, [_vp, _i32, ctypes.POINTER(_i32), ctypes.POINTER(_vp), ctypes.POINTER(_u64)]),
    'qh_upload': (_i32, [_vp, _vp, _u64, _u64]),
    'qh_download': (_i32, [_vp, _vp, _u64, _u64]),
    'qh_apply1': (_i32, [_vp, _i32, _dp]),
    'qh_applyc': (_i32, [_vp, _i32, _i32, _dp]),
    'qh_apply_bits': (_i32, [_vp, _u64, _i32, _dp]),
    'qh_apply_matrix': (_i32, [_vp, _i32, ctypes.POINTER(ctypes.c_int32), _u64, _dp]),
    'qh_apply_mux': (_i32, [_vp, _i32, ctypes.POINTER(ctypes.c_int32), _i32, _dp]),
    'qh_apply_diag': (_i32, [_vp, _i32, ctypes.POINTER(ctypes.c_int32), _dp]),
    'qh_set_fusion': (_i32, [_vp, _i32]),
    'qh_set_relayout': (_i32, [_vp, _i32, ctypes.POINTER(_i32)]),
    'qh_apply_stream': (_i32, [_vp, _u64, ctypes.POINTER(ctypes.c_int32), _dp]),
    'qh_flush': (_i32, [_vp]),
    'qh_sync': (_i32, [_vp]),
    'qh_pending_gates': (_i32, [_vp, ctypes.POINTER(_u64)]),
    'qh_discard_pending': (_i32, [_vp]),
    'qh_remap_swap': (_i32, [_vp, _i32, _i32]),
    'qh_get_bitmap': (_i32, [_vp, ctypes.POINTER(ctypes.c_int32)]),
    'qh_phys_to_logical': (_i32, [_vp, _u64, ctypes.POINTER(_u64)]),
    'qh_logical_to_phys': (_i32, [_vp, _u64, ctypes.POINTER(_u64)]),
    'qh_norm2': (_i32, [_vp, _dp]),
    'qh_amplitude': (_i32, [_vp, _u64, _dp]),
    'qh_argmax': (_i32, [_vp, ctypes.POINTER(_u64), _dp]),
    'qh_prob_bit': (_i32, [_vp, _i32, _dp]),
    'qh_prob_bit_value': (_i32, [_vp, _i32, _i32, _dp]),
    'qh_scale': (_i32, [_vp, ctypes.c_double, ctypes.c_double]),
    'qh_project_bit': (_i32, [_vp, _i32, _i32]),
    'qh_marginal': (_i32, [_vp, _i32, ctypes.POINTER(ctypes.c_int32), _dp]),
    'qh_sample': (_i32, [_vp, _u64, _dp, ctypes.POINTER(ctypes.c_uint64)]),
    'qh_project_bits': (_i32, [_vp, _u64, _u64]),
    'qh_expect_pauli': (_i32, [_vp, _u64, ctypes.POINTER(_u64), ctypes.POINTER(_u64), _dp]),
    'qh_select': (_i32, [_vp, ctypes.c_double, _u64, ctypes.POINTER(QhEntry), ctypes.POINTER(_u64), _dp]),
    'qh_topk': (_i32, [_vp, _u64, ctypes.POINTER(QhEntry), ctypes.POINTER(_u64)]),
    'qh_amplitudes': (_i32, [_vp, _u64, ctypes.POINTER(_u64), _dp, ctypes.POINTER(_u64)]),
    'qh_clone': (_i32, [_vp, ctypes.POINTER(_vp)]),
    'qh_copy': (_i32, [_vp, _vp]),
    'qh_inner': (_i32, [_vp, _vp, _dp]),
    'qh_inner_plan': (_i32, [_vp, _vp, ctypes.POINTER(QhInnerTiles)]),
    'qh_axpby': (_i32, [_vp, _dp, _vp, _dp, _dp]),
    'qh_extend': (_i32, [_vp, _i32, _dp, _u64, ctypes.POINTER(_vp)]),
    'qh_release': (_i32, [_vp, _i32, ctypes.POINTER(ctypes.c_int32), _u64, _dp, ctypes.POINTER(_vp)]),
    'qh_get_stats': (_i32, [_vp, ctypes.POINTER(QhStats)]),
    'qh_reset_stats': (_i32, [_vp]),
    'qh_timer_begin': (_i32, [_vp]),
    'qh_timer_end': (_i32, [_vp, ctypes.POINTER(ctypes.c_float)]),
    'qh_timer_lap': (_i32, [_vp]),
    'qh_timer_laps': (_i32, [_vp, ctypes.POINTER(ctypes.c_float), _i32, ctypes.POINTER(_i32)]),
    'qh_plan_json': (_i32, [_vp, ctypes.c_char_p, _u64, ctypes.POINTER(_u64)]),
    'qh_plan_export': (_i32, [_vp, _vp, _u64, ctypes.POINTER(_u64)]),
    'qh_plan_handlers': (_i32, [_vp, _vp, _u64, ctypes.POINTER(_u64)]),
    'qh_host_apply1': (_i32, [_vp, _dp, _i32, _i32, _i32]),
    'qh_host_applyc': (_i32, [_vp, _dp, _i32, _i32, _i32, _i32]),
    'qh_host_release': (_i32, []),
}


class QhXStats(ctypes.Structure):
  _fields_ = [('exchanges', _u64), ('rounds', _u64), ('bytes_sent', _u64), ('slabs', _u64),
              ('sweeps_overlapped', _u64), ('span_ms', ctypes.c_double), ('rounds_packed', _u64),
              ('geometry_checks', _u64), ('comm_ranks', ctypes.c_uint32), ('comm_rank', ctypes.c_uint32)]

  def as_dict(self):
    return {k: getattr(self, k) for k, _ in self._fields_}


class QhXGeom(ctypes.Structure):
  _fields_ = [('signature', _u64), ('slab_mask', _u64), ('block_bits', _u64), ('rounds_per_slab', _u64), ('staging_bytes', _u64),
              ('slabs', ctypes.c_uint32), ('chunk_bits', ctypes.c_uint32), ('packed', ctypes.c_uint32), ('peers', ctypes.c_uint32),
              ('sweeps_before', ctypes.c_uint32), ('last_sweep_split', ctypes.c_uint32)]

  def as_dict(self):
    return {k: int(getattr(self, k)) for k, _ in self._fields_}


ROUND_FN = ctypes.CFUNCTYPE(ctypes.c_int, _vp, ctypes.c_int, ctypes.POINTER(ctypes.c_int), ctypes.POINTER(_vp),
                            ctypes.POINTER(_vp), _u64)

SIGNATURES.update({
    'qh_comm_unique_id': (_i32, [_vp]),
    'qh_comm_init': (_i32, [_vp, _i32, _i32, _vp]),
    'qh_comm_init_custom': (_i32, [_vp, _i32, _i32, ROUND_FN, _vp]),
    'qh_comm_init_dry': (_i32, [_vp, _i32, _i32]),
    'qh_exchange_geometry': (_i32, [_vp, ctypes.POINTER(QhXGeom)]),
    'qh_comm_destroy': (_i32, [_vp]),
    'qh_exchange_alltoall': (_i32, [_vp, _i32, _u64]),
    'qh_exchange_pair': (_i32, [_vp, _i32, _i32, _u64]),
    'qh_exchange_loopback': (_i32, [_vp, _i32, _u64]),
    'qh_exchange_wait': (_i32, [_vp]),
    'qh_exchange_stats': (_i32, [_vp, ctypes.POINTER(QhXStats)]),
    'qh_comm_allreduce_sum': (_i32, [_vp, _dp, _i32]),
})


class QhError(RuntimeError):
  def __init__(self, code, msg):
    super().__init__(f'qcc_hip error {code}: {msg}')
    self.code = code


def build(force=False, verbose=False):
  deps = SOURCES + [HEADER] + HEADERS
  if (not force and os.path.exists(LIB_PATH)
      and all(os.path.getmtime(LIB_PATH) >= os.path.getmtime(d) for d in deps)):
    return LIB_PATH
  cmd = ['hipcc', '--offload-arch=gfx950', '-O3', '-std=c++17', '-shared', '-fPIC',
         '-o', LIB_PATH, SOURCES[0], SOURCES[-1]]
  if verbose:
    print(' '.join(cmd))
  subprocess.check_call(cmd, cwd=ROOT)
  return LIB_PATH


_lib = None


def _preload_torch_runtime():
  import sys
  if 'torch' in sys.modules:
    return
  if os.environ.get('WORLD_SIZE') or os.environ.get('QCC_PRELOAD_TORCH') == '1':
    import torch


def load():
  global _lib
  if _lib is not None:
    return _lib
  _preload_torch_runtime()
  if not os.path.exists(LIB_PATH):
    raise RuntimeError(
        f'{LIB_PATH} is missing: build it with `python -c "import __graft_entry__ as g; g.build()"` '
        '(hipcc --offload-arch=gfx950).  qcc_amd has no CPU fallback.')
  lib = ctypes.CDLL(LIB_PATH)
  for name, (res, args) in SIGNATURES.items():
    fn = getattr(lib, name)
    fn.restype, fn.argtypes = res, args
  _lib = lib
  return lib


def check(rc):
  if rc != QH_OK:
    raise QhError(rc, load().qh_last_error().decode(errors='replace'))


def device_count():
  n = _i32(0)
  load().qh_device_count(ctypes.byref(n))
  return n.value
```

Baseline: 28470 gate-applies/s.

## Stream sweep launches during planning and bound plan search when GPU idle

When the stream is idle, the greedy planner now hands each finished sweep to a sink that stages its parameters and launches it at once, so GPU work overlaps host planning. Idle plan search is pruned with dependency-cone bounds and its budget is capped by the predicted saving over the greedy plan. Shapes already at the lower bound get one search stream. Op buffers become per-sweep staged slices, and a plan_ms query is added. The risks are extra synchronisation when buffers fill and weaker plans from the shorter search.

```diff
diff --git a/include/qcc_hip.h b/include/qcc_hip.h
--- a/include/qcc_hip.h
+++ b/include/qcc_hip.h
@@ -164,6 +164,7 @@
 int qh_timer_lap(qh_handle h);
 int qh_timer_laps(qh_handle h, float *milliseconds, int cap, int *count);
 int qh_plan_json(qh_handle h, char *buf, uint64_t cap, uint64_t *needed);
+int qh_plan_ms(qh_handle h, double *milliseconds);
 
 int qh_plan_export(qh_handle h, void *buf, uint64_t cap, uint64_t *needed);
 
diff --git a/qcc_amd/csrc/engine.hip b/qcc_amd/csrc/engine.hip
--- a/qcc_amd/csrc/engine.hip
+++ b/qcc_amd/csrc/engine.hip
@@ -397,6 +397,11 @@
 qh::PlanRequest plan_request(const qh_state_s *h, bool relayout) {
   return qh::PlanRequest{h->nloc, h->bw, h->shard, relayout, h->nglob > h->nloc, qh::PlanSwitches::from_env()};
 }
+qh::PlanRequest plan_request_now(const qh_state_s *h) {
+  qh::PlanRequest rq = plan_request(h, relayout_wanted(h));
+  rq.idle = qh::plan_idle(rq, h->stream, h->dry, h->comm != nullptr);
+  return rq;
+}
 hipError_t alloc_state_buffer(void **p, size_t bytes) {
   static const int contig = env_int("QH_ALLOC_CONTIG", -1), debug = env_int("QH_ALLOC_DEBUG", 0);
   const auto t0 = std::chrono::steady_clock::now();
@@ -2527,7 +2532,7 @@
 int qh_plan_json(qh_handle h, char *buf, uint64_t cap, uint64_t *needed) {
   if (!h) return fail(QH_ERR_ARG, "null");
   std::string s;
-  if (int rc = qh::guard_planning(&g_err, [&] { s = qh::plan_to_json(h->queue, plan_request(h, relayout_wanted(h))); })) return rc;
+  if (int rc = qh::guard_planning(&g_err, [&] { s = qh::plan_to_json(h->queue, plan_request_now(h), &h->sweep.plan_ms); })) return rc;
   if (needed) *needed = s.size() + 1;
   if (buf && cap) {
     const uint64_t n = std::min<uint64_t>(cap - 1, s.size());
@@ -2537,11 +2542,17 @@
   return QH_OK;
 }
 
+int qh_plan_ms(qh_handle h, double *ms) {
+  if (!h || !ms) return fail(QH_ERR_ARG, "null");
+  *ms = h->sweep.plan_ms;
+  return QH_OK;
+}
+
 int qh_plan_export(qh_handle h, void *buf, uint64_t cap, uint64_t *needed) {
   if (!h) return fail(QH_ERR_ARG, "null");
   if (!qh::sweep_supported(h->nloc, h->bw)) return fail(QH_ERR_ARG, "state too small for sweeps");
   qh::PlanResult pr;
-  if (int rc = qh::guard_planning(&g_err, [&] { pr = qh::plan_best(h->queue, plan_request(h, relayout_wanted(h))); })) return rc;
+  if (int rc = qh::guard_planning(&g_err, [&] { pr = qh::plan_best(h->queue, plan_request_now(h)); })) return rc;
   std::vector<uint64_t> out;
   auto put_bytes = [&](const void *p, size_t n) {
     const size_t w = (n + 7) / 8, at = out.size();
@@ -2606,7 +2617,7 @@
   if (!h) return fail(QH_ERR_ARG, "null");
   if (!qh::sweep_supported(h->nloc, h->bw)) return fail(QH_ERR_ARG, "state too small for sweeps");
   qh::PlanResult pr;
-  if (int rc = qh::guard_planning(&g_err, [&] { pr = qh::plan_best(h->queue, plan_request(h, relayout_wanted(h))); })) return rc;
+  if (int rc = qh::guard_planning(&g_err, [&] { pr = qh::plan_best(h->queue, plan_request_now(h)); })) return rc;
   std::vector<uint32_t> out{0x51484831u, (uint32_t)pr.sweeps.size()};
   std::vector<qh::SweepOp> ops;
   std::vector<qh::DGroup> groups;
diff --git a/qcc_amd/csrc/kernels_sweep.hip.h b/qcc_amd/csrc/kernels_sweep.hip.h
--- a/qcc_amd/csrc/kernels_sweep.hip.h
+++ b/qcc_amd/csrc/kernels_sweep.hip.h
@@ -1,6 +1,7 @@
 #pragma once
 #include <hip/hip_runtime.h>
 
+#include <chrono>
 #include <string>
 #include <vector>
 
@@ -350,6 +351,7 @@
 struct SweepBuffers {
   std::deque<PlanCacheEntry> plans;
   StagedUpload<1> ops;
+  double plan_ms = 0;
 };
 
 inline bool sweep_supported(int nloc, int bw) { return (bw == 128 || bw == 64) && nloc >= kLaneBits + 2; }
@@ -525,129 +527,61 @@
   arr->clear();
 }
 
-inline int run_fused(const std::vector<GateRec> &queue, const PlanRequest &rq, void *psi, hipStream_t stream, bool dry,
+inline bool plan_idle(const PlanRequest &rq, hipStream_t stream, bool dry, bool sharded) {
+  if (sharded || rq.keep_ghosts) return false;
+  if (rq.sw.idle_pin >= 0) return rq.sw.idle_pin != 0;
+  if (dry) return true;
+  const hipError_t e = hipStreamQuery(stream);
+  if (e != hipSuccess) (void)hipGetLastError();
+  return e == hipSuccess;
+}
+
+inline int run_fused(const std::vector<GateRec> &queue, const PlanRequest &rq_in, void *psi, hipStream_t stream, bool dry,
                      SweepBuffers *bufs, qh_stats *stats, std::string *err, SlabIO *slab = nullptr, void *psi_alt = nullptr,
                      void **result = nullptr, uint8_t *final_pos = nullptr, TileMaxOut *tmax = nullptr) {
+  PlanRequest rq = rq_in;
+  rq.idle = plan_idle(rq_in, stream, dry, slab != nullptr);
   const int nloc = rq.nloc, bw = rq.bw;
   const uint64_t shard = rq.shard;
-  std::shared_ptr<const PlanResult> cached;
-  const int rc = guard_planning(err, [&] {
-    const std::string key = rq.key();
-    const bool use_cache = !getenv("QH_PLAN_CACHE") || atoi(getenv("QH_PLAN_CACHE")) != 0;
-    if (use_cache)
-      for (auto &e : bufs->plans)
-        if (e.key == key && same_queue(e.queue, queue)) { cached = e.plan; return; }
-    cached = std::make_shared<const PlanResult>(plan_best(queue, rq));
-    if (use_cache) {
-      bufs->plans.push_front(PlanCacheEntry{queue, key, cached});
-      if (bufs->plans.size() > 4) bufs->plans.pop_back();
-    }
-  });
-  if (rc) return rc;
-  const PlanResult &pr = *cached;
-  const int pace = dry ? 0 : flush_pace(pr, bw == 128, nloc);
-  stats->gates_noop += pr.noop_gates;
-  size_t n_ops = 0, n_groups = 0, n_ot = 0, n_tab = 0;
-  for (auto &sp : pr.sweeps) {
-    if (popc(sp.fixed_ones) + sp.rb + sp.nlanehi() + sp.nwave > kMaxIns) {
-      *err = "sweep needs more inserted bits than the tile enumeration supports";
-      return QH_ERR_ARG;
-    }
-    n_ops += sp.ops.size() + 1;
-    n_groups += sp.groups.size();
-    n_ot += sp.oterms.size();
-    n_tab += sp.tables.size();
-  }
-  const bool want_tmax = tmax && tmax->buf && !dry && !slab && !pr.sweeps.empty() && pr.sweeps.back().fixed_ones == 0 &&
-                         (pr.sweeps.back().ntiles >> pr.sweeps.back().nwave) <= tmax->cap;
+  const size_t amp = bw == 128 ? 16 : 8;
   if (tmax) tmax->valid = false;
-  const size_t bytes_prm = pr.sweeps.size() * sizeof(SweepParams);
-  const size_t bytes_ops = n_ops * sizeof(SweepOp), bytes_groups = n_groups * sizeof(DGroup),
-               bytes_ot = (n_ot * sizeof(OTerm) + 15) / 16 * 16, bytes_tab = n_tab * sizeof(double);
-  const size_t total = bytes_prm + bytes_ops + bytes_groups + bytes_ot + bytes_tab + 256;
-  std::vector<char> host_dry;
-  char *hbase = nullptr, *d_base = nullptr;
-  if (dry) {
-    host_dry.resize(total);
-    hbase = host_dry.data();
-  } else {
-    if (hipEvent_t e = bufs->ops.busy()) (void)hipEventSynchronize(e);
-    size_t cap = bufs->ops.host.cap;
-    if (cap < total) {
-      if (cap) (void)hipStreamSynchronize(stream);
-      cap = std::max<size_t>(total * 2, 1 << 20);
-    }
-    unsigned slot = 0;
-    const hipError_t e = bufs->ops.acquire(cap, &hbase, &d_base, &slot);
-    if (e != hipSuccess) {
-      *err = std::string("op buffers (pinned + device): ") + hipGetErrorString(e);
-      return e == hipErrorOutOfMemory ? QH_ERR_NOMEM : QH_ERR_HIP;
-    }
-  }
-  memset(hbase, 0, total);
-  char *h_prm = hbase, *h_ops = h_prm + bytes_prm, *h_groups = h_ops + bytes_ops,
-       *h_ot = h_groups + bytes_groups, *h_tab = h_ot + bytes_ot;
-  {
-    size_t io = 0, ig = 0, it = 0, is = 0, itab = 0;
-    for (auto &sp : pr.sweeps) {
-      SweepParams prm{};
-      prm.ops = (const SweepOp *)(d_base + bytes_prm) + io;
-      prm.groups = (const DGroup *)(d_base + bytes_prm + bytes_ops) + ig;
-      prm.oterms = (const OTerm *)(d_base + bytes_prm + bytes_ops + bytes_groups) + it;
-      prm.nops = (uint32_t)sp.ops.size();
-      prm.n_ltab_lds = (uint32_t)(bw == 128 ? ltab_lds_count<true>(sp) : ltab_lds_count<false>(sp));
-      prm.tables_rel = (uint32_t)((d_base + bytes_prm + bytes_ops + bytes_groups + bytes_ot + itab * sizeof(double)) -
-                                  (const char *)prm.groups);
-      for (int k = 0; k < 64; ++k) {
-        uint64_t o = 0;
-        for (int b = 0; b < sp.rb; ++b)
-          if ((k >> b) & 1) o |= 1ull << sp.regpos[b];
-        prm.slot_off[k] = o * (bw == 128 ? 16 : 8);
-        o = 0;
-        for (int b = 0; b < sp.rb; ++b)
-          if ((k >> b) & 1) o |= 1ull << (sp.relayout ? sp.reg_dest[b] : sp.regpos_store[b]);
-        prm.slot_off_store[k] = o * (bw == 128 ? 16 : 8);
-      }
-      prm.store_delta_mask = sp.relayout ? 0ull : ~0ull;
-      if (want_tmax && is + 1 == pr.sweeps.size()) prm.tilemax = (uint64_t)tmax->buf;
-      memcpy(h_prm + is * sizeof(SweepParams), &prm, sizeof prm);
-      build_device_copy(sp, bw, prm.n_ltab_lds, (SweepOp *)(h_ops + io * sizeof(SweepOp)), (DGroup *)(h_groups + ig * sizeof(DGroup)));
-      if (!sp.oterms.empty()) memcpy(h_ot + it * sizeof(OTerm), sp.oterms.data(), sp.oterms.size() * sizeof(OTerm));
-      if (!sp.tables.empty()) memcpy(h_tab + itab * sizeof(double), sp.tables.data(), sp.tables.size() * sizeof(double));
-      io += sp.ops.size() + 1; ig += sp.groups.size(); it += sp.oterms.size(); itab += sp.tables.size(); is++;
-    }
-  }
-  if (!dry) {
-    hipError_t e = hipMemcpyAsync(d_base, hbase, total, hipMemcpyHostToDevice, stream);
-    if (e == hipSuccess) e = bufs->ops.commit(stream, 0);
-    if (e != hipSuccess) {
-      *err = std::string("hipMemcpyAsync(op buffer): ") + hipGetErrorString(e);
-      return QH_ERR_HIP;
-    }
-  }
-#ifdef QH_PROF
-  static char *d_prof = nullptr;
-  const size_t prof_bytes = kProfRows * kProfRecs * 8;
-  if (!dry) {
-    if (!d_prof) (void)hipMalloc(&d_prof, prof_bytes * 16);
-    (void)hipMemsetAsync(d_prof, 0, prof_bytes * 16, stream);
-    for (size_t k = 0; k < pr.sweeps.size() && k < 16; ++k) {
-      const uint64_t v = (uint64_t)(d_prof + k * prof_bytes);
-      (void)hipMemcpyAsync(d_base + k * sizeof(SweepParams) + offsetof(SweepParams, prof_buf), &v, 8,
-                           hipMemcpyHostToDevice, stream);
-      (void)hipStreamSynchronize(stream);
-    }
-  }
-#endif
   if (result) *result = psi;
-  if (final_pos) memcpy(final_pos, pr.final_pos, 64);
   static const bool timing = env_flag("QH_SWEEP_TIMING", false);
   std::vector<hipEvent_t> tev;
   void *cur = psi, *other = psi_alt;
-  size_t is = 0;
+  int pace = 0;
   uint64_t avoid_cur = slab ? slab->avoid : 0;
   uint64_t earlier_tiles = 0;
-  for (auto &sp : pr.sweeps) {
+  auto wants_tmax = [&](const SweepPlan &last_sp) {
+    return tmax && tmax->buf && !dry && !slab && last_sp.fixed_ones == 0 && (last_sp.ntiles >> last_sp.nwave) <= tmax->cap;
+  };
+  auto stage = [&](const SweepPlan &sp, bool tmax_here, char *h_prm, char *h_ops, char *h_groups, char *h_ot, char *h_tab,
+                   const char *d_ops, const char *d_groups, const char *d_ot, const char *d_tab) {
+    SweepParams prm{};
+    prm.ops = (const SweepOp *)d_ops;
+    prm.groups = (const DGroup *)d_groups;
+    prm.oterms = (const OTerm *)d_ot;
+    prm.nops = (uint32_t)sp.ops.size();
+    prm.n_ltab_lds = (uint32_t)(bw == 128 ? ltab_lds_count<true>(sp) : ltab_lds_count<false>(sp));
+    prm.tables_rel = (uint32_t)(d_tab - (const char *)prm.groups);
+    for (int k = 0; k < 64; ++k) {
+      uint64_t o = 0;
+      for (int b = 0; b < sp.rb; ++b)
+        if ((k >> b) & 1) o |= 1ull << sp.regpos[b];
+      prm.slot_off[k] = o * amp;
+      o = 0;
+      for (int b = 0; b < sp.rb; ++b)
+        if ((k >> b) & 1) o |= 1ull << (sp.relayout ? sp.reg_dest[b] : sp.regpos_store[b]);
+      prm.slot_off_store[k] = o * amp;
+    }
+    prm.store_delta_mask = sp.relayout ? 0ull : ~0ull;
+    if (tmax_here) prm.tilemax = (uint64_t)tmax->buf;
+    memcpy(h_prm, &prm, sizeof prm);
+    build_device_copy(sp, bw, prm.n_ltab_lds, (SweepOp *)h_ops, (DGroup *)h_groups);
+    if (!sp.oterms.empty()) memcpy(h_ot, sp.oterms.data(), sp.oterms.size() * sizeof(OTerm));
+    if (!sp.tables.empty()) memcpy(h_tab, sp.tables.data(), sp.tables.size() * sizeof(double));
+  };
+  auto launch_one = [&](const SweepPlan &sp, bool first, bool last, const SweepParams *prm, const char *h_prm, bool tmax_here) -> int {
     auto moved = [&](uint64_t v) {
       if (!sp.relayout) return v;
       uint64_t o = v >> nloc << nloc;
@@ -658,10 +592,8 @@
       *err = "internal: a relayout sweep was planned without a second buffer";
       return QH_ERR_ARG;
     }
-    const SweepParams *prm = (const SweepParams *)d_base + is;
     SweepParams hprm;
-    memcpy(&hprm, h_prm + is * sizeof(SweepParams), sizeof hprm);
-    const bool first = is == 0, last = is + 1 == pr.sweeps.size();
+    memcpy(&hprm, h_prm, sizeof hprm);
     bool launched = false;
     if (slab) {
       if (first && slab->arrivals && !slab->arrivals->empty()) {
@@ -712,7 +644,7 @@
       (void)hipEventRecord(e, stream);
       tev.push_back(e);
     }
-    if (want_tmax && last) {
+    if (tmax_here) {
       tmax->nunits = sp.ntiles >> sp.nwave;
       if (hipMemsetAsync(tmax->buf, 0, tmax->nunits * 8, stream) != hipSuccess) { *err = "hipMemsetAsync(tile maxima)"; return QH_ERR_HIP; }
       uint64_t tm = 0;
@@ -735,11 +667,167 @@
     }
     avoid_cur = moved(avoid_cur);
     earlier_tiles = moved(earlier_tiles | (sweep_tile_bits(sp) & ~((1ull << kLaneBits) - 1)));
-    is++;
     stats->kernels_launched++;
     stats->sweeps++;
     stats->bytes_algorithmic += sp.alg_bytes;
     stats->bytes_swept += sp.swept_bytes;
+    return QH_OK;
+  };
+  const char *too_many_bits = "sweep needs more inserted bits than the tile enumeration supports";
+  size_t streamed = 0, stream_off = 0, stream_cap = 0;
+  int stream_rc = QH_OK;
+  double sink_ms = 0;
+  char *s_hbase = nullptr, *s_dbase = nullptr;
+  SweepSink sink = [&](const PlanResult &so_far, bool last) {
+    if (stream_rc) return;
+    const auto t0 = std::chrono::steady_clock::now();
+    stream_rc = [&]() -> int {
+      const SweepPlan &sp = so_far.sweeps.back();
+      if (popc(sp.fixed_ones) + sp.rb + sp.nlanehi() + sp.nwave > kMaxIns) { *err = too_many_bits; return QH_ERR_ARG; }
+      const size_t b_prm = (sizeof(SweepParams) + 15) / 16 * 16, b_ops = (sp.ops.size() + 1) * sizeof(SweepOp),
+                   b_groups = sp.groups.size() * sizeof(DGroup), b_ot = (sp.oterms.size() * sizeof(OTerm) + 15) / 16 * 16,
+                   b_tab = sp.tables.size() * sizeof(double);
+      const size_t bytes = (b_prm + b_ops + b_groups + b_ot + b_tab + 256 + 255) / 256 * 256;
+      if (!s_hbase || stream_off + bytes > stream_cap) {
+        if (!s_hbase) { if (hipEvent_t e = bufs->ops.busy()) (void)hipEventSynchronize(e); }
+        size_t cap = std::max<size_t>(bufs->ops.host.cap, 1 << 20);
+        if (s_hbase || cap < bytes) {
+          if (bufs->ops.host.cap) (void)hipStreamSynchronize(stream);
+          if (cap < 2 * bytes) cap = 2 * bytes;
+        }
+        unsigned slot = 0;
+        const hipError_t e = bufs->ops.acquire(cap, &s_hbase, &s_dbase, &slot);
+        if (e != hipSuccess) {
+          *err = std::string("op buffers (pinned + device): ") + hipGetErrorString(e);
+          return e == hipErrorOutOfMemory ? QH_ERR_NOMEM : QH_ERR_HIP;
+        }
+        stream_cap = cap;
+        stream_off = 0;
+      }
+      char *h = s_hbase + stream_off;
+      const char *d = s_dbase + stream_off;
+      memset(h, 0, bytes);
+      const bool tmax_here = last && wants_tmax(sp);
+      stage(sp, tmax_here, h, h + b_prm, h + b_prm + b_ops, h + b_prm + b_ops + b_groups, h + b_prm + b_ops + b_groups + b_ot,
+            d + b_prm, d + b_prm + b_ops, d + b_prm + b_ops + b_groups, d + b_prm + b_ops + b_groups + b_ot);
+      if (hipMemcpyAsync(s_dbase + stream_off, h, bytes, hipMemcpyHostToDevice, stream) != hipSuccess) {
+        *err = "hipMemcpyAsync(op buffer)";
+        return QH_ERR_HIP;
+      }
+      stream_off += bytes;
+      pace = flush_pace(so_far, bw == 128, nloc);
+      const int rc = launch_one(sp, streamed == 0, last, (const SweepParams *)d, h, tmax_here);
+      if (rc == QH_OK) ++streamed;
+      return rc;
+    }();
+    sink_ms += std::chrono::duration<double, std::milli>(std::chrono::steady_clock::now() - t0).count();
+  };
+#ifdef QH_PROF
+  const bool may_stream = false;
+#else
+  const bool may_stream = rq.idle && !dry && !slab;
+#endif
+  std::shared_ptr<const PlanResult> cached;
+  const auto plan_t0 = std::chrono::steady_clock::now();
+  const int rc = guard_planning(err, [&] {
+    const std::string key = rq.key();
+    const bool use_cache = !getenv("QH_PLAN_CACHE") || atoi(getenv("QH_PLAN_CACHE")) != 0;
+    if (use_cache)
+      for (auto &e : bufs->plans)
+        if (e.key == key && same_queue(e.queue, queue)) { cached = e.plan; return; }
+    cached = std::make_shared<const PlanResult>(plan_best(queue, rq, may_stream ? &sink : nullptr));
+    if (use_cache) {
+      bufs->plans.push_front(PlanCacheEntry{queue, key, cached});
+      if (bufs->plans.size() > 4) bufs->plans.pop_back();
+    }
+  });
+  bufs->plan_ms = std::chrono::duration<double, std::milli>(std::chrono::steady_clock::now() - plan_t0).count() - sink_ms;
+  if (s_hbase && bufs->ops.commit(stream, 0) != hipSuccess && !stream_rc) { *err = "hipEventRecord(op buffer)"; stream_rc = QH_ERR_HIP; }
+  if (rc) return rc;
+  if (stream_rc) return stream_rc;
+  const PlanResult &pr = *cached;
+  stats->gates_noop += pr.noop_gates;
+  if (final_pos) memcpy(final_pos, pr.final_pos, 64);
+#ifdef QH_PROF
+  static char *d_prof = nullptr;
+  const size_t prof_bytes = kProfRows * kProfRecs * 8;
+#endif
+  if (!streamed) {
+    pace = dry ? 0 : flush_pace(pr, bw == 128, nloc);
+    size_t n_ops = 0, n_groups = 0, n_ot = 0, n_tab = 0;
+    for (auto &sp : pr.sweeps) {
+      if (popc(sp.fixed_ones) + sp.rb + sp.nlanehi() + sp.nwave > kMaxIns) {
+        *err = too_many_bits;
+        return QH_ERR_ARG;
+      }
+      n_ops += sp.ops.size() + 1;
+      n_groups += sp.groups.size();
+      n_ot += sp.oterms.size();
+      n_tab += sp.tables.size();
+    }
+    const bool want_tmax = !pr.sweeps.empty() && wants_tmax(pr.sweeps.back());
+    const size_t bytes_prm = pr.sweeps.size() * sizeof(SweepParams);
+    const size_t bytes_ops = n_ops * sizeof(SweepOp), bytes_groups = n_groups * sizeof(DGroup),
+                 bytes_ot = (n_ot * sizeof(OTerm) + 15) / 16 * 16, bytes_tab = n_tab * sizeof(double);
+    const size_t total = bytes_prm + bytes_ops + bytes_groups + bytes_ot + bytes_tab + 256;
+    std::vector<char> host_dry;
+    char *hbase = nullptr, *d_base = nullptr;
+    if (dry) {
+      host_dry.resize(total);
+      hbase = host_dry.data();
+    } else {
+      if (hipEvent_t e = bufs->ops.busy()) (void)hipEventSynchronize(e);
+      size_t cap = bufs->ops.host.cap;
+      if (cap < total) {
+        if (cap) (void)hipStreamSynchronize(stream);
+        cap = std::max<size_t>(total * 2, 1 << 20);
+      }
+      unsigned slot = 0;
+      const hipError_t e = bufs->ops.acquire(cap, &hbase, &d_base, &slot);
+      if (e != hipSuccess) {
+        *err = std::string("op buffers (pinned + device): ") + hipGetErrorString(e);
+        return e == hipErrorOutOfMemory ? QH_ERR_NOMEM : QH_ERR_HIP;
+      }
+    }
+    memset(hbase, 0, total);
+    char *h_prm = hbase, *h_ops = h_prm + bytes_prm, *h_groups = h_ops + bytes_ops,
+         *h_ot = h_groups + bytes_groups, *h_tab = h_ot + bytes_ot;
+    {
+      size_t io = 0, ig = 0, it = 0, is = 0, itab = 0;
+      for (auto &sp : pr.sweeps) {
+        stage(sp, want_tmax && is + 1 == pr.sweeps.size(), h_prm + is * sizeof(SweepParams), h_ops + io * sizeof(SweepOp),
+              h_groups + ig * sizeof(DGroup), h_ot + it * sizeof(OTerm), h_tab + itab * sizeof(double),
+              d_base + bytes_prm + io * sizeof(SweepOp), d_base + bytes_prm + bytes_ops + ig * sizeof(DGroup),
+              d_base + bytes_prm + bytes_ops + bytes_groups + it * sizeof(OTerm),
+              d_base + bytes_prm + bytes_ops + bytes_groups + bytes_ot + itab * sizeof(double));
+        io += sp.ops.size() + 1; ig += sp.groups.size(); it += sp.oterms.size(); itab += sp.tables.size(); is++;
+      }
+    }
+    if (!dry) {
+      hipError_t e = hipMemcpyAsync(d_base, hbase, total, hipMemcpyHostToDevice, stream);
+      if (e == hipSuccess) e = bufs->ops.commit(stream, 0);
+      if (e != hipSuccess) {
+        *err = std::string("hipMemcpyAsync(op buffer): ") + hipGetErrorString(e);
+        return QH_ERR_HIP;
+      }
+    }
+#ifdef QH_PROF
+    if (!dry) {
+      if (!d_prof) (void)hipMalloc(&d_prof, prof_bytes * 16);
+      (void)hipMemsetAsync(d_prof, 0, prof_bytes * 16, stream);
+      for (size_t k = 0; k < pr.sweeps.size() && k < 16; ++k) {
+        const uint64_t v = (uint64_t)(d_prof + k * prof_bytes);
+        (void)hipMemcpyAsync(d_base + k * sizeof(SweepParams) + offsetof(SweepParams, prof_buf), &v, 8,
+                             hipMemcpyHostToDevice, stream);
+        (void)hipStreamSynchronize(stream);
+      }
+    }
+#endif
+    for (size_t is = 0; is < pr.sweeps.size(); ++is) {
+      const bool last = is + 1 == pr.sweeps.size();
+      const int lrc = launch_one(pr.sweeps[is], is == 0, last, (const SweepParams *)d_base + is, h_prm + is * sizeof(SweepParams), want_tmax && last);
+      if (lrc) return lrc;
+    }
   }
 #ifdef QH_PROF
   if (!dry && getenv("QH_PROF_OUT")) {
diff --git a/qcc_amd/csrc/planner.h b/qcc_amd/csrc/planner.h
--- a/qcc_amd/csrc/planner.h
+++ b/qcc_amd/csrc/planner.h
@@ -5,11 +5,13 @@
 #include <algorithm>
 #include <atomic>
 #include <cassert>
+#include <chrono>
 #include <cmath>
 #include <cstdio>
 #include <cstdlib>
 #include <cstring>
 #include <exception>
+#include <functional>
 #include <new>
 #include <string>
 #include <thread>
@@ -81,6 +83,7 @@
   int tiles_wb = 0;
   std::vector<std::vector<int>> tiles;
   bool threads = true, log = false, dag = false, verbose = false;
+  int idle_pin = -1;
 
   static PlanSwitches from_env() {
     PlanSwitches w;
@@ -105,6 +108,7 @@
     }
     w.threads = env_flag("QH_PLAN_SEARCH_THREADS", true), w.log = env_flag("QH_PLAN_SEARCH_LOG", false);
     w.dag = env_flag("QH_PLAN_DAG", false), w.verbose = env_flag("QH_PLAN_VERBOSE", false);
+    if (const char *e = getenv("QH_PLAN_IDLE")) w.idle_pin = atoi(e) != 0;
     return w;
   }
   std::string key() const {
@@ -127,9 +131,10 @@
   bool relayout;
   bool keep_ghosts;
   PlanSwitches sw;
+  bool idle = false;
   std::string key() const {
     return std::to_string(nloc) + "," + std::to_string(bw) + "," + std::to_string(shard) + "," + std::to_string(relayout) +
-           std::to_string(keep_ghosts) + ":" + sw.key();
+           std::to_string(keep_ghosts) + std::to_string(idle) + ":" + sw.key();
   }
 };
 
@@ -210,6 +215,9 @@
   uint64_t alg_bytes = 0;
   uint64_t swept_bytes = 0;
 };
+
+struct PlanResult;
+using SweepSink = std::function<void(const PlanResult &so_far, bool last)>;
 
 struct PlanResult {
   std::vector<SweepPlan> sweeps;
@@ -555,9 +563,50 @@
     }
     return true;
   }
+  size_t cone_bound(const std::vector<GateRec> &queue) {
+    std::vector<GateRec> pending;
+    std::vector<uint64_t> alg;
+    uint64_t noops = 0;
+    prepare(queue, &pending, &alg, &noops);
+    std::vector<PassRec> rec0;
+    int back[64];
+    uint64_t movable = 0;
+    canonical_records(pending, &rec0, back, &movable);
+    std::vector<int> node_bit;
+    std::vector<std::vector<int>> succ, pred;
+    build_dag(rec0, &node_bit, &succ, &pred);
+    const int cap = lane_hi_ + rb_cap_ + max_wave_;
+    constexpr int kLevels = 16;
+    struct Cone { int lb; uint64_t q[kLevels]; };
+    const size_t ng = node_bit.size();
+    auto walk = [&](const std::vector<std::vector<int>> &before, bool reverse, std::vector<int> *lb_out) {
+      std::vector<Cone> cone(ng);
+      for (size_t i = 0; i < ng; ++i) {
+        const size_t v = reverse ? ng - 1 - i : i;
+        Cone c{0, {0}};
+        for (int u : before[v]) {
+          c.lb = std::max(c.lb, cone[u].lb);
+          for (int l = 0; l <= cone[u].lb; ++l) c.q[l] |= cone[u].q[l];
+        }
+        const uint64_t qv = (1ull << node_bit[v]) & movable;
+        int lb = c.lb;
+        for (int l = 0; l <= c.lb; ++l) lb = std::max(lb, l - 1 + (popc(c.q[l] | qv) + cap - 1) / cap);
+        c.lb = std::min(lb, kLevels - 1);
+        for (int l = 0; l <= c.lb; ++l) c.q[l] |= qv;
+        cone[v] = c;
+        (*lb_out)[v] = c.lb;
+      }
+    };
+    std::vector<int> below(ng, 0), above(ng, 0);
+    walk(pred, false, &below);
+    walk(succ, true, &above);
+    size_t bound = 0;
+    for (size_t v = 0; v < ng; ++v) bound = std::max(bound, (size_t)(below[v] + above[v] + 1));
+    return bound;
+  }
   void set_tiles(const std::vector<std::vector<int>> &t) { tiles_ = t; }
 
-  PlanResult plan(const std::vector<GateRec> &queue) {
+  PlanResult plan(const std::vector<GateRec> &queue, const SweepSink *sink = nullptr) {
     PlanResult out;
     std::vector<GateRec> pending;
     std::vector<uint64_t> alg;
@@ -616,6 +665,7 @@
       pending.swap(rest);
       alg.swap(rest_alg);
       weight_.swap(rest_w);
+      if (sink) (*sink)(out, pending.empty());
     }
     return out;
   }
@@ -1797,12 +1847,13 @@
   return e;
 }
 
+inline double stream_floor_ms(int nwave) { return nwave >= 2 ? 6.0 : 5.5; }
 inline double plan_predicted_ms(const PlanResult &pr, int nloc, int bw) {
   double ms = 0;
   for (const SweepPlan &sp : pr.sweeps) {
     const double scale = (double)sp.swept_bytes / (2.0 * 16.0 * (double)(1ull << 30));
     const double e_ops_j = sweep_op_energy_nj(sp) * (double)sp.ntiles * 1e-9;
-    const double floor_ms = (sp.nwave >= 2 ? 6.0 : 5.5) * scale;
+    const double floor_ms = stream_floor_ms(sp.nwave) * scale;
     ms += std::max(floor_ms, 3.0 * scale + 0.99 * e_ops_j) + (sp.nwave >= 2 ? 0.3 * scale : 0.0);
   }
   (void)nloc; (void)bw;
@@ -1830,15 +1881,20 @@
   return n;
 }
 
-inline PlanResult plan_best(const std::vector<GateRec> &queue, const PlanRequest &rq) {
+constexpr double kSearchChangesPerMs = 75000.0;
+constexpr double kIdleSearchShare = 1.0 / 3.0;
+
+inline PlanResult plan_best(const std::vector<GateRec> &queue, const PlanRequest &rq, const SweepSink *sink = nullptr) {
   const PlanSwitches &sw = rq.sw;
   const int nloc = rq.nloc, bw = rq.bw;
   const bool keep_ghosts = rq.keep_ghosts;
-  if (sw.wave_pinned) return Planner(rq).plan(queue);
+  const bool idle = rq.idle && !keep_ghosts;
+  if (!idle) sink = nullptr;
+  if (sw.wave_pinned) return Planner(rq).plan(queue, sink);
   if (!sw.tiles.empty()) {
     Planner forced(rq, sw.tiles_wb);
     forced.set_tiles(sw.tiles);
-    return forced.plan(queue);
+    return forced.plan(queue, sink);
   }
   int best_wb = 1;
   size_t best_n = 0, n_of[kMaxWaveBits + 1] = {0, 0, 0};
@@ -1866,7 +1922,7 @@
   const int cap0 = (kLaneBits - lane_low) + std::min({sw.max_rb, max_reg_bits(bw), nloc - kLaneBits});
   if (best_n >= 3 && sw.search) {
     const double sweep_us = 2.0 * (double)(bw == 128 ? 16 : 8) * (double)(1ull << nloc) / 5.5e6;
-    const uint64_t budget = sw.steps_pinned ? sw.steps : std::min<uint64_t>((uint64_t)(sweep_us * 640.0), 5000000);
+    uint64_t budget = sw.steps_pinned ? sw.steps : std::min<uint64_t>((uint64_t)(sweep_us * 640.0), 5000000);
     struct Task {
       int wb;
       size_t K;
@@ -1880,19 +1936,45 @@
     const size_t nmovable = (size_t)popc(dense_bits >> lane_low);
     std::vector<std::pair<int, size_t>> shapes;
     for (int wb : {1, 2, 0}) {
-      if (budget < 5000) break;
+      if (!idle && budget < 5000) break;
       if (wb != best_wb && (wb == 0 || far_of[wb] || n_of[wb] == 0 || best_n < 4 || (wb == 2 && !sw.search_wb2))) continue;
       if (only_wb >= 0 && wb != only_wb) continue;
       const size_t cap = (size_t)(cap0 + wb), greedy = n_of[wb];
       const size_t kmin = std::max<size_t>({2, (nmovable + cap - 1) / cap, greedy > 3 ? greedy - 3 : 0});
       for (size_t K = kmin; K + 1 <= greedy && K <= best_n && K <= 8; ++K) shapes.emplace_back(wb, K);
     }
+    PlanResult greedy_plan;
+    if (idle) {
+      size_t cone_of[kMaxWaveBits + 1] = {0, 0, 0};
+      for (auto &sh : shapes) if (!cone_of[sh.first]) cone_of[sh.first] = Planner(rq, sh.first).cone_bound(queue);
+      shapes.erase(std::remove_if(shapes.begin(), shapes.end(), [&](const std::pair<int, size_t> &sh) { return sh.second < cone_of[sh.first]; }), shapes.end());
+      if (sw.log) fprintf(stderr, "[qh plan search] idle: dependency bounds %zu / %zu / %zu sweeps for 0 / 1 / 2 wave bits\n", cone_of[0], cone_of[1], cone_of[2]);
+      if (shapes.empty()) {
+        if (sw.log) fprintf(stderr, "[qh plan search] idle: greedy only, %zu sweeps with %d wave bit(s): no search task\n", best_n, best_wb);
+        return chosen.plan(queue, sink);
+      }
+      greedy_plan = chosen.plan(queue);
+      const double scale = (double)(bw == 128 ? 16 : 8) * (double)(1ull << nloc) / (16.0 * (double)(1ull << 30));
+      double bound_ms = 1e300;
+      for (const auto &sh : shapes) {
+        const size_t cap = (size_t)(cap0 + sh.first), kbound = std::max<size_t>({1, (nmovable + cap - 1) / cap, cone_of[sh.first]});
+        bound_ms = std::min(bound_ms, (double)kbound * (stream_floor_ms(sh.first) + (sh.first >= 2 ? 0.3 : 0.0)) * scale);
+      }
+      const double saving_ms = plan_predicted_ms(greedy_plan, nloc, bw) - bound_ms;
+      if (!sw.steps_pinned) budget = saving_ms > 0 ? std::min<uint64_t>(budget, (uint64_t)(saving_ms * kIdleSearchShare * kSearchChangesPerMs)) : 0;
+      if (sw.log)
+        fprintf(stderr, "[qh plan search] idle: greedy %zu sweeps, predicted %.2f ms; the bounds allow %.2f ms: saving <= %.2f ms, %llu label changes per task\n",
+                greedy_plan.sweeps.size(), plan_predicted_ms(greedy_plan, nloc, bw), bound_ms, saving_ms, (unsigned long long)budget);
+      if (budget < 5000) return greedy_plan;
+    }
     int streams = 6;
     if (const unsigned hw = usable_cpus(); hw && !keep_ghosts && !shapes.empty())
       streams = std::max(1, std::min(6, (int)(hw / shapes.size())));
     if (sw.streams) streams = sw.streams;
-    for (const auto &sh : shapes)
-      for (int s = 0; s < streams; ++s) { tasks.emplace_back(); tasks.back().wb = sh.first; tasks.back().K = sh.second; tasks.back().stream = (uint64_t)(s + 1); }
+    for (const auto &sh : shapes) {
+      const bool at_bound = idle && sh.second <= (nmovable + (size_t)(cap0 + sh.first) - 1) / (size_t)(cap0 + sh.first);
+      for (int s = 0; s < (at_bound ? 1 : streams); ++s) { tasks.emplace_back(); tasks.back().wb = sh.first; tasks.back().K = sh.second; tasks.back().stream = (uint64_t)(s + 1); }
+    }
     auto run = [&](Task &t) {
       const size_t i = (size_t)(&t - &tasks[0]);
       try {
@@ -1911,9 +1993,8 @@
     std::vector<std::thread> pool;
     const size_t workers = sw.threads ? std::min<size_t>(tasks.size(), usable_cpus()) : 0;
     try { while (pool.size() < workers) pool.emplace_back(drain); } catch (...) {}
-    PlanResult greedy_plan;
     std::exception_ptr greedy_failed;
-    try { greedy_plan = chosen.plan(queue); } catch (...) { greedy_failed = std::current_exception(); next = tasks.size(); }
+    try { if (!idle) greedy_plan = chosen.plan(queue); } catch (...) { greedy_failed = std::current_exception(); next = tasks.size(); }
     drain();
     for (std::thread &x : pool) x.join();
     if (greedy_failed) std::rethrow_exception(greedy_failed);
@@ -1939,7 +2020,7 @@
     if (win) return win->pr;
     return greedy_plan;
   }
-  return chosen.plan(queue);
+  return chosen.plan(queue, sink);
 }
 
 template <class F> int guard_planning(std::string *err, F &&f) {
@@ -1948,9 +2029,11 @@
   return QH_OK;
 }
 
-inline std::string plan_to_json(const std::vector<GateRec> &queue, const PlanRequest &rq) {
+inline std::string plan_to_json(const std::vector<GateRec> &queue, const PlanRequest &rq, double *plan_ms = nullptr) {
   if (rq.nloc < kLaneBits + 2) return "{\"sweeps\":[],\"note\":\"state too small for sweeps\"}";
+  const auto t0 = std::chrono::steady_clock::now();
   PlanResult pr = plan_best(queue, rq);
+  if (plan_ms) *plan_ms = std::chrono::duration<double, std::milli>(std::chrono::steady_clock::now() - t0).count();
   std::string s = "{\"noop_gates\":" + std::to_string(pr.noop_gates);
   if (rq.sw.dag)
     s += ",\"dag\":" + Planner(rq, 1).dag_json(queue);
diff --git a/qcc_amd/device.py b/qcc_amd/device.py
--- a/qcc_amd/device.py
+++ b/qcc_amd/device.py
@@ -458,6 +458,11 @@
     native.check(self.lib.qh_timer_laps(self.h, buf, cap, ctypes.byref(n)))
     return [float(buf[k]) for k in range(min(n.value, cap))]
 
+  def plan_ms(self):
+    ms = ctypes.c_double()
+    native.check(self.lib.qh_plan_ms(self.h, ctypes.byref(ms)))
+    return ms.value
+
   def plan_json(self):
     need = ctypes.c_uint64()
     native.check(self.lib.qh_plan_json(self.h, None, 0, ctypes.byref(need)))
diff --git a/qcc_amd/native.py b/qcc_amd/native.py
--- a/qcc_amd/native.py
+++ b/qcc_amd/native.py
@@ -113,6 +113,7 @@
     'qh_timer_lap': (_i32, [_vp]),
     'qh_timer_laps': (_i32, [_vp, ctypes.POINTER(ctypes.c_float), _i32, ctypes.POINTER(_i32)]),
     'qh_plan_json': (_i32, [_vp, ctypes.c_char_p, _u64, ctypes.POINTER(_u64)]),
+    'qh_plan_ms': (_i32, [_vp, _dp]),
     'qh_plan_export': (_i32, [_vp, _vp, _u64, ctypes.POINTER(_u64)]),
     'qh_plan_handlers': (_i32, [_vp, _vp, _u64, ctypes.POINTER(_u64)]),
     'qh_host_apply1': (_i32, [_vp, _dp, _i32, _i32, _i32]),
```

Result: no change. 28460 gate-applies/s (median of 2 runs) (-0.0%).
